# weilonghu/KGC-GCN

Measured on NVIDIA B200. Metric: edges/sec GCN fwd+bwd, higher is better.
Workload: dtype f32

## Files before the change

### include/kgc_b200.h

```cpp
#ifndef KGC_B200_H_
#define KGC_B200_H_

#include <stddef.h>
#include <stdint.h>

#ifdef __cplusplus
extern "C" {
#endif
#if defined(__GNUC__)
#pragma GCC visibility push(default)
#endif

#define KGC_ABI_VERSION 1

typedef struct { int32_t beg, end, out, flags; } kgc_item_t;

#define KGC_CHUNK_EDGES 32
typedef struct { int32_t head_slot, tail_slot; } kgc_chunk_t;

typedef struct { int32_t eid, a, b; float norm; } kgc_edge_rec_t;

const char* kgc_last_error(void);
int kgc_abi_version(void);

size_t kgc_csr_workspace_bytes(int64_t n_edges2, int64_t n_nodes, int64_t n_types);
int kgc_csr_build(const int64_t* src, const int64_t* dst, const int64_t* type,
                  int64_t n_edges2, int64_t n_edges_in, int64_t n_nodes, int64_t n_dst_rows, int64_t dst_offset,
                  int64_t n_types, int32_t deg_given, int32_t* deg, float* norm,
                  int32_t* perm_dst, int32_t* rowptr_dst, int32_t* rowmid_dst, kgc_edge_rec_t* rec_dst,
                  int32_t* perm_src, int32_t* rowptr_src, kgc_edge_rec_t* rec_src,
                  int32_t* perm_type, int32_t* rowptr_type, kgc_edge_rec_t* rec_type,
                  int64_t type_block_rows, void* workspace, size_t workspace_bytes, void* stream);
int64_t kgc_csr_type_rows(int64_t n_nodes, int64_t n_types, int64_t type_block_rows);
int kgc_block_sum(const float* in, int64_t n_blocks, int64_t n, float* out, void* stream);

int kgc_stream_plan_flags(const int32_t* seg_beg, const int32_t* seg_end, const int32_t* seg_row, int64_t n_seg,
                          int64_t n_rec, int32_t chunk, uint32_t* rowflags, int32_t* rec_seg, int32_t* inter, void* stream);

int kgc_agg_fwd(const float* x, const float* rel, int64_t n_types, const float* ee,
                const kgc_edge_rec_t* rec_dst, const uint32_t* rowflags, const kgc_chunk_t* chunks, int64_t n_rec,
                float* out_final, float* carry, int32_t D, void* stream);

int kgc_rows_fill(const int32_t* rows, int64_t n_rows, const float* addend, float* out, int32_t D, void* stream);

int kgc_rows_reduce(const float* part_in, const kgc_item_t* items, int64_t n_items, int64_t n_large,
                    float* out_final, float* out_part, const float* addend, int32_t D, void* stream);

int kgc_agg_bwd_src(const float* x, const float* rel, int64_t n_types, const float* ee, const float* g3,
                    const kgc_edge_rec_t* rec_src, const uint32_t* rowflags, const kgc_chunk_t* chunks, int64_t n_rec,
                    int64_t n_dst_rows, int64_t n_edges_in, const float* loop_addend,
                    float* d_ee, float* dx_final, float* carry, int32_t D, void* stream);

int kgc_agg_bwd_rel(const float* x, const float* ee, const float* g3,
                    const kgc_edge_rec_t* rec_type, const uint32_t* rowflags, const kgc_chunk_t* chunks, int64_t n_rec,
                    int64_t n_dst_rows, int64_t n_edges_in,
                    float* drel_final, float* carry, int32_t D, void* stream);

int64_t kgc_tail_num_blocks(int64_t n_rows);
int kgc_dropout_mask(const int64_t* seed, int32_t plane, float drop_p, int64_t n_elem, uint8_t* mask, void* stream);
int32_t kgc_keep_pitch(void);
int kgc_tail_fwd(const float* res3, const uint8_t* mask_in, const uint8_t* mask_out, const int64_t* seed, float drop_p,
                 float keep_scale, const float* bias, int64_t n_rows, int32_t Dout, float* pre, double* partials,
                 uint8_t* keep, void* stream);
int kgc_colsum_finalize(const double* partials, int64_t n_blocks, int32_t Dout, double* sums, void* stream);
int kgc_colstats_from_sums(const double* sums, int64_t n_rows, int32_t Dout, float eps, int32_t training,
                           const float* running_mean, const float* running_var, float* stats, void* stream);
int kgc_colstats_finalize(const double* partials, int64_t n_blocks, int64_t n_rows, int32_t Dout, float eps,
                          float momentum, float* running_mean, float* running_var, int64_t* num_batches_tracked,
                          double* sums, float* stats, void* stream);
int kgc_colsum_finalize2(const double* partials, int64_t n_blocks, int32_t Dout, double* sums, float* sums32,
                         void* stream);
int kgc_tail_apply(const float* pre, const float* stats, const float* gamma, const float* beta,
                   int64_t n_rows, int32_t Dout, float* all_ent, const int64_t* out_seed, float out_drop_p,
                   uint8_t* out_keep, void* stream);
int kgc_tail_bwd_reduce(const float* g_ent, const float* pre, const float* stats, const float* gamma, const float* beta,
                        int64_t n_rows, int32_t Dout, double* partials, const uint8_t* out_keep, float out_scale,
                        void* stream);
int kgc_tail_bwd_apply(const float* g_ent, const float* pre, const float* stats, const float* gamma, const float* beta,
                       const double* sums, int32_t training, int64_t n_rows, int64_t n_rows_global, int32_t Dout,
                       float* d_out, const uint8_t* keep, float keep_scale, float* d_res2, const uint8_t* out_keep,
                       float out_scale, void* stream);

int kgc_conv_prep(const float* rels, int32_t n_rels, const float* loop_rel, const float* loop_edge, const float* w_in,
                  const float* w_out, const float* w_loop, const float* w_rel, int32_t D, int32_t Dout, float* relp,
                  float* all_rel, float* packed_fwd, float* packed_bwd, void* stream);
int kgc_conv_param_grads(const float* m_loop, const float* w_loop, const float* loop_rel, const float* loop_edge,
                         const float* relp, const float* w_rel, const float* g_rel, const float* d_relp,
                         int32_t n_rels, int32_t D, int32_t Dout, float* d_w_loop, float* d_loop_rel,
                         float* d_loop_edge, float* d_rels, float* d_w_rel, const float* rel_add, void* stream);

size_t kgc_gemm_packed_b_bytes(int32_t N, int32_t K);
int kgc_gemm_pack_b(const float* B, int64_t stride_k, int64_t stride_n, int32_t N, int32_t K, float* packed,
                    void* stream);
int kgc_gemm_nt(const float* A, int64_t M, int32_t K, int64_t lda, const float* packed_b, int32_t N, float* C,
                int64_t ldc, void* stream);
int kgc_gemm_nt_batch(int32_t n_prob, const float* const* A, int64_t M, int32_t K, int64_t lda,
                      const float* const* packed_b, int32_t N, float* const* C, int64_t ldc, void* stream);
int kgc_gemm_nt_batch_masked(int32_t n_prob, const float* const* A, int64_t M, int32_t K, int64_t lda,
                             const float* const* packed_b, int32_t N, float* const* C, int64_t ldc, const uint8_t* keep,
                             int32_t keep_pitch, float keep_scale, void* stream);
int kgc_gemm_nt_trans(const float* At, int64_t M, int32_t K, int64_t ldat, const float* packed_b, int32_t N,
                      float* Ct, int64_t ldct, void* stream);
void kgc_gemm_set_debug(long long* buf);

size_t kgc_gemm_tn_workspace_bytes(int64_t M, int32_t Ka, int32_t Nb);
int kgc_gemm_tn(const float* A, int64_t lda, const float* B, int64_t ldb, int64_t M, int32_t Ka, int32_t Nb,
                float* C, void* workspace, size_t workspace_bytes, void* stream);

size_t kgc_gemm_tn_tc_workspace_bytes(int64_t M, int32_t Ka, int32_t Nb);
int kgc_gemm_tn_tc(const float* A, int64_t lda, const float* B, int64_t ldb, int64_t M, int32_t Ka, int32_t Nb,
                   float* C, void* workspace, size_t workspace_bytes, void* stream);

int kgc_gemm_nt_splitk(const float* A, int64_t lda, const float* Bt, int64_t ldb, int64_t K, int32_t Ma, int32_t Nb,
                       float* C, void* workspace, size_t workspace_bytes, void* stream);

int kgc_gemm_tn_tc_batch(int32_t n_prob, const float* const* A, int64_t lda, const float* const* B, int64_t ldb,
                         int64_t M, int32_t Ka, int32_t Nb, float* const* C, void* workspace, size_t workspace_bytes,
                         void* stream);
int kgc_gemm_tn_tc_batch_masked(int32_t n_prob, const float* const* A, int64_t lda, const float* const* B, int64_t ldb,
                                int64_t M, int32_t Ka, int32_t Nb, float* const* C, void* workspace, size_t workspace_bytes,
                                const uint8_t* keep, int32_t keep_pitch, float keep_scale, void* stream);

int kgc_label_build(const int64_t* qid, int64_t B, const int64_t* triples, const int64_t* ptr,
                    const int32_t* idx, int64_t n_entity, float pos, float add,
                    int64_t* triple_out, float* label, void* stream);

int kgc_neg_sample(const int64_t* qid, int64_t B, const int64_t* ptr, const int32_t* idx, int64_t n_entity,
                   const uint32_t* draws, int32_t k, int32_t tries, int32_t* neg, void* stream);

int kgc_edge_sample(const int64_t* src, const int64_t* dst, const int64_t* type, int64_t n_triples, const uint32_t* draws,
                    int64_t m, int64_t* sub_src, int64_t* sub_dst, int64_t* sub_type, int64_t* eids, void* stream);

size_t kgc_bn2d_partials_bytes(int32_t C);
int kgc_bn2d_relu_drop_fwd(const float* x, int64_t B, int32_t C, int32_t HW, const float* gamma, const float* beta,
                           float* running_mean, float* running_var, float eps, float momentum, int32_t training,
                           int32_t relu, const int64_t* seed, float drop_p, double* partials, float* stats, float* y,
                           void* stream);
int kgc_bn2d_relu_drop_bwd(const float* dy, const float* x, int64_t B, int32_t C, int32_t HW, const float* gamma,
                           const float* beta, const float* stats, int32_t training, int32_t relu, const int64_t* seed,
                           float drop_p, double* partials, float* sums, float* dx, void* stream);

int kgc_conv1ch_supported(int32_t F, int32_t K, int32_t H, int32_t W);
size_t kgc_conv1ch_bwd_workspace_bytes(int64_t B, int32_t F, int32_t K);
int kgc_conv1ch_fwd(const float* x, const float* w, const float* bias, int64_t B, int32_t F, int32_t K, int32_t H,
                    int32_t W, float* y, void* stream);
int kgc_conv1ch_bwd(const float* dy, const float* x, const float* w, int64_t B, int32_t F, int32_t K, int32_t H,
                    int32_t W, float* dx, float* dw, void* workspace, void* stream);

typedef struct { float* param; const float* grad; float* exp_avg; float* exp_avg_sq; } kgc_opt_tensor_t;
int32_t kgc_opt_chunk_elems(void);
int kgc_clip_adam_step(const kgc_opt_tensor_t* tensors, const int32_t* items, int64_t n_items, const float* hyper,
                       double* state, double* partials, void* stream);

int kgc_p2p_allreduce(void* const* stage_ptrs_dev, int64_t offset_bytes, void* const* flag_ptrs_dev, int32_t rank,
                      int32_t world, uint32_t* epoch, int32_t* error, const void* in, void* out, int64_t n_bytes,
                      int32_t is_double, void* stream);
int kgc_p2p_barrier(void* const* flag_ptrs_dev, int32_t rank, int32_t world, uint32_t* epoch, int32_t* error, void* stream);
int kgc_p2p_halo_gather(void* const* table_ptrs_dev, int32_t rank, const int32_t* rows, const int32_t* order, int64_t n_rows,
                        int64_t block_rows, int32_t D, void* stream);
int kgc_p2p_halo_reduce(void* const* part_ptrs_dev, int32_t world, const int32_t* idx, const int32_t* row_ids, int64_t n_rows,
                        const float* addend, float* out, int32_t D, void* stream);

typedef struct kgc_ingest kgc_ingest_t;
int kgc_ingest_open(const char* data_dir, kgc_ingest_t** out);
void kgc_ingest_close(kgc_ingest_t* h);
int64_t kgc_ingest_count(const kgc_ingest_t* h, int32_t what);
int kgc_ingest_copy(const kgc_ingest_t* h, int32_t array, void* dst, int64_t capacity_bytes);
const char* kgc_ingest_name(const kgc_ingest_t* h, int32_t kind, int64_t id);

int kgc_score_1n_fwd(const float* ent, int64_t n_ent, int32_t D, int64_t ld_ent, const float* packed_x, int32_t B,
                     const float* bias, float* pred, int64_t ld_pred, void* stream);
int kgc_score_1n_logits(const float* ent, int64_t n_ent, int32_t D, int64_t ld_ent, const float* packed_x, int32_t B,
                        const float* bias, float* logits, int64_t ld_logits, void* stream);
int kgc_score_1n_bwd_logit(const float* d_pred, int64_t ld_dp, const float* pred, int64_t ld_p, int64_t n_ent,
                           int32_t B, int32_t ldt, float* d_logitT, float* d_bias, void* stream);

int64_t kgc_label_mask_words(int64_t n_entity);
int kgc_label_mask_build(const int64_t* qid, int64_t B, const int64_t* triples, const int64_t* ptr, const int32_t* idx,
                         int64_t n_entity, uint32_t* mask, int64_t* triple_out, void* stream);
int kgc_bce_1n_bwd_logit(const float* pred, int64_t ld_p, const uint32_t* mask, int64_t n_ent, int32_t B, int32_t ldt,
                         float pos, float add, float* d_logitT, float* d_bias, double* loss_partial, float* loss,
                         void* stream);
int kgc_score_1n_fwd_t(const float* ent, int64_t n_ent, int32_t D, int64_t ld_ent, const float* packed_x, int32_t B,
                       const float* bias, float* pred_t, int64_t ld_t, void* stream);
int64_t kgc_bce_1n_t_blocks(int64_t n_ent);
int kgc_label_mask_t_build(const int64_t* qid, int64_t B, const int64_t* ptr, const int32_t* idx, int64_t n_entity,
                           uint32_t* mask_t, void* stream);
int kgc_bce_1n_bwd_logit_t(float* pred_t, const uint32_t* mask_t, int64_t n_ent, int32_t B, int32_t ldt, float pos, float add,
                           float* d_bias, double* loss_partial, float* loss, void* stream);

int32_t kgc_score_kpad(int32_t d);
int kgc_score_pack_entities(const float* all_ent, const float* bias, int64_t n, int32_t d,
                            uint16_t* e_bf16, void* stream);
int kgc_score_pack_queries(const float* xq, int64_t b, int32_t d, uint16_t* q_bf16, void* stream);
size_t kgc_score_pairs_workspace_bytes(int64_t n_pairs, int32_t kpad);
int kgc_score_pairs(const uint16_t* q_bf16, const uint16_t* e_bf16, const int32_t* pair_q, const int32_t* pair_e,
                    int64_t n_pairs, int32_t kpad, float* s_out, void* workspace, size_t workspace_bytes,
                    void* stream);
int kgc_score_rank(const uint16_t* q_bf16, const uint16_t* e_bf16, int64_t b, int64_t n, int32_t kpad,
                   const float* thr, int32_t* count_gt, int32_t* count_eq, void* stream);
int kgc_rank_count_dense(const float* logits, int64_t ld, int64_t n_ent, int64_t b, const float* thr,
                         int32_t* count_gt, int32_t* count_eq, void* stream);
int kgc_rank_finalize(const int32_t* count_gt, const int32_t* count_eq, const float* thr, const float* s_filt,
                      const int64_t* filt_ptr, const int32_t* filt_idx, const int64_t* obj, int64_t b,
                      int32_t* ranks, int32_t* eq_out, double* sums13, void* stream);

size_t kgc_score_topk_workspace_bytes(int64_t b, int64_t n, int32_t kpad, int32_t k);
int kgc_score_topk(const uint16_t* q_bf16, const uint16_t* e_bf16, int64_t b, int64_t n, int32_t kpad,
                   const int64_t* excl_ptr, const int32_t* excl_idx, int32_t k, float* top_s, int32_t* top_id,
                   int32_t* count, void* workspace, size_t workspace_bytes, void* stream);
size_t kgc_topk_dense_workspace_bytes(int64_t b, int64_t n, int32_t k);
int kgc_topk_dense(const float* logits, int64_t ld, int64_t n, int64_t b, const int64_t* excl_ptr,
                   const int32_t* excl_idx, int32_t k, float* top_s, int32_t* top_id, int32_t* count,
                   void* workspace, size_t workspace_bytes, void* stream);

#if defined(__GNUC__)
#pragma GCC visibility pop
#endif
#ifdef __cplusplus
}
#endif
#endif
```

### kgc-gcn_b200/_lib.py

```python
import ctypes
import os

import torch

_HERE = os.path.dirname(os.path.abspath(__file__))
LIB_PATH = os.environ.get('KGC_LIB_PATH') or os.path.join(_HERE, 'libkgc_b200.so')
_LIB = None

_vp, _i64, _i32, _f32, _sz = ctypes.c_void_p, ctypes.c_int64, ctypes.c_int32, ctypes.c_float, ctypes.c_size_t

SIGNATURES = {
    'kgc_last_error': (ctypes.c_char_p, []),
    'kgc_abi_version': (ctypes.c_int, []),
    'kgc_csr_workspace_bytes': (_sz, [_i64, _i64, _i64]),
    'kgc_csr_build': (ctypes.c_int, [_vp, _vp, _vp, _i64, _i64, _i64, _i64, _i64, _i64, _i32, _vp, _vp, _vp, _vp, _vp,
                                     _vp, _vp, _vp, _vp, _vp, _vp, _vp, _i64, _vp, _sz, _vp]),
    'kgc_csr_type_rows': (_i64, [_i64, _i64, _i64]),
    'kgc_block_sum': (ctypes.c_int, [_vp, _i64, _i64, _vp, _vp]),
    'kgc_stream_plan_flags': (ctypes.c_int, [_vp, _vp, _vp, _i64, _i64, _i32, _vp, _vp, _vp, _vp]),
    'kgc_agg_fwd': (ctypes.c_int, [_vp, _vp, _i64, _vp, _vp, _vp, _vp, _i64, _vp, _vp, _i32, _vp]),
    'kgc_rows_fill': (ctypes.c_int, [_vp, _i64, _vp, _vp, _i32, _vp]),
    'kgc_rows_reduce': (ctypes.c_int, [_vp, _vp, _i64, _i64, _vp, _vp, _vp, _i32, _vp]),
    'kgc_agg_bwd_src': (ctypes.c_int, [_vp, _vp, _i64, _vp, _vp, _vp, _vp, _vp, _i64, _i64, _i64, _vp, _vp, _vp, _vp, _i32, _vp]),
    'kgc_agg_bwd_rel': (ctypes.c_int, [_vp, _vp, _vp, _vp, _vp, _vp, _i64, _i64, _i64, _vp, _vp, _i32, _vp]),
    'kgc_tail_num_blocks': (_i64, [_i64]),
    'kgc_dropout_mask': (ctypes.c_int, [_vp, _i32, _f32, _i64, _vp, _vp]),
    'kgc_keep_pitch': (_i32, []),
    'kgc_tail_fwd': (ctypes.c_int, [_vp, _vp, _vp, _vp, _f32, _f32, _vp, _i64, _i32, _vp, _vp, _vp, _vp]),
    'kgc_colsum_finalize': (ctypes.c_int, [_vp, _i64, _i32, _vp, _vp]),
    'kgc_colstats_from_sums': (ctypes.c_int, [_vp, _i64, _i32, _f32, _i32, _vp, _vp, _vp, _vp]),
    'kgc_colstats_finalize': (ctypes.c_int, [_vp, _i64, _i64, _i32, _f32, _f32, _vp, _vp, _vp, _vp, _vp, _vp]),
    'kgc_colsum_finalize2': (ctypes.c_int, [_vp, _i64, _i32, _vp, _vp, _vp]),
    'kgc_tail_apply': (ctypes.c_int, [_vp, _vp, _vp, _vp, _i64, _i32, _vp, _vp, _f32, _vp, _vp]),
    'kgc_tail_bwd_reduce': (ctypes.c_int, [_vp, _vp, _vp, _vp, _vp, _i64, _i32, _vp, _vp, _f32, _vp]),
    'kgc_tail_bwd_apply': (ctypes.c_int, [_vp, _vp, _vp, _vp, _vp, _vp, _i32, _i64, _i64, _i32, _vp, _vp, _f32, _vp, _vp, _f32, _vp]),
    'kgc_gemm_packed_b_bytes': (_sz, [_i32, _i32]),
    'kgc_gemm_pack_b': (ctypes.c_int, [_vp, _i64, _i64, _i32, _i32, _vp, _vp]),
    'kgc_gemm_nt': (ctypes.c_int, [_vp, _i64, _i32, _i64, _vp, _i32, _vp, _i64, _vp]),
    'kgc_conv_prep': (ctypes.c_int, [_vp, _i32] + [_vp] * 6 + [_i32, _i32] + [_vp] * 5),
    'kgc_conv_param_grads': (ctypes.c_int, [_vp] * 8 + [_i32, _i32, _i32] + [_vp] * 7),
    'kgc_gemm_nt_batch': (ctypes.c_int, [_i32, _vp, _i64, _i32, _i64, _vp, _i32, _vp, _i64, _vp]),
    'kgc_gemm_nt_batch_masked': (ctypes.c_int, [_i32, _vp, _i64, _i32, _i64, _vp, _i32, _vp, _i64, _vp, _i32, _f32, _vp]),
    'kgc_gemm_tn_tc_batch_masked': (ctypes.c_int, [_i32, _vp, _i64, _vp, _i64, _i64, _i32, _i32, _vp, _vp, _sz, _vp, _i32, _f32, _vp]),
    'kgc_gemm_nt_trans': (ctypes.c_int, [_vp, _i64, _i32, _i64, _vp, _i32, _vp, _i64, _vp]),
    'kgc_gemm_nt_splitk': (ctypes.c_int, [_vp, _i64, _vp, _i64, _i64, _i32, _i32, _vp, _vp, _sz, _vp]),
    'kgc_gemm_set_debug': (None, [_vp]),
    'kgc_gemm_tn_workspace_bytes': (_sz, [_i64, _i32, _i32]),
    'kgc_gemm_tn_tc_workspace_bytes': (_sz, [_i64, _i32, _i32]),
    'kgc_gemm_tn_tc': (ctypes.c_int, [_vp, _i64, _vp, _i64, _i64, _i32, _i32, _vp, _vp, _sz, _vp]),
    'kgc_gemm_tn_tc_batch': (ctypes.c_int, [_i32, _vp, _i64, _vp, _i64, _i64, _i32, _i32, _vp, _vp, _sz, _vp]),
    'kgc_gemm_tn': (ctypes.c_int, [_vp, _i64, _vp, _i64, _i64, _i32, _i32, _vp, _vp, _sz, _vp]),
    'kgc_label_build': (ctypes.c_int, [_vp, _i64, _vp, _vp, _vp, _i64, _f32, _f32, _vp, _vp, _vp]),
    'kgc_neg_sample': (ctypes.c_int, [_vp, _i64, _vp, _vp, _i64, _vp, _i32, _i32, _vp, _vp]),
    'kgc_edge_sample': (ctypes.c_int, [_vp, _vp, _vp, _i64, _vp, _i64, _vp, _vp, _vp, _vp, _vp]),
    'kgc_bn2d_partials_bytes': (_sz, [_i32]),
    'kgc_bn2d_relu_drop_fwd': (ctypes.c_int, [_vp, _i64, _i32, _i32, _vp, _vp, _vp, _vp, _f32, _f32, _i32, _i32, _vp, _f32, _vp, _vp, _vp, _vp]),
    'kgc_bn2d_relu_drop_bwd': (ctypes.c_int, [_vp, _vp, _i64, _i32, _i32, _vp, _vp, _vp, _i32, _i32, _vp, _f32, _vp, _vp, _vp, _vp]),
    'kgc_conv1ch_supported': (_i32, [_i32, _i32, _i32, _i32]),
    'kgc_conv1ch_bwd_workspace_bytes': (_sz, [_i64, _i32, _i32]),
    'kgc_conv1ch_fwd': (ctypes.c_int, [_vp, _vp, _vp, _i64, _i32, _i32, _i32, _i32, _vp, _vp]),
    'kgc_conv1ch_bwd': (ctypes.c_int, [_vp, _vp, _vp, _i64, _i32, _i32, _i32, _i32, _vp, _vp, _vp, _vp]),
    'kgc_opt_chunk_elems': (_i32, []),
    'kgc_clip_adam_step': (ctypes.c_int, [_vp, _vp, _i64, _vp, _vp, _vp, _vp]),
    'kgc_p2p_allreduce': (ctypes.c_int, [_vp, _i64, _vp, _i32, _i32, _vp, _vp, _vp, _vp, _i64, _i32, _vp]),
    'kgc_p2p_barrier': (ctypes.c_int, [_vp, _i32, _i32, _vp, _vp, _vp]),
    'kgc_p2p_halo_gather': (ctypes.c_int, [_vp, _i32, _vp, _vp, _i64, _i64, _i32, _vp]),
    'kgc_p2p_halo_reduce': (ctypes.c_int, [_vp, _i32, _vp, _vp, _i64, _vp, _vp, _i32, _vp]),
    'kgc_ingest_open': (ctypes.c_int, [ctypes.c_char_p, _vp]),
    'kgc_ingest_close': (None, [_vp]),
    'kgc_ingest_count': (_i64, [_vp, _i32]),
    'kgc_ingest_copy': (ctypes.c_int, [_vp, _i32, _vp, _i64]),
    'kgc_ingest_name': (ctypes.c_char_p, [_vp, _i32, _i64]),
    'kgc_score_1n_fwd': (ctypes.c_int, [_vp, _i64, _i32, _i64, _vp, _i32, _vp, _vp, _i64, _vp]),
    'kgc_score_1n_logits': (ctypes.c_int, [_vp, _i64, _i32, _i64, _vp, _i32, _vp, _vp, _i64, _vp]),
    'kgc_rank_count_dense': (ctypes.c_int, [_vp, _i64, _i64, _i64, _vp, _vp, _vp, _vp]),
    'kgc_score_1n_bwd_logit': (ctypes.c_int, [_vp, _i64, _vp, _i64, _i64, _i32, _i32, _vp, _vp, _vp]),
    'kgc_label_mask_words': (_i64, [_i64]),
    'kgc_label_mask_build': (ctypes.c_int, [_vp, _i64, _vp, _vp, _vp, _i64, _vp, _vp, _vp]),
    'kgc_bce_1n_bwd_logit': (ctypes.c_int, [_vp, _i64, _vp, _i64, _i32, _i32, _f32, _f32, _vp, _vp, _vp, _vp, _vp]),
    'kgc_score_1n_fwd_t': (ctypes.c_int, [_vp, _i64, _i32, _i64, _vp, _i32, _vp, _vp, _i64, _vp]),
    'kgc_bce_1n_t_blocks': (_i64, [_i64]),
    'kgc_label_mask_t_build': (ctypes.c_int, [_vp, _i64, _vp, _vp, _i64, _vp, _vp]),
    'kgc_bce_1n_bwd_logit_t': (ctypes.c_int, [_vp, _vp, _i64, _i32, _i32, _f32, _f32, _vp, _vp, _vp, _vp]),
    'kgc_score_kpad': (_i32, [_i32]),
    'kgc_score_pack_entities': (ctypes.c_int, [_vp, _vp, _i64, _i32, _vp, _vp]),
    'kgc_score_pack_queries': (ctypes.c_int, [_vp, _i64, _i32, _vp, _vp]),
    'kgc_score_pairs_workspace_bytes': (_sz, [_i64, _i32]),
    'kgc_score_pairs': (ctypes.c_int, [_vp, _vp, _vp, _vp, _i64, _i32, _vp, _vp, _sz, _vp]),
    'kgc_score_rank': (ctypes.c_int, [_vp, _vp, _i64, _i64, _i32, _vp, _vp, _vp, _vp]),
    'kgc_rank_finalize': (ctypes.c_int, [_vp, _vp, _vp, _vp, _vp, _vp, _vp, _i64, _vp, _vp, _vp, _vp]),
    'kgc_score_topk_workspace_bytes': (_sz, [_i64, _i64, _i32, _i32]),
    'kgc_score_topk': (ctypes.c_int, [_vp, _vp, _i64, _i64, _i32, _vp, _vp, _i32, _vp, _vp, _vp, _vp, _sz, _vp]),
    'kgc_topk_dense_workspace_bytes': (_sz, [_i64, _i64, _i32]),
    'kgc_topk_dense': (ctypes.c_int, [_vp, _i64, _i64, _i64, _vp, _vp, _i32, _vp, _vp, _vp, _vp, _sz, _vp]),
}


def lib():
    global _LIB
    if _LIB is None:
        if not os.path.exists(LIB_PATH):
            raise RuntimeError('{} is missing: build it with `python -c "import __graft_entry__ as g; g.build()"` '
                               '(nvcc, sm_100a). There is no CPU or PyTorch fallback.'.format(LIB_PATH))
        handle = ctypes.CDLL(LIB_PATH)
        for name, (res, args) in SIGNATURES.items():
            fn = getattr(handle, name)
            fn.restype, fn.argtypes = res, args
        if handle.kgc_abi_version() != 1:
            raise RuntimeError('libkgc_b200.so ABI version mismatch')
        _LIB = handle
    return _LIB


LAUNCHES = 0
_KERNELS_PER_CALL = {'kgc_csr_build': 16, 'kgc_label_mask_build': 2, 'kgc_bce_1n_bwd_logit': 2, 'kgc_bce_1n_bwd_logit_t': 2, 'kgc_label_mask_t_build': 2, 'kgc_score_pairs': 3, 'kgc_rank_finalize': 2, 'kgc_score_topk': 2, 'kgc_topk_dense': 2, 'kgc_gemm_tn': 2, 'kgc_gemm_tn_tc': 2, 'kgc_gemm_tn_tc_batch': 2, 'kgc_gemm_tn_tc_batch_masked': 2}


def call(name, *args):
    global LAUNCHES
    h = lib()
    LAUNCHES += _KERNELS_PER_CALL.get(name, 1)
    rc = getattr(h, name)(*args)
    if rc != 0:
        raise RuntimeError('{} failed: {}'.format(name, h.kgc_last_error().decode('utf-8', 'replace')))


_WARNED = set()


def library_path(site, reason):
    msg = 'kgc_gcn_b200: {} is running on the torch library path ({})'.format(site, reason)
    if os.environ.get('KGC_STRICT', '0') not in ('', '0'):
        raise RuntimeError(msg + ' and KGC_STRICT=1 forbids it')
    if site not in _WARNED:
        _WARNED.add(site)
        import warnings
        warnings.warn(msg, RuntimeWarning, stacklevel=3)


def ptr(t):
    return None if t is None else ctypes.c_void_p(t.data_ptr())


def stream():
    return ctypes.c_void_p(torch.cuda.current_stream().cuda_stream)


def require_cuda(t, dtype, name):
    if not (torch.is_tensor(t) and t.is_cuda):
        raise RuntimeError('{} must be a CUDA tensor: the M-GCN hot path runs on the GPU only (no CPU fallback)'.format(name))
    if t.dtype != dtype:
        raise TypeError('{} must be {}, got {}'.format(name, dtype, t.dtype))
    return t if t.is_contiguous() else t.contiguous()
```

### kgc-gcn_b200/conv.py

```python
import os

import torch
import torch.nn as nn

from . import _lib
from .plan import get_plan


def get_param(shape):
    param = nn.Parameter(torch.empty(*shape))
    nn.init.xavier_uniform_(param.data)
    return param


def _mm(a, b, out):
    return torch.mm(a, b, out=out)


def gemm_nt(a, b_kn, out, plan=None, tag='b', packed=None):
    M, K = a.shape
    N = out.shape[1]
    if a.stride(1) != 1 or out.stride(1) != 1:
        raise ValueError('gemm_nt needs unit inner strides')
    p = _lib.ptr
    if packed is None:
        nbytes = int(_lib.lib().kgc_gemm_packed_b_bytes(N, K))
        if nbytes == 0:
            raise ValueError('gemm_nt: unsupported shape K={} N={}'.format(K, N))
        packed = plan.scratch('gemm_pack_' + tag, (nbytes // 4,)) if plan is not None else \
            torch.empty((nbytes // 4,), dtype=torch.float32, device=a.device)
        _lib.call('kgc_gemm_pack_b', p(b_kn), b_kn.stride(0), b_kn.stride(1), N, K, p(packed), _lib.stream())
    dst = out if (out.data_ptr() % 16 == 0 and out.stride(0) % 4 == 0) else \
        torch.empty((M, (N + 3) // 4 * 4), dtype=torch.float32, device=a.device)[:, :N]
    _lib.call('kgc_gemm_nt', p(a), M, K, a.stride(0), p(packed), N, p(dst), dst.stride(0), _lib.stream())
    if dst is not out:
        out.copy_(dst)
    return out


def gemm_nt_batch(a_list, packed_list, out_list, keep=None, keep_scale=1.0):
    import ctypes
    n = len(a_list)
    M, K = a_list[0].shape
    N = out_list[0].shape[1]
    lda, ldc = a_list[0].stride(0), out_list[0].stride(0)
    for a, o in zip(a_list, out_list):
        if a.shape != (M, K) or o.shape != (M, N) or a.stride() != (lda, 1) or o.stride() != (ldc, 1):
            raise ValueError('gemm_nt_batch needs operands of identical shape and strides')
    arr = lambda ts: (ctypes.c_void_p * n)(*[t.data_ptr() for t in ts])
    if keep is not None:
        _lib.call('kgc_gemm_nt_batch_masked', n, arr(a_list), M, K, lda, arr(packed_list), N, arr(out_list), ldc,
                  _lib.ptr(keep), keep.stride(0), float(keep_scale), _lib.stream())
    else:
        _lib.call('kgc_gemm_nt_batch', n, arr(a_list), M, K, lda, arr(packed_list), N, arr(out_list), ldc, _lib.stream())
    return out_list


def gemm_tn_batch(a_list, b_list, out_list, plan=None, keep=None, keep_scale=1.0):
    import ctypes
    n = len(a_list)
    M, Ka = a_list[0].shape
    Nb = b_list[0].shape[1]
    lda, ldb = a_list[0].stride(0), b_list[0].stride(0)
    same = all(a.shape == (M, Ka) and b.shape == (M, Nb) and a.stride() == (lda, 1) and b.stride() == (ldb, 1)
               and o.is_contiguous() for a, b, o in zip(a_list, b_list, out_list))
    if not same or Ka > 128 or Nb > 224:
        if keep is not None:
            raise ValueError('gemm_tn_batch: the masked form needs Ka <= 128, Nb <= 224 and operands of identical shape')
        for a, b, o in zip(a_list, b_list, out_list):
            gemm_tn(a, b, o, plan)
        return out_list
    nbytes = int(_lib.lib().kgc_gemm_tn_tc_workspace_bytes(M, Ka, Nb))
    ws = plan.scratch('kgc_gemm_tn_tc_ws', (nbytes // 4,)) if plan is not None else \
        torch.empty((nbytes // 4,), dtype=torch.float32, device=a_list[0].device)
    arr = lambda ts: (ctypes.c_void_p * n)(*[t.data_ptr() for t in ts])
    if keep is not None:
        _lib.call('kgc_gemm_tn_tc_batch_masked', n, arr(a_list), lda, arr(b_list), ldb, M, Ka, Nb, arr(out_list), _lib.ptr(ws),
                  nbytes, _lib.ptr(keep), keep.stride(0), float(keep_scale), _lib.stream())
    else:
        _lib.call('kgc_gemm_tn_tc_batch', n, arr(a_list), lda, arr(b_list), ldb, M, Ka, Nb, arr(out_list), _lib.ptr(ws), nbytes,
                  _lib.stream())
    return out_list


def _pack_b(b_kn):
    K, N = b_kn.shape
    nbytes = int(_lib.lib().kgc_gemm_packed_b_bytes(N, K))
    if nbytes == 0:
        raise ValueError('unsupported small operand K={} N={} (K <= 256, N <= 1024)'.format(K, N))
    packed = torch.empty((nbytes // 4,), dtype=torch.float32, device=b_kn.device)
    _lib.call('kgc_gemm_pack_b', _lib.ptr(b_kn), b_kn.stride(0), b_kn.stride(1), N, K, _lib.ptr(packed), _lib.stream())
    return packed


def gemm_nt_trans(a_t, b_kn, out_t):
    K, M = a_t.shape
    N = b_kn.shape[1]
    if a_t.stride(1) != 1 or out_t.stride(1) != 1 or out_t.shape != (N, M):
        raise ValueError('gemm_nt_trans needs unit inner strides and out_t of shape [N, M]')
    p = _lib.ptr
    _lib.call('kgc_gemm_nt_trans', p(a_t), M, K, a_t.stride(0), p(_pack_b(b_kn)), N, p(out_t), out_t.stride(0), _lib.stream())
    return out_t


def gemm_nt_splitk(a, bt, out):
    Ma, K = a.shape
    Nb = bt.shape[0]
    if a.stride(1) != 1 or bt.stride(1) != 1 or not out.is_contiguous():
        raise ValueError('gemm_nt_splitk needs unit inner strides and a contiguous output')
    nbytes = int(_lib.lib().kgc_gemm_tn_tc_workspace_bytes(K, Ma, Nb))
    ws = torch.empty((nbytes // 4,), dtype=torch.float32, device=a.device)
    p = _lib.ptr
    _lib.call('kgc_gemm_nt_splitk', p(a), a.stride(0), p(bt), bt.stride(0), K, Ma, Nb, p(out), p(ws), nbytes, _lib.stream())
    return out


class _LinearFn(torch.autograd.Function):

    @staticmethod
    def forward(ctx, x, weight, bias):
        x_, w_ = x.detach(), weight.detach()
        y = gemm_nt_splitk(x_, w_, torch.empty((x_.shape[0], w_.shape[0]), dtype=torch.float32, device=x.device))
        if bias is not None:
            y += bias.detach()
        ctx.save_for_backward(x_, w_)
        ctx.has_bias = bias is not None
        return y

    @staticmethod
    def backward(ctx, dy):
        x, w = ctx.saved_tensors
        dy = dy.contiguous()
        dx = dw = db = None
        if ctx.needs_input_grad[0]:
            dx = gemm_nt_trans(w, dy.t(), torch.empty_like(x))
        if ctx.needs_input_grad[1]:
            dw = gemm_nt_trans(x, dy, torch.empty_like(w))
        if ctx.has_bias and ctx.needs_input_grad[2]:
            db = dy.sum(0)
        return dx, dw, db


def linear_tc_supported(x, weight):
    B, F = x.shape
    O = weight.shape[0]
    return (x.is_cuda and x.dtype == torch.float32 and weight.dtype == torch.float32 and x.is_contiguous()
            and weight.is_contiguous() and 0 < B <= 128 and O <= 224 and O % 4 == 0 and F % 32 == 0 and F >= 4096
            and x.data_ptr() % 16 == 0 and weight.data_ptr() % 16 == 0)


def linear_tc(x, weight, bias=None):
    return _LinearFn.apply(x, weight, bias)


def gemm_tn(a, b, out, plan=None, tensor_cores=True):
    M, Ka = a.shape
    Nb = b.shape[1]
    if a.stride(1) != 1 or b.stride(1) != 1 or not out.is_contiguous():
        raise ValueError('gemm_tn needs unit inner strides and a contiguous output')
    if Nb > 256:
        raise ValueError('gemm_tn supports Nb <= 256')
    name = 'kgc_gemm_tn_tc' if (tensor_cores and Nb <= 224) else 'kgc_gemm_tn'
    for i0 in range(0, Ka, 128):
        kb = min(128, Ka - i0)
        a_blk, out_blk = a[:, i0:i0 + kb], out[i0:i0 + kb]
        nbytes = int(getattr(_lib.lib(), name + '_workspace_bytes')(M, kb, Nb))
        ws = plan.scratch(name + '_ws', (nbytes // 4,)) if plan is not None else \
            torch.empty((nbytes // 4,), dtype=torch.float32, device=a.device)
        p = _lib.ptr
        _lib.call(name, p(a_blk), a.stride(0), p(b), b.stride(0), M, kb, Nb, p(out_blk), p(ws), nbytes, _lib.stream())
    return out


class _Done(object):

    def wait(self):
        return None


class _StreamJoin(object):

    def __init__(self, stream):
        self.stream = stream

    def wait(self):
        torch.cuda.current_stream().wait_stream(self.stream)


class _Collectives(object):

    def __init__(self, group, world, n_global, n_hub=0, hub_idx_mine=None, hub_rows_mine=None, p2p=None, rank=0,
                 halo_rows=None, n_loc=None):
        self.group, self.world, self.n_global, self.rank = group, int(world), int(n_global), int(rank)
        self.n_loc = None if n_loc is None else int(n_loc)
        self.p2p = p2p
        self.halo_rows = halo_rows
        self.n_hub, self.hub_idx_mine, self.hub_rows_mine = int(n_hub), hub_idx_mine, hub_rows_mine

    def sum_hub_rows(self, planes, n_loc):
        if self.n_hub == 0:
            return
        buf = planes[:, n_loc:, :].contiguous()
        self.all_reduce(buf, 'hub_f')
        if self.hub_idx_mine.numel():
            planes[:, self.hub_rows_mine, :] = buf[:, self.hub_idx_mine, :]

    def spread_hub_rows(self, planes, n_planes, n_loc):
        if self.n_hub == 0:
            return
        buf = torch.zeros((n_planes, self.n_hub, planes.shape[2]), dtype=planes.dtype, device=planes.device)
        if self.hub_idx_mine.numel():
            buf[:, self.hub_idx_mine, :] = planes[:n_planes, self.hub_rows_mine, :]
        self.all_reduce(buf, 'hub_b')
        planes[:n_planes, n_loc:, :] = buf

    def all_gather_rows(self, x_local, async_op=False):
        import torch.distributed as dist
        out = torch.empty((self.world * x_local.shape[0],) + tuple(x_local.shape[1:]), dtype=x_local.dtype,
                          device=x_local.device)
        work = dist.all_gather_into_tensor(out, x_local.contiguous(), group=self.group, async_op=async_op)
        return (out, work) if async_op else out

    def gather_compact(self, x_blk):
        full = self.all_gather_rows(x_blk)
        return torch.cat([x_blk, full.index_select(0, self.halo_rows)], 0)

    def reduce_compact(self, partial, block):
        full = partial.new_zeros((self.world * block, partial.shape[1]))
        full[self.rank * block:(self.rank + 1) * block] = partial[:block]
        full[self.halo_rows] = partial[block:block + self.halo_rows.numel()]
        return self.reduce_scatter_rows(full)

    def reduce_scatter_rows(self, full, async_op=False):
        import torch.distributed as dist
        rows = full.shape[0] // self.world
        if dist.get_backend(self.group) == 'gloo':
            dist.all_reduce(full, group=self.group)
            r = dist.get_rank(self.group)
            out = full[r * rows:(r + 1) * rows].clone()
            return (out, None) if async_op else out
        out = torch.empty((rows,) + tuple(full.shape[1:]), dtype=full.dtype, device=full.device)
        work = dist.reduce_scatter_tensor(out, full.contiguous(), group=self.group, async_op=async_op)
        return (out, work) if async_op else out

    def all_reduce(self, t, tag=None):
        if self.p2p is not None and tag is not None and self.p2p.all_reduce(t, tag):
            return t
        import torch.distributed as dist
        dist.all_reduce(t, group=self.group)
        return t


class _ConvFn(torch.autograd.Function):

    @staticmethod
    def forward(ctx, x, rels, ee, w_in, w_out, w_loop, w_rel, loop_rel, loop_edge, gamma, beta, bias,
                plan, mask_in, mask_out, keep_scale, training, running_mean, running_var, eps, coll, seed, drop_p,
                bn_track=None, out_drop=None):
        Nl, D = x.shape
        Dout = w_in.shape[1]
        p, st = _lib.ptr, _lib.stream
        x = _lib.require_cuda(x, torch.float32, 'x')
        ee = _lib.require_cuda(ee, torch.float32, 'edge_embs')
        n_global = Nl if coll is None else coll.n_global
        n_hub = 0 if coll is None else coll.n_hub
        n_loc = Nl if coll is None or coll.n_loc is None else coll.n_loc
        if not 0 <= n_loc - Nl <= 1:
            raise ValueError('x has {} rows, the partition expects {} or {}'.format(Nl, n_loc, n_loc - 1))
        Nb = n_loc + n_hub
        compact = coll is not None and coll.halo_rows is not None
        n_table = Nl if coll is None else (Nb + coll.halo_rows.numel() if compact else Nb * coll.world)
        hybrid = coll is not None and coll.p2p is not None and coll.p2p.hybrid
        n_dst = n_table if hybrid else Nb
        if ee.shape[0] != plan.num_edges2 or n_dst != plan.num_dst_rows or plan.num_nodes != n_table:
            raise ValueError('edge_embs / x do not match the graph plan')
        T = rels.shape[0] + 1
        if T != plan.num_types:
            raise ValueError('rels_embs rows + 1 must equal the number of edge types of the plan')
        nf = int(_lib.lib().kgc_gemm_packed_b_bytes(Dout, D)) // 4
        nbk = int(_lib.lib().kgc_gemm_packed_b_bytes(D, Dout)) // 4
        if nf == 0 or nbk == 0:
            raise ValueError('unsupported layer width {} -> {} (<= 256)'.format(D, Dout))
        relp = torch.empty((T, D), dtype=torch.float32, device=x.device)
        all_rel_pad = torch.empty((T, Dout), dtype=torch.float32, device=x.device)
        packed_f = torch.empty((3, nf), dtype=torch.float32, device=x.device)
        packed_b = torch.empty((4, nbk), dtype=torch.float32, device=x.device)
        rels_c, wts = rels.detach().contiguous(), [w.detach().contiguous() for w in (w_in, w_out, w_loop, w_rel)]
        main, side = torch.cuda.current_stream(), plan.side_stream()
        side.wait_stream(main)
        with torch.cuda.stream(side):
            _lib.call('kgc_conv_prep', p(rels_c), T - 1, p(loop_rel.detach()), p(loop_edge.detach()), p(wts[0]), p(wts[1]),
                      p(wts[2]), p(wts[3]), D, Dout, p(relp), p(all_rel_pad), p(packed_f), p(packed_b), st())
        gather = None
        if coll is None:
            x_full = x
        elif coll.p2p is not None:
            ex = coll.p2p.exchange_stream
            ex.wait_stream(main)
            with torch.cuda.stream(ex):
                x_full = coll.p2p.gather(x, fence=not training)
            gather = _StreamJoin(ex)
        elif compact:
            x_blk = x if Nb == Nl else torch.cat([x, x.new_zeros((Nb - Nl, D))], 0)
            x_full, gather = coll.gather_compact(x_blk), _Done()
        else:
            x_full, gather = coll.all_gather_rows(x if Nb == Nl else torch.cat([x, x.new_zeros((Nb - Nl, D))], 0),
                                                  async_op=True)

        res3 = plan.scratch('res3', (3, Nl, Dout))
        if gather is not None:
            main.wait_stream(side)
            gemm_nt(x, None, res3[2], packed=packed_f[2])
            gather.wait()
        if max(x_full.shape[0], 3 * n_dst, ee.shape[0]) * (D // 4) >= 1 << 32:
            raise ValueError('kgc_gcn_b200: node / edge tables of 2^32 float4 elements or more are not supported')
        agg = torch.empty((2, n_dst, D), dtype=torch.float32, device=x.device)

        def level0(sp, out_final, carry):
            _lib.call('kgc_agg_fwd', p(x_full), p(rels_c), T - 1, p(ee), p(plan.rec_dst), p(sp.rowflags), p(sp.chunks), sp.n_rec,
                      p(out_final), p(carry), D, st())
        plan.run_reduction(plan.fwd, level0, agg, D, tag='f')
        if gather is None:
            main.wait_stream(side)

        if hybrid:
            coll.p2p.reduce_agg(agg)
        if gather is not None:
            coll.sum_hub_rows(agg, n_loc)
            gemm_nt_batch([agg[0, :Nl], agg[1, :Nl]], [packed_f[0], packed_f[1]], [res3[0], res3[1]])
        else:
            gemm_nt_batch([agg[0], agg[1], x], [packed_f[0], packed_f[1], packed_f[2]], [res3[0], res3[1], res3[2]])

        nb = int(_lib.lib().kgc_tail_num_blocks(Nl))
        partials = plan.scratch('colpart', (nb, 2, Dout), torch.float64)
        sums = torch.empty((2, Dout), dtype=torch.float64, device=x.device)
        pre = torch.empty((Nl, Dout), dtype=torch.float32, device=x.device)
        stats = torch.empty((3, Dout), dtype=torch.float32, device=x.device)
        all_ent = torch.empty((Nl, Dout), dtype=torch.float32, device=x.device)
        dropping = (mask_in is not None or seed is not None) and drop_p > 0.0
        keep = torch.empty((Nl, int(_lib.lib().kgc_keep_pitch())), dtype=torch.uint8, device=x.device) if dropping else None
        _lib.call('kgc_tail_fwd', p(res3), p(mask_in), p(mask_out), p(seed), float(drop_p), float(keep_scale), p(bias),
                  Nl, Dout, p(pre), p(partials), p(keep), st())
        if training and coll is None:
            mom, nbt = bn_track if bn_track is not None else (0.0, None)
            _lib.call('kgc_colstats_finalize', p(partials), nb, n_global, Dout, float(eps), float(mom),
                      p(running_mean) if bn_track is not None else None, p(running_var) if bn_track is not None else None,
                      p(nbt), None, p(stats), st())
        else:
            if training:
                _lib.call('kgc_colsum_finalize', p(partials), nb, Dout, p(sums), st())
                coll.all_reduce(sums, 'bn_f')
            _lib.call('kgc_colstats_from_sums', p(sums), n_global, Dout, float(eps), int(training), p(running_mean),
                      p(running_var), p(stats), st())
        out_p, out_seed = out_drop if out_drop is not None else (0.0, None)
        out_keep = torch.empty((Nl, int(_lib.lib().kgc_keep_pitch())), dtype=torch.uint8, device=x.device) if out_seed is not None else None
        _lib.call('kgc_tail_apply', p(pre), p(stats), p(gamma), p(beta), Nl, Dout, p(all_ent), p(out_seed), float(out_p),
                  p(out_keep), st())
        ctx.out_scale = 1.0 / (1.0 - float(out_p)) if out_seed is not None else 1.0
        all_rel = all_rel_pad[:-1]

        ctx.plan, ctx.training, ctx.keep_scale, ctx.has_bias, ctx.coll = plan, bool(training), float(keep_scale), \
            bias is not None, coll
        ctx.drop_p = float(drop_p)
        ctx.save_for_backward(x, x_full, relp, ee, w_in, w_out, w_loop, w_rel, loop_rel, loop_edge, gamma, beta, agg, pre,
                              all_ent, stats, keep, packed_b, out_keep)
        ctx.mark_non_differentiable(stats)
        return all_ent, all_rel, stats

    @staticmethod
    def backward(ctx, g_ent, g_rel, _g_stats):
        (x, x_full, relp, ee, w_in, w_out, w_loop, w_rel, loop_rel, loop_edge, gamma, beta, agg, pre, all_ent, stats, keep,
         packed_b, out_keep) = ctx.saved_tensors
        plan, coll = ctx.plan, ctx.coll
        Nl, D = x.shape
        n_global = Nl if coll is None else coll.n_global
        n_hub = 0 if coll is None else coll.n_hub
        n_loc = Nl if coll is None or coll.n_loc is None else coll.n_loc
        Nb = n_loc + n_hub
        Dout = w_in.shape[1]
        T = relp.shape[0]
        p, st = _lib.ptr, _lib.stream
        dev = x.device
        if g_ent is None:
            g_ent = torch.zeros_like(all_ent)
        g_ent = g_ent.contiguous()

        nb = int(_lib.lib().kgc_tail_num_blocks(Nl))
        partials = plan.scratch('colpart', (nb, 2, Dout), torch.float64)
        sums = torch.empty((2, Dout), dtype=torch.float64, device=dev)
        d_out = plan.scratch('d_out', (Nl, Dout))
        _lib.call('kgc_tail_bwd_reduce', p(g_ent), p(pre), p(stats), p(gamma), p(beta), Nl, Dout, p(partials), p(out_keep),
                  ctx.out_scale, st())
        if coll is None:
            sums32 = torch.empty((2, Dout), dtype=torch.float32, device=dev)
            _lib.call('kgc_colsum_finalize2', p(partials), nb, Dout, p(sums), p(sums32), st())
        else:
            _lib.call('kgc_colsum_finalize', p(partials), nb, Dout, p(sums), st())
            coll.all_reduce(sums, 'bn_b')
            sums32 = sums.float()
        mode = os.environ.get('KGC_TAIL_PLANES', '')
        three = (3 * Nl * Dout * 4 > (48 << 20)) if mode not in ('1', '3') else mode == '3'
        d_res2 = plan.scratch('d_res2', (2, Nl, Dout)) if three else None
        _lib.call('kgc_tail_bwd_apply', p(g_ent), p(pre), p(stats), p(gamma), p(beta), p(sums), int(ctx.training), Nl,
                  n_global, Dout, p(d_out), p(keep), ctx.keep_scale, p(d_res2), p(out_keep), ctx.out_scale, st())
        ups = [d_res2[0], d_res2[1], d_out] if three else [d_out, d_out, d_out]
        gkeep = None if three else keep
        d_beta, d_gamma = sums32[0], sums32[1]

        flat = torch.empty((3 * D * Dout + T * D + (Dout if ctx.has_bias else 0),), dtype=torch.float32, device=dev)
        d_w_in, d_w_out, m_loop = (flat[k * D * Dout:(k + 1) * D * Dout].view(D, Dout) for k in range(3))
        d_relp = flat[3 * D * Dout:3 * D * Dout + T * D].view(T, D)
        main, side = torch.cuda.current_stream(), plan.side_stream()
        side.wait_stream(main)
        with torch.cuda.stream(side):
            gemm_tn_batch([agg[0, :Nl], agg[1, :Nl], x], ups, [d_w_in, d_w_out, m_loop], plan,
                          keep=gkeep, keep_scale=ctx.keep_scale)
            if ctx.has_bias:
                torch.sum(d_out, 0, out=flat[3 * D * Dout + T * D:])

        hybrid = coll is not None and coll.p2p is not None and coll.p2p.hybrid
        g3 = coll.p2p.g3_planes() if hybrid else plan.scratch('g3', (3, Nb, D))
        gemm_nt_batch(ups, [packed_b[0], packed_b[1], packed_b[2]],
                      [g3[0, :Nl], g3[1, :Nl], g3[2, :Nl]], keep=gkeep, keep_scale=ctx.keep_scale)
        if n_hub:
            coll.spread_hub_rows(g3, 2, n_loc)
        if hybrid:
            coll.p2p.gather_g()
        p2p = None if coll is None else coll.p2p
        d_x_full = p2p.partial if (p2p is not None and not hybrid) else torch.empty((plan.num_nodes, D), dtype=torch.float32, device=dev)
        d_ee = torch.empty_like(ee)
        loop_addend = g3[2] if (coll is None or hybrid) else None

        def level0_src(sp, out_final, carry):
            _lib.call('kgc_agg_bwd_src', p(x_full), p(relp), relp.shape[0], p(ee), p(g3), p(plan.rec_src), p(sp.rowflags), p(sp.chunks),
                      sp.n_rec, plan.num_dst_rows, plan.num_edges_in, p(loop_addend), p(d_ee), p(out_final), p(carry),
                      D, st())
        plan.run_reduction(plan.bwd_src, level0_src, d_x_full, D, addend=loop_addend, tag='s')
        scatter = None
        if hybrid:
            ex = p2p.exchange_stream
            ex.wait_stream(main)
            with torch.cuda.stream(ex):
                p2p.reduce_dx(d_x_full, channel=1)
            d_x = d_x_full[:Nl]
        elif p2p is not None:
            d_x = torch.empty((Nl, D), dtype=torch.float32, device=dev)
            ex = p2p.exchange_stream
            ex.wait_stream(main)
            with torch.cuda.stream(ex):
                p2p.reduce(g3[2, :Nl], Nl, out=d_x, channel=1)
        compact = coll is not None and coll.halo_rows is not None
        if coll is not None and p2p is None and not compact:
            d_x, scatter = coll.reduce_scatter_rows(d_x_full, async_op=True)

        def level0_rel(sp, out_final, carry):
            _lib.call('kgc_agg_bwd_rel', p(x_full), p(ee), p(g3), p(plan.rec_type), p(sp.rowflags), p(sp.chunks), sp.n_rec,
                      plan.num_dst_rows, plan.num_edges_in, p(out_final), p(carry), D, st())
        plan.run_rel_reduction(level0_rel, d_relp, D)

        main.wait_stream(side)
        if coll is None:
            d_x = d_x_full
        elif p2p is not None:
            coll.all_reduce(flat, 'flat')
            main.wait_stream(p2p.exchange_stream)
        elif compact:
            coll.all_reduce(flat, 'flat')
            d_x = coll.reduce_compact(d_x_full, Nb)[:Nl] + g3[2, :Nl]
        else:
            coll.all_reduce(flat, 'flat')
            if scatter is not None:
                scatter.wait()
            d_x = d_x[:Nl] + g3[2, :Nl]
        d_bias = flat[3 * D * Dout + T * D:] * 3.0 if ctx.has_bias else None
        small = torch.empty((2 * D * Dout + 2 * D + (T - 1) * D,), dtype=torch.float32, device=dev)
        d_w_loop, d_w_rel = small[:D * Dout].view(D, Dout), small[D * Dout:2 * D * Dout].view(D, Dout)
        o = 2 * D * Dout
        d_loop_rel, d_loop_edge, d_rels = small[o:o + D].view(1, D), small[o + D:o + 2 * D].view(1, D), small[o + 2 * D:].view(T - 1, D)
        g_rel_c = None if g_rel is None else g_rel.contiguous()
        rel_add = None
        if g_rel_c is not None and T - 1 >= 256 and g_rel_c.data_ptr() % 16 == 0 and Dout % 4 == 0 and (D * Dout) % 32 == 0:
            rel_add = gemm_nt(g_rel_c, None, torch.empty((T - 1, D), dtype=torch.float32, device=dev), packed=packed_b[3])
            gemm_tn(relp[:T - 1], g_rel_c, d_w_rel, plan)
        _lib.call('kgc_conv_param_grads', p(m_loop), p(w_loop.detach().contiguous()), p(loop_rel.detach()), p(loop_edge.detach()),
                  p(relp), p(w_rel.detach().contiguous()), p(g_rel_c), p(d_relp), T - 1, D, Dout, p(d_w_loop), p(d_loop_rel),
                  p(d_loop_edge), p(d_rels), p(d_w_rel), p(rel_add), st())
        return (d_x, d_rels, d_ee, d_w_in, d_w_out, d_w_loop, d_w_rel, d_loop_rel, d_loop_edge, d_gamma, d_beta, d_bias,
                None, None, None, None, None, None, None, None, None, None, None, None, None)


class MGCNConv(nn.Module):

    def __init__(self, in_channels, out_channels, num_relations, bias=False, dropout=0.1, **kwargs):
        super(MGCNConv, self).__init__()
        self.in_channels = in_channels
        self.out_channels = out_channels
        self.num_relations = num_relations
        self.aggr = 'add'

        self.ent_bn = nn.BatchNorm1d(out_channels)
        self.drop = nn.Dropout(dropout)
        self.act = torch.tanh

        self.loop_weight = get_param((in_channels, out_channels))
        self.in_weight = get_param((in_channels, out_channels))
        self.out_weight = get_param((in_channels, out_channels))
        self.rels_weight = get_param((in_channels, out_channels))
        self.loop_rel = get_param((1, in_channels))
        self.loop_edge = get_param((1, in_channels))

        if bias is True:
            self.register_parameter('bias', nn.Parameter(torch.zeros(out_channels)))
        else:
            self.register_parameter('bias', None)
        self._forced_masks = None
        self.register_buffer('_drop_seed', torch.zeros(1, dtype=torch.int64), persistent=False)
        self._drop_seeded = False

    def set_dropout_masks(self, mask_in, mask_out):
        self._forced_masks = None if mask_in is None else (mask_in, mask_out)

    def compute_norm(self, edge_index, num_ent):
        ei = torch.cat([edge_index, edge_index], 1).contiguous()
        et = torch.zeros(ei.size(1), dtype=torch.int64, device=ei.device)
        return get_plan(ei, et, num_ent, 1).norm[:edge_index.size(1)].clone()

    def _masks(self, n_rows, device):
        p = self.drop.p
        if not self.training or p == 0.0:
            return None, None, 1.0, None, 0.0
        if self._forced_masks is not None:
            m_in, m_out = self._forced_masks
            return (m_in.to(device=device, dtype=torch.uint8).contiguous(),
                    m_out.to(device=device, dtype=torch.uint8).contiguous(), 1.0 / (1.0 - p), None, p)
        if not self._drop_seeded:
            self._drop_seed.fill_(int(torch.randint(0, 2 ** 62, (1,)).item()))
            self._drop_seeded = True
        self._drop_seed.add_(0x9E3779B97F4A7C15 & 0x7FFFFFFFFFFFFFFF)
        return None, None, 1.0 / (1.0 - p), self._drop_seed.clone(), p

    def _out_drop_cfg(self, p, seed):
        if not self.training or not p or p <= 0.0:
            return None
        if seed is None:
            if not self._drop_seeded:
                self._drop_seed.fill_(int(torch.randint(0, 2 ** 62, (1,)).item()))
                self._drop_seeded = True
            self._drop_seed.add_(0x9E3779B97F4A7C15 & 0x7FFFFFFFFFFFFFFF)
            seed = self._drop_seed.clone()
        self._last_out_seed = seed
        return float(p), seed

    def dropout_masks(self, seed, n_rows):
        out = []
        for plane in (0, 1):
            m = torch.empty((n_rows, self.out_channels), dtype=torch.uint8, device=seed.device)
            _lib.call('kgc_dropout_mask', _lib.ptr(seed), plane, float(self.drop.p), m.numel(), _lib.ptr(m), _lib.stream())
            out.append(m)
        return out

    def forward(self, x, edge_index, edge_type, edge_norm, edge_embs, rels_embs, size=None, _out_drop=0.0):
        num_ent = x.size(0)
        plan = get_plan(edge_index, edge_type, num_ent, rels_embs.size(0) + 1)
        m_in, m_out, keep_scale, seed, drop_p = self._masks(num_ent, x.device)
        self._last_seed = seed
        bn = self.ent_bn
        use_batch_stats = self.training or bn.running_mean is None
        track = self.training and bn.track_running_stats and bn.running_mean is not None
        fused = track and bn.momentum is not None
        all_ent, all_rel, stats = _ConvFn.apply(
            x, rels_embs, edge_embs, self.in_weight, self.out_weight, self.loop_weight, self.rels_weight,
            self.loop_rel, self.loop_edge, bn.weight, bn.bias, self.bias, plan, m_in, m_out, keep_scale,
            use_batch_stats, bn.running_mean, bn.running_var, bn.eps, None, seed, drop_p,
            (float(bn.momentum), bn.num_batches_tracked) if fused else None, self._out_drop_cfg(_out_drop, seed))
        if track and not fused:
            self._update_running_stats(stats, num_ent)
        return all_ent, all_rel

    def _update_running_stats(self, stats, n_rows):
        bn = self.ent_bn
        if self.training and bn.track_running_stats and bn.running_mean is not None:
            with torch.no_grad():
                bn.num_batches_tracked += 1
                mom = bn.momentum if bn.momentum is not None else 1.0 / float(bn.num_batches_tracked)
                unbias = float(n_rows) / float(max(n_rows - 1, 1))
                bn.running_mean.mul_(1.0 - mom).add_(stats[0], alpha=mom)
                bn.running_var.mul_(1.0 - mom).add_(stats[1], alpha=mom * unbias)

    def forward_partitioned(self, x_local, part, edge_embs_local, rels_embs):
        m_in, m_out, keep_scale, seed, drop_p = self._masks(x_local.size(0), x_local.device)
        if seed is not None:
            seed = seed + part.rank
        self._last_seed = seed
        bn = self.ent_bn
        use_batch_stats = self.training or bn.running_mean is None
        coll = _Collectives(part.group, part.world, part.num_nodes, part.n_hub, part.hub_idx_mine, part.hub_rows_mine,
                            part.p2p(x_local.shape[1]), part.rank, getattr(part, 'halo_rows64', None), part.n_loc)
        all_ent, all_rel, stats = _ConvFn.apply(
            x_local, rels_embs, edge_embs_local, self.in_weight, self.out_weight, self.loop_weight, self.rels_weight,
            self.loop_rel, self.loop_edge, bn.weight, bn.bias, self.bias, part.plan, m_in, m_out, keep_scale,
            use_batch_stats, bn.running_mean, bn.running_var, bn.eps, coll, seed, drop_p)
        self._update_running_stats(stats, part.num_nodes)
        return all_ent, all_rel

    def __repr__(self):
        return '{}({}, {}, num_relations={})'.format(self.__class__.__name__, self.in_channels, self.out_channels,
                                                     self.num_relations)
```

### kgc-gcn_b200/csrc/gemm_tf32x3.cu

```cuda
#include <cuda.h>

#include <cstdlib>
#include "common.cuh"

namespace kgc {
namespace {

constexpr int kBM = 128;
constexpr int kBK = 32;
constexpr int kUK = 8;
constexpr int kMaxKB = 8;
constexpr int kMaxStages = 8;
constexpr int kAStages = 4;
constexpr int kAccCols = 256;
constexpr int kTmemColsTS = kAccCols + kAStages * 64;
constexpr int kTileA = kBM * kBK * 4;
constexpr int kThreadsG = 480;
constexpr int kSplitWarps = 8;
constexpr int kBBudget = 116 * 1024;
constexpr int kTmemColsG = 256;
constexpr int kEpiBuf = 32 * 128;
constexpr int kEpiStage = 4 * 2 * kEpiBuf;

__device__ __forceinline__ uint32_t s_u32(const void* p) { return (uint32_t)__cvta_generic_to_shared(p); }
__device__ __forceinline__ void mb_init(uint64_t* bar, uint32_t count) {
  asm volatile("mbarrier.init.shared::cta.b64 [%0], %1;" ::"r"(s_u32(bar)), "r"(count));
}
__device__ __forceinline__ void mb_expect_tx(uint64_t* bar, uint32_t bytes) {
  asm volatile("mbarrier.arrive.expect_tx.shared::cta.b64 _, [%0], %1;" ::"r"(s_u32(bar)), "r"(bytes) : "memory");
}
__device__ __forceinline__ void mb_arrive(uint64_t* bar) {
  asm volatile("mbarrier.arrive.shared::cta.b64 _, [%0];" ::"r"(s_u32(bar)) : "memory");
}
__device__ __forceinline__ void mb_wait(uint64_t* bar, uint32_t parity) {
  asm volatile(
      "{\n"
      ".reg .pred P1;\n"
      "LAB_WAIT:\n"
      "mbarrier.try_wait.parity.shared::cta.b64 P1, [%0], %1;\n"
      "@P1 bra DONE;\n"
      "bra LAB_WAIT;\n"
      "DONE:\n"
      "}" ::"r"(s_u32(bar)),
      "r"(parity)
      : "memory");
}
__device__ __forceinline__ void tma_2d(void* smem_dst, const CUtensorMap* map, uint64_t* bar, int c0, int c1) {
  asm volatile(
      "cp.async.bulk.tensor.2d.shared::cluster.global.mbarrier::complete_tx::bytes [%0], [%1, {%3, %4}], [%2];" ::"r"(
          s_u32(smem_dst)),
      "l"(reinterpret_cast<uint64_t>(map)), "r"(s_u32(bar)), "r"(c0), "r"(c1)
      : "memory");
}
__device__ __forceinline__ void tma_3d(void* smem_dst, const CUtensorMap* map, uint64_t* bar, int c0, int c1, int c2) {
  asm volatile(
      "cp.async.bulk.tensor.3d.shared::cluster.global.mbarrier::complete_tx::bytes [%0], [%1, {%3, %4, %5}], [%2];" ::"r"(
          s_u32(smem_dst)),
      "l"(reinterpret_cast<uint64_t>(map)), "r"(s_u32(bar)), "r"(c0), "r"(c1), "r"(c2)
      : "memory");
}
__device__ __forceinline__ void tma_store_2d(const CUtensorMap* map, const void* smem_src, int c0, int c1) {
  asm volatile("cp.async.bulk.tensor.2d.global.shared::cta.bulk_group [%0, {%2, %3}], [%1];" ::"l"(
                   reinterpret_cast<uint64_t>(map)),
               "r"(s_u32(smem_src)), "r"(c0), "r"(c1)
               : "memory");
}
__device__ __forceinline__ void tma_store_3d(const CUtensorMap* map, const void* smem_src, int c0, int c1, int c2) {
  asm volatile("cp.async.bulk.tensor.3d.global.shared::cta.bulk_group [%0, {%2, %3, %4}], [%1];" ::"l"(
                   reinterpret_cast<uint64_t>(map)),
               "r"(s_u32(smem_src)), "r"(c0), "r"(c1), "r"(c2)
               : "memory");
}
__device__ __forceinline__ void umma_tf32(uint32_t tmem_d, uint64_t adesc, uint64_t bdesc, uint32_t idesc, uint32_t acc) {
  asm volatile(
      "{\n"
      ".reg .pred p;\n"
      "setp.ne.b32 p, %4, 0;\n"
      "tcgen05.mma.cta_group::1.kind::tf32 [%0], %1, %2, %3, p;\n"
      "}" ::"r"(tmem_d),
      "l"(adesc), "l"(bdesc), "r"(idesc), "r"(acc)
      : "memory");
}
__device__ __forceinline__ void umma_tf32_ts(uint32_t tmem_d, uint32_t a_tmem, uint64_t bdesc, uint32_t idesc, uint32_t acc) {
  asm volatile(
      "{\n"
      ".reg .pred p;\n"
      "setp.ne.b32 p, %4, 0;\n"
      "tcgen05.mma.cta_group::1.kind::tf32 [%0], [%1], %2, %3, p;\n"
      "}" ::"r"(tmem_d),
      "r"(a_tmem), "l"(bdesc), "r"(idesc), "r"(acc)
      : "memory");
}
__device__ __forceinline__ void tmem_st16_g(uint32_t taddr, const uint32_t (&v)[16]) {
  asm volatile(
      "tcgen05.st.sync.aligned.32x32b.x16.b32 [%0], "
      "{%1, %2, %3, %4, %5, %6, %7, %8, %9, %10, %11, %12, %13, %14, %15, %16};" ::"r"(taddr),
      "r"(v[0]), "r"(v[1]), "r"(v[2]), "r"(v[3]), "r"(v[4]), "r"(v[5]), "r"(v[6]), "r"(v[7]), "r"(v[8]), "r"(v[9]),
      "r"(v[10]), "r"(v[11]), "r"(v[12]), "r"(v[13]), "r"(v[14]), "r"(v[15])
      : "memory");
}
__device__ __forceinline__ bool elect_one() {
  uint32_t pred = 0;
  asm volatile(
      "{\n"
      ".reg .b32 rx;\n"
      ".reg .pred px;\n"
      "elect.sync rx|px, 0xFFFFFFFF;\n"
      "@px mov.s32 %0, 1;\n"
      "}"
      : "+r"(pred));
  return pred != 0;
}
__device__ __forceinline__ uint32_t tf32_rn(float v) { return (__float_as_uint(v) + 0x1000u) & 0xFFFFE000u; }
__device__ __forceinline__ void split_tf32(uint32_t v, uint32_t& hi, uint32_t& lo) {
  hi = tf32_rn(__uint_as_float(v));
  lo = tf32_rn(__uint_as_float(v) - __uint_as_float(hi));
}
__device__ __forceinline__ void umma_commit_g(uint64_t* bar) {
  asm volatile("tcgen05.commit.cta_group::1.mbarrier::arrive::one.shared::cluster.b64 [%0];" ::"r"(s_u32(bar)) : "memory");
}
__device__ __forceinline__ void tmem_ld32_g(uint32_t taddr, uint32_t (&v)[32]) {
  asm volatile(
      "tcgen05.ld.sync.aligned.32x32b.x32.b32 "
      "{%0, %1, %2, %3, %4, %5, %6, %7, %8, %9, %10, %11, %12, %13, %14, %15, "
      "%16, %17, %18, %19, %20, %21, %22, %23, %24, %25, %26, %27, %28, %29, %30, %31}, [%32];"
      : "=r"(v[0]), "=r"(v[1]), "=r"(v[2]), "=r"(v[3]), "=r"(v[4]), "=r"(v[5]), "=r"(v[6]), "=r"(v[7]), "=r"(v[8]),
        "=r"(v[9]), "=r"(v[10]), "=r"(v[11]), "=r"(v[12]), "=r"(v[13]), "=r"(v[14]), "=r"(v[15]), "=r"(v[16]),
        "=r"(v[17]), "=r"(v[18]), "=r"(v[19]), "=r"(v[20]), "=r"(v[21]), "=r"(v[22]), "=r"(v[23]), "=r"(v[24]),
        "=r"(v[25]), "=r"(v[26]), "=r"(v[27]), "=r"(v[28]), "=r"(v[29]), "=r"(v[30]), "=r"(v[31])
      : "r"(taddr));
}
__device__ __forceinline__ uint64_t sw128_desc(uint32_t smem_addr) {
  uint64_t d = 0;
  d |= (uint64_t)((smem_addr & 0x3FFFF) >> 4);
  d |= (uint64_t)(1024 >> 4) << 32;
  d |= (uint64_t)1 << 46;
  d |= (uint64_t)2 << 61;
  return d;
}

constexpr int kMaxBatch = 3;
struct GemmMaps {
  CUtensorMap a[kMaxBatch], bhi[kMaxBatch], blo[kMaxBatch], c[kMaxBatch], c16[kMaxBatch];
};

struct GemmParams {
  int64_t M;
  int32_t n_prob;
  int32_t N, K;
  int32_t n_kb, ksteps, NT, n_ntiles, n_mtiles, stages;
  float* C;
  int64_t ldc;
  const float* row_bias;
  int32_t act;
  int32_t trans_c;
  int32_t trans_a;
  const uint8_t* keep;
  int32_t keep_pitch;
  float keep_scale;
  long long* dbg;
};

__global__ void __launch_bounds__(kThreadsG, 1)
gemm_tf32x3_kernel(const __grid_constant__ GemmMaps maps, const GemmParams P) {
  extern __shared__ uint8_t smem_raw[];
  if (P.dbg != nullptr && threadIdx.x == 0) {
    long long g;
    asm volatile("mov.u64 %0, %globaltimer;" : "=l"(g));
    atomicMin(reinterpret_cast<long long*>(P.dbg) + 8 * 64 + 0, g);
    if (blockIdx.x == 0) { P.dbg[8 * 64 + 2] = g; P.dbg[8 * 64 + 3] = clock64(); }
  }
  uint8_t* base = reinterpret_cast<uint8_t*>((reinterpret_cast<uintptr_t>(smem_raw) + 1023) & ~uintptr_t(1023));
  const int warp = threadIdx.x / 32, lane = threadIdx.x % 32;
  const int tile_b = P.NT * kBK * 4;
  const int tile_b_al = (tile_b + 1023) & ~1023;
  uint8_t* s_bhi = base;
  uint8_t* s_blo = s_bhi + P.n_kb * tile_b_al;
  const int kStages = P.stages;
  uint8_t* s_a = s_blo + P.n_kb * tile_b_al;
  uint8_t* s_stage = s_a + kStages * kTileA;
  uint64_t* bars = reinterpret_cast<uint64_t*>(s_stage + kEpiStage);
  uint64_t* b_full = bars;
  uint64_t* raw_full = bars + 1;
  uint64_t* raw_empty = raw_full + kMaxStages;
  uint64_t* split_full = raw_empty + kMaxStages;
  uint64_t* split_empty = split_full + kAStages;
  uint64_t* acc_full = split_empty + kAStages;
  uint64_t* acc_empty = acc_full + 2;
  uint32_t* tmem_slot = reinterpret_cast<uint32_t*>(acc_empty + 2);

  if (warp == 0 && lane == 0) {
    mb_init(b_full, 1);
    for (int i = 0; i < kStages; ++i) {
      mb_init(raw_full + i, 1);
      mb_init(raw_empty + i, kSplitWarps);
    }
    for (int i = 0; i < kAStages; ++i) {
      mb_init(split_full + i, kSplitWarps);
      mb_init(split_empty + i, 1);
    }
    for (int i = 0; i < 2; ++i) {
      mb_init(acc_full + i, 1);
      mb_init(acc_empty + i, 4);
    }
    asm volatile("fence.mbarrier_init.release.cluster;" ::: "memory");
    asm volatile("fence.proxy.async.shared::cta;" ::: "memory");
  }
  if (warp == 14) {
    asm volatile("tcgen05.alloc.cta_group::1.sync.aligned.shared::cta.b32 [%0], %1;" ::"r"(s_u32(tmem_slot)), "r"(kTmemColsTS)
                 : "memory");
    asm volatile("tcgen05.relinquish_alloc_permit.cta_group::1.sync.aligned;" ::: "memory");
  }
  asm volatile("tcgen05.fence::before_thread_sync;" ::: "memory");
  __syncthreads();
  asm volatile("tcgen05.fence::after_thread_sync;" ::: "memory");
  const uint32_t tmem_base = *tmem_slot;
  const uint32_t tmem_a = tmem_base + kAccCols;
  const bool dbg_on = P.dbg != nullptr && blockIdx.x == 0;
  int dbg_n = 0;
#define KGC_DBG(role) do { if (dbg_on && dbg_n < 64) P.dbg[(role) * 64 + dbg_n++] = clock64(); } while (0)

  const int groups = P.n_prob * P.n_ntiles;
  const int prob = (blockIdx.x % groups) / P.n_ntiles;
  const int nt = blockIdx.x % P.n_ntiles;
  const int first = blockIdx.x / groups;
  const int step = gridDim.x / groups;
  const CUtensorMap* map_a = &maps.a[prob];
  const CUtensorMap* map_bhi = &maps.bhi[prob];
  const CUtensorMap* map_blo = &maps.blo[prob];
  const CUtensorMap* map_c = &maps.c[prob];
  const CUtensorMap* map_c16 = &maps.c16[prob];

  if (warp == 0) {
    if (lane == 0) {
      mb_expect_tx(b_full, 2u * P.n_kb * tile_b);
      for (int kb = 0; kb < P.n_kb; ++kb) {
        tma_2d(s_bhi + kb * tile_b_al, map_bhi, b_full, kb * kBK, nt * P.NT);
        tma_2d(s_blo + kb * tile_b_al, map_blo, b_full, kb * kBK, nt * P.NT);
      }
      int stage = 0;
      uint32_t phase = 0;
      for (int mt = first; mt < P.n_mtiles; mt += step) {
        for (int kb = 0; kb < P.n_kb; ++kb) {
          mb_wait(raw_empty + stage, phase ^ 1);
          KGC_DBG(0);
          mb_expect_tx(raw_full + stage, kTileA);
          if (P.trans_a) tma_3d(s_a + stage * kTileA, map_a, raw_full + stage, 0, kb * kBK, mt * (kBM / 32));
          else tma_2d(s_a + stage * kTileA, map_a, raw_full + stage, kb * kBK, mt * kBM);
          if (++stage == kStages) { stage = 0; phase ^= 1; }
        }
      }
    }
  } else if (warp >= 2 && warp < 2 + kSplitWarps) {
    const int quarter = warp % 4, half = (warp - 2) / 4;
    const int r = quarter * 32 + lane;
    int stage = 0, ts = 0;
    uint32_t phase = 0, tphase = 0;
    const bool masked = P.keep != nullptr && prob < 2 && !P.trans_a;
    uint32_t kcur[kMaxKB], knxt[kMaxKB];
#pragma unroll
    for (int j = 0; j < kMaxKB; ++j) kcur[j] = knxt[j] = 0u;
    auto load_keep = [&](int mt_, uint32_t (&w)[kMaxKB]) {
      const int64_t grow = (int64_t)mt_ * kBM + r;
      if (mt_ < P.n_mtiles && grow < P.M) {
        const uint4* kp = reinterpret_cast<const uint4*>(P.keep + grow * P.keep_pitch);
#pragma unroll
        for (int q = 0; q < kMaxKB / 2; ++q) {
          const uint4 t4 = __ldg(kp + q);
          w[2 * q] = half ? t4.y : t4.x;
          w[2 * q + 1] = half ? t4.w : t4.z;
        }
      }
    };
    if (masked) load_keep(first, knxt);
    for (int mt = first; mt < P.n_mtiles; mt += step) {
      if (masked) {
#pragma unroll
        for (int j = 0; j < kMaxKB; ++j) kcur[j] = knxt[j];
        load_keep(mt + step, knxt);
      }
      for (int kb = 0; kb < P.n_kb; ++kb) {
        uint32_t kw = 0;
        if (masked) {
#pragma unroll
          for (int j = 0; j < kMaxKB; ++j)
            if (kb == j) kw = kcur[j];
          if (prob == 1) kw >>= 4;
        }
        mb_wait(raw_full + stage, phase);
        if (warp == 2 && lane == 0) KGC_DBG(1);
        uint32_t h[16], l[16];
        if (P.trans_a) {
          const uint8_t* col = s_a + stage * kTileA + quarter * 4096 + ((lane & 3) << 2);
#pragma unroll
          for (int i = 0; i < 16; ++i) {
            const int kk = half * 16 + i;
            const uint32_t v = *reinterpret_cast<const uint32_t*>(col + kk * 128 + (((lane >> 2) ^ (kk & 7)) << 4));
            split_tf32(v, h[i], l[i]);
          }
        } else {
          const uint8_t* row = s_a + stage * kTileA + r * 128;
          uint4 v[4];
#pragma unroll
          for (int i = 0; i < 4; ++i) v[i] = *reinterpret_cast<const uint4*>(row + (((half * 4 + i) ^ (r & 7)) << 4));
          if (masked) {
#pragma unroll
            for (int i = 0; i < 4; ++i) {
              const uint32_t nb = kw >> (8 * i);
              v[i].x = (nb & 1u) ? __float_as_uint(__uint_as_float(v[i].x) * P.keep_scale) : 0u;
              v[i].y = (nb & 2u) ? __float_as_uint(__uint_as_float(v[i].y) * P.keep_scale) : 0u;
              v[i].z = (nb & 4u) ? __float_as_uint(__uint_as_float(v[i].z) * P.keep_scale) : 0u;
              v[i].w = (nb & 8u) ? __float_as_uint(__uint_as_float(v[i].w) * P.keep_scale) : 0u;
            }
          }
#pragma unroll
          for (int i = 0; i < 4; ++i) {
            split_tf32(v[i].x, h[4 * i + 0], l[4 * i + 0]);
            split_tf32(v[i].y, h[4 * i + 1], l[4 * i + 1]);
            split_tf32(v[i].z, h[4 * i + 2], l[4 * i + 2]);
            split_tf32(v[i].w, h[4 * i + 3], l[4 * i + 3]);
          }
        }
        __syncwarp();
        if (lane == 0) mb_arrive(raw_empty + stage);
        mb_wait(split_empty + ts, tphase ^ 1);
        if (warp == 2 && lane == 0) KGC_DBG(2);
        asm volatile("tcgen05.fence::after_thread_sync;" ::: "memory");
        const uint32_t taddr = tmem_a + ((uint32_t)(quarter * 32) << 16) + ts * 64 + half * 16;
        tmem_st16_g(taddr, h);
        tmem_st16_g(taddr + 32, l);
        asm volatile("tcgen05.wait::st.sync.aligned;" ::: "memory");
        asm volatile("tcgen05.fence::before_thread_sync;" ::: "memory");
        __syncwarp();
        if (lane == 0) mb_arrive(split_full + ts);
        if (warp == 2 && lane == 0) KGC_DBG(3);
        if (++stage == kStages) { stage = 0; phase ^= 1; }
        if (++ts == kAStages) { ts = 0; tphase ^= 1; }
      }
    }
  } else if (warp == 1) {
    {
      const uint32_t idesc = (1u << 4) | (2u << 7) | (2u << 10) | ((uint32_t)(P.NT >> 3) << 17) | ((uint32_t)(kBM >> 4) << 24);
      int ts = 0, acc = 0;
      uint32_t tphase = 0, acc_phase = 0;
      mb_wait(b_full, 0);
      asm volatile("tcgen05.fence::after_thread_sync;" ::: "memory");
      for (int mt = first; mt < P.n_mtiles; mt += step) {
        mb_wait(acc_empty + acc, acc_phase ^ 1);
        asm volatile("tcgen05.fence::after_thread_sync;" ::: "memory");
        const uint32_t d_addr = tmem_base + acc * (kAccCols / 2);
        for (int kb = 0; kb < P.n_kb; ++kb) {
          mb_wait(split_full + ts, tphase);
          if (lane == 0) KGC_DBG(4);
          asm volatile("tcgen05.fence::after_thread_sync;" ::: "memory");
          const int nk = min(kBK / kUK, P.ksteps - kb * (kBK / kUK));
          const uint32_t a_hi = tmem_a + ts * 64, a_lo = a_hi + 32;
          const uint64_t b_hi = sw128_desc(s_u32(s_bhi + kb * tile_b_al));
          const uint64_t b_lo = sw128_desc(s_u32(s_blo + kb * tile_b_al));
          if (elect_one()) {
#pragma unroll
            for (int k = 0; k < kBK / kUK; ++k) {
              if (k < nk) {
                umma_tf32_ts(d_addr, a_lo + 8 * k, b_hi + 2 * k, idesc, (k != 0 || kb != 0) ? 1u : 0u);
                umma_tf32_ts(d_addr, a_hi + 8 * k, b_lo + 2 * k, idesc, 1u);
                umma_tf32_ts(d_addr, a_hi + 8 * k, b_hi + 2 * k, idesc, 1u);
              }
            }
            umma_commit_g(split_empty + ts);
            if (kb == P.n_kb - 1) umma_commit_g(acc_full + acc);
          }
          __syncwarp();
          if (lane == 0) KGC_DBG(5);
          if (++ts == kAStages) { ts = 0; tphase ^= 1; }
        }
        if (++acc == 2) { acc = 0; acc_phase ^= 1; }
      }
    }
  } else if (warp >= 10 && warp <= 13) {
    const int quarter = warp % 4;
    uint8_t* stg = s_stage + (warp - 10) * (2 * kEpiBuf);
    const int64_t row_q = quarter * 32;
    int acc = 0, buf = 0;
    uint32_t acc_phase = 0;
    for (int mt = first; mt < P.n_mtiles; mt += step) {
      mb_wait(acc_full + acc, acc_phase);
      if (warp == 10 && lane == 0) KGC_DBG(6);
      asm volatile("tcgen05.fence::after_thread_sync;" ::: "memory");
      const int64_t m0 = (int64_t)mt * kBM + row_q;
      const uint32_t taddr = tmem_base + ((uint32_t)(quarter * 32) << 16) + acc * (kAccCols / 2);
      for (int c0 = 0; c0 < P.NT; c0 += 32) {
        uint32_t v[32];
        tmem_ld32_g(taddr + c0, v);
        asm volatile("tcgen05.wait::ld.sync.aligned;" ::: "memory");
        if (c0 + 32 >= P.NT) {
          asm volatile("tcgen05.fence::before_thread_sync;" ::: "memory");
          __syncwarp();
          if (lane == 0) mb_arrive(acc_empty + acc);
        }
        if (lane == 0) asm volatile("cp.async.bulk.wait_group.read 1;" ::: "memory");
        __syncwarp();
        uint8_t* bb = stg + buf * kEpiBuf;
        const bool wide = c0 + 32 <= P.NT;
        if (P.row_bias != nullptr) {
          const float bv = m0 + lane < P.M ? P.row_bias[m0 + lane] : 0.f;
#pragma unroll
          for (int j = 0; j < 32; ++j) {
            const float z = __uint_as_float(v[j]) + bv;
            v[j] = __float_as_uint(P.act == 1 ? 1.f / (1.f + expf(-z)) : z);
          }
        }
        if (P.trans_c) {
#pragma unroll
          for (int j = 0; j < 32; ++j)
            *reinterpret_cast<uint32_t*>(bb + j * 128 + ((((lane >> 2) ^ (j & 7)) << 4) | ((lane & 3) << 2))) = v[j];
        } else if (wide) {
          uint8_t* bx = bb + lane * 128;
          const int sw = lane & 7;
#pragma unroll
          for (int q = 0; q < 8; ++q)
            *reinterpret_cast<uint4*>(bx + ((q ^ sw) << 4)) = make_uint4(v[4 * q], v[4 * q + 1], v[4 * q + 2], v[4 * q + 3]);
        } else {
          uint8_t* bx = bb + lane * 64;
          const int sw = (lane >> 1) & 3;
#pragma unroll
          for (int q = 0; q < 4; ++q)
            *reinterpret_cast<uint4*>(bx + ((q ^ sw) << 4)) = make_uint4(v[4 * q], v[4 * q + 1], v[4 * q + 2], v[4 * q + 3]);
        }
        asm volatile("fence.proxy.async.shared::cta;" ::: "memory");
        __syncwarp();
        if (lane == 0) {
          const int col = nt * P.NT + c0;
          if (m0 < P.M && col < P.N) {
            if (P.trans_c) tma_store_2d(wide ? map_c : map_c16, bb, (int)m0, col);
            else tma_store_2d(wide ? map_c : map_c16, bb, col, (int)m0);
          }
          asm volatile("cp.async.bulk.commit_group;" ::: "memory");
        }
        buf ^= 1;
      }
      if (warp == 10 && lane == 0) KGC_DBG(7);
      if (++acc == 2) { acc = 0; acc_phase ^= 1; }
    }
    if (lane == 0) asm volatile("cp.async.bulk.wait_group 0;" ::: "memory");
  }
  asm volatile("tcgen05.fence::before_thread_sync;" ::: "memory");
  __syncthreads();
  if (P.dbg != nullptr && threadIdx.x == 0) {
    long long g;
    asm volatile("mov.u64 %0, %globaltimer;" : "=l"(g));
    atomicMax(reinterpret_cast<long long*>(P.dbg) + 8 * 64 + 1, g);
    if (blockIdx.x == 0) { P.dbg[8 * 64 + 4] = g; P.dbg[8 * 64 + 5] = clock64(); }
  }
  if (warp == 14) {
    asm volatile("tcgen05.dealloc.cta_group::1.sync.aligned.b32 %0, %1;" ::"r"(tmem_base), "r"(kTmemColsTS) : "memory");
  }
}

__global__ void pack_b_kernel(const float* __restrict__ B, int64_t sk, int64_t sn, int N, int K, int n_pad, int k_pad,
                              float* __restrict__ hi, float* __restrict__ lo) {
  const int i = blockIdx.x * blockDim.x + threadIdx.x;
  if (i >= n_pad * k_pad) return;
  const int n = i / k_pad, k = i % k_pad;
  float v = 0.f;
  if (n < N && k < K) v = B[(int64_t)k * sk + (int64_t)n * sn];
  uint32_t h, l;
  split_tf32(__float_as_uint(v), h, l);
  hi[i] = __uint_as_float(h);
  lo[i] = __uint_as_float(l);
}

struct PrepArgs {
  const float *rels, *loop_rel, *loop_edge, *w0, *w1, *w2, *w_rel;
  int n_rels, D, Dout;
  int n_pad_f, k_pad_f, n_pad_b, k_pad_b;
  float *relp, *all_rel, *packed_f, *packed_b;
};

__global__ void __launch_bounds__(256) conv_prep_kernel(const PrepArgs a) {
  const int T = a.n_rels + 1;
  int i = blockIdx.x * blockDim.x + threadIdx.x;
  const int n0 = T * a.D, n1 = T * a.Dout, nf = a.n_pad_f * a.k_pad_f, nb = a.n_pad_b * a.k_pad_b;
  if (i < n0) {
    const int t = i / a.D, c = i % a.D;
    a.relp[i] = t < a.n_rels ? a.rels[i] : a.loop_rel[c];
    return;
  }
  i -= n0;
  if (i < n1) {
    const int t = i / a.Dout, o = i % a.Dout;
    const float* r = t < a.n_rels ? a.rels + (int64_t)t * a.D : a.loop_rel;
    float acc = 0.f;
#pragma unroll 25
    for (int c = 0; c < a.D; ++c) acc = fmaf(r[c], a.w_rel[(int64_t)c * a.Dout + o], acc);
    a.all_rel[i] = acc;
    return;
  }
  i -= n1;
  if (i < 3 * nf) {
    const int h = i / nf, j0 = i % nf, k = j0 / a.n_pad_f, n = j0 % a.n_pad_f, j = n * a.k_pad_f + k;
    float v = 0.f;
    if (n < a.Dout && k < a.D) {
      const float* wh = h == 0 ? a.w0 : (h == 1 ? a.w1 : a.w2);
      v = wh[(int64_t)k * a.Dout + n];
      if (h == 2) v *= a.loop_rel[k] * a.loop_edge[k];
    }
    uint32_t hi, lo;
    split_tf32(__float_as_uint(v), hi, lo);
    float* dst = a.packed_f + (int64_t)h * 2 * nf;
    dst[j] = __uint_as_float(hi);
    dst[nf + j] = __uint_as_float(lo);
    return;
  }
  i -= 3 * nf;
  if (i < 4 * nb) {
    const int h = i / nb, j = i % nb, n = j / a.k_pad_b, k = j % a.k_pad_b;
    float v = 0.f;
    if (n < a.D && k < a.Dout) {
      const float* wh = h == 0 ? a.w0 : (h == 1 ? a.w1 : (h == 2 ? a.w2 : a.w_rel));
      v = wh[(int64_t)n * a.Dout + k];
      if (h == 2) v *= a.loop_rel[n] * a.loop_edge[n];
    }
    uint32_t hi, lo;
    split_tf32(__float_as_uint(v), hi, lo);
    float* dst = a.packed_b + (int64_t)h * 2 * nb;
    dst[j] = __uint_as_float(hi);
    dst[nb + j] = __uint_as_float(lo);
  }
}

struct ParamGradArgs {
  const float *m_loop, *w_loop, *loop_rel, *loop_edge, *relp, *w_rel, *g_rel, *d_relp;
  int n_rels, D, Dout;
  float *d_w_loop, *d_loop_rel, *d_loop_edge, *d_rels, *d_w_rel;
};

__global__ void __launch_bounds__(256) conv_param_grads_kernel(const ParamGradArgs a) {
  const int T = a.n_rels + 1;
  int i = blockIdx.x * blockDim.x + threadIdx.x;
  const int nw = a.D * a.Dout;
  if (i < nw) {
    const int c = i / a.Dout;
    a.d_w_loop[i] = a.loop_rel[c] * a.loop_edge[c] * a.m_loop[i];
    return;
  }
  i -= nw;
  if (i < nw) {
    const int c = i / a.Dout, o = i % a.Dout;
    float acc = 0.f;
    if (a.g_rel != nullptr) {
#pragma unroll 8
      for (int t = 0; t < a.n_rels; ++t) acc = fmaf(a.relp[(int64_t)t * a.D + c], a.g_rel[(int64_t)t * a.Dout + o], acc);
    }
    a.d_w_rel[i] = acc;
    return;
  }
  i -= nw;
  const int pair = i / 32, lane = i % 32;
  if (pair < T * a.D) {
    const int t = pair / a.D, c = pair % a.D;
    const float* u = t < a.n_rels ? a.g_rel + (int64_t)t * a.Dout : a.m_loop + (int64_t)c * a.Dout;
    const float* w = t < a.n_rels ? a.w_rel + (int64_t)c * a.Dout : a.w_loop + (int64_t)c * a.Dout;
    float acc = 0.f;
    if (t == a.n_rels || a.g_rel != nullptr)
      for (int o = lane; o < a.Dout; o += 32) acc = fmaf(u[o], w[o], acc);
#pragma unroll
    for (int s = 16; s > 0; s >>= 1) acc += __shfl_xor_sync(0xFFFFFFFFu, acc, s);
    if (lane == 0) {
      const float val = a.d_relp[pair];
      if (t < a.n_rels) {
        a.d_rels[pair] = val + acc;
      } else {
        a.d_loop_edge[c] = acc * a.loop_rel[c];
        a.d_loop_rel[c] = acc * a.loop_edge[c] + val;
      }
    }
  }
}

__global__ void __launch_bounds__(256) conv_param_grads2_kernel(const ParamGradArgs a, const float* __restrict__ rel_add) {
  int i = blockIdx.x * blockDim.x + threadIdx.x;
  const int nw = a.D * a.Dout;
  if (i < nw) {
    const int c = i / a.Dout;
    a.d_w_loop[i] = a.loop_rel[c] * a.loop_edge[c] * a.m_loop[i];
    return;
  }
  i -= nw;
  const int n_el = a.n_rels * a.D, n_el_pad = (n_el + 31) & ~31;
  if (i < n_el_pad) {
    if (i < n_el) a.d_rels[i] = a.d_relp[i] + rel_add[i];
    return;
  }
  i -= n_el_pad;
  const int c = i / 32, lane = i % 32;
  if (c < a.D) {
    const float* u = a.m_loop + (int64_t)c * a.Dout;
    const float* w = a.w_loop + (int64_t)c * a.Dout;
    float acc = 0.f;
    for (int o = lane; o < a.Dout; o += 32) acc = fmaf(u[o], w[o], acc);
#pragma unroll
    for (int s = 16; s > 0; s >>= 1) acc += __shfl_xor_sync(0xFFFFFFFFu, acc, s);
    if (lane == 0) {
      a.d_loop_edge[c] = acc * a.loop_rel[c];
      a.d_loop_rel[c] = acc * a.loop_edge[c] + a.d_relp[(int64_t)a.n_rels * a.D + c];
    }
  }
}

typedef CUresult (*EncodeTiledFn)(CUtensorMap*, CUtensorMapDataType, cuuint32_t, void*, const cuuint64_t*, const cuuint64_t*,
                                  const cuuint32_t*, const cuuint32_t*, CUtensorMapInterleave, CUtensorMapSwizzle,
                                  CUtensorMapL2promotion, CUtensorMapFloatOOBfill);
int encode_fn(EncodeTiledFn* out) {
  ensure_thread_context();
  static EncodeTiledFn cached = nullptr;
  if (!cached) {
    void* fn = nullptr;
    cudaDriverEntryPointQueryResult qres;
    KGC_CUDA_TRY(cudaGetDriverEntryPoint("cuTensorMapEncodeTiled", &fn, cudaEnableDefault, &qres));
    KGC_REQUIRE(qres == cudaDriverEntryPointSuccess && fn != nullptr, "cuTensorMapEncodeTiled not available");
    cached = reinterpret_cast<EncodeTiledFn>(fn);
  }
  *out = cached;
  return 0;
}
int make_map_f32(CUtensorMap* map, const void* ptr, int64_t rows, int64_t cols, int64_t pitch, int box_rows,
                 CUtensorMapSwizzle swizzle = CU_TENSOR_MAP_SWIZZLE_128B, int box_cols = kBK) {
  EncodeTiledFn enc;
  if (encode_fn(&enc)) return 1;
  KGC_REQUIRE((reinterpret_cast<uintptr_t>(ptr) & 15) == 0 && (pitch * 4) % 16 == 0, "operand must be 16-byte aligned with a 16-byte pitch");
  cuuint64_t dims[2] = {(cuuint64_t)cols, (cuuint64_t)rows};
  cuuint64_t strides[1] = {(cuuint64_t)pitch * 4};
  cuuint32_t box[2] = {(cuuint32_t)box_cols, (cuuint32_t)box_rows};
  cuuint32_t estr[2] = {1, 1};
  CUresult r = enc(map, CU_TENSOR_MAP_DATA_TYPE_FLOAT32, 2, const_cast<void*>(ptr), dims, strides, box, estr,
                   CU_TENSOR_MAP_INTERLEAVE_NONE, swizzle, CU_TENSOR_MAP_L2_PROMOTION_L2_256B,
                   CU_TENSOR_MAP_FLOAT_OOB_FILL_NONE);
  KGC_REQUIRE(r == CUDA_SUCCESS, "cuTensorMapEncodeTiled failed (" + std::to_string((int)r) + ")");
  return 0;
}

int make_map_f32_groups(CUtensorMap* map, const void* ptr, int64_t rows, int groups, int64_t pitch, int box_groups,
                        CUtensorMapSwizzle swizzle) {
  EncodeTiledFn enc;
  if (encode_fn(&enc)) return 1;
  KGC_REQUIRE((reinterpret_cast<uintptr_t>(ptr) & 15) == 0 && (pitch * 4) % 16 == 0, "operand must be 16-byte aligned with a 16-byte pitch");
  cuuint64_t dims[3] = {32, (cuuint64_t)rows, (cuuint64_t)groups};
  cuuint64_t strides[2] = {(cuuint64_t)pitch * 4, 128};
  cuuint32_t box[3] = {32, 32, (cuuint32_t)box_groups};
  cuuint32_t estr[3] = {1, 1, 1};
  CUresult r = enc(map, CU_TENSOR_MAP_DATA_TYPE_FLOAT32, 3, const_cast<void*>(ptr), dims, strides, box, estr,
                   CU_TENSOR_MAP_INTERLEAVE_NONE, swizzle, CU_TENSOR_MAP_L2_PROMOTION_L2_256B,
                   CU_TENSOR_MAP_FLOAT_OOB_FILL_NONE);
  KGC_REQUIRE(r == CUDA_SUCCESS, "cuTensorMapEncodeTiled (grouped operand) failed (" + std::to_string((int)r) + ")");
  return 0;
}
int make_map_f32_mn_groups(CUtensorMap* map, const void* ptr, int64_t rows, int groups, int64_t pitch) {
  return make_map_f32_groups(map, ptr, rows, groups, pitch, groups, CU_TENSOR_MAP_SWIZZLE_128B_ATOM_32B);
}

int make_map_f32_parts(CUtensorMap* map, const void* ptr, int64_t parts, int64_t rows, int64_t cols) {
  EncodeTiledFn enc;
  if (encode_fn(&enc)) return 1;
  KGC_REQUIRE((reinterpret_cast<uintptr_t>(ptr) & 15) == 0 && cols % 4 == 0, "partials must be 16-byte aligned with a 16-byte pitch");
  cuuint64_t dims[3] = {(cuuint64_t)cols, (cuuint64_t)rows, (cuuint64_t)parts};
  cuuint64_t strides[2] = {(cuuint64_t)cols * 4, (cuuint64_t)rows * cols * 4};
  cuuint32_t box[3] = {32, 32, 1};
  cuuint32_t estr[3] = {1, 1, 1};
  CUresult r = enc(map, CU_TENSOR_MAP_DATA_TYPE_FLOAT32, 3, const_cast<void*>(ptr), dims, strides, box, estr,
                   CU_TENSOR_MAP_INTERLEAVE_NONE, CU_TENSOR_MAP_SWIZZLE_128B, CU_TENSOR_MAP_L2_PROMOTION_L2_256B,
                   CU_TENSOR_MAP_FLOAT_OOB_FILL_NONE);
  KGC_REQUIRE(r == CUDA_SUCCESS, "cuTensorMapEncodeTiled failed (" + std::to_string((int)r) + ")");
  return 0;
}

struct Tiling {
  int n_kb, k_pad, ksteps, NT, n_ntiles, n_pad;
};
int make_tiling(int N, int K, Tiling* t) {
  if (N <= 0 || K <= 0 || K > kMaxKB * kBK || N > 1024) return 1;
  t->n_kb = (K + kBK - 1) / kBK;
  t->k_pad = t->n_kb * kBK;
  t->ksteps = (K + kUK - 1) / kUK;
  int nt_max = kBBudget / (2 * t->n_kb * kBK * 4);
  nt_max = nt_max / 16 * 16;
  if (nt_max > 128) nt_max = 128;
  if (nt_max < 16) return 1;
  t->n_ntiles = (N + nt_max - 1) / nt_max;
  t->NT = ((N + t->n_ntiles - 1) / t->n_ntiles + 15) / 16 * 16;
  t->n_pad = t->NT * t->n_ntiles;
  return 0;
}


constexpr int kTnRows = 32;
constexpr int kTnBox = kTnRows * 128;
constexpr int kTnStages = 3;
constexpr int kTnLoStages = 2;
constexpr int kTnMaxGb = 7;

struct GemmTnMaps {
  CUtensorMap a[kMaxBatch], b[kMaxBatch], a3[kMaxBatch], b3[kMaxBatch], p[kMaxBatch];
};

struct GemmTnParams {
  int64_t M;
  int32_t n_prob, n_slabs;
  int32_t Ka, Nb, ga, gb, n_pad;
  int32_t ga_full, gb_full;
  int32_t kmajor;
  int64_t rows_per_cta;
  float* partial;
  const uint8_t* keep;
  int32_t keep_pitch;
  float keep_scale;
  long long* dbg;
};

__device__ __forceinline__ uint64_t sw128_mn_desc(uint32_t smem_addr) {
  uint64_t d = 0;
  d |= (uint64_t)((smem_addr & 0x3FFFF) >> 4);
  d |= (uint64_t)(kTnBox >> 4) << 16;
  d |= (uint64_t)(512 >> 4) << 32;
  d |= (uint64_t)1 << 46;
  d |= (uint64_t)1 << 61;
  return d;
}

__global__ void __launch_bounds__(kThreadsG, 1)
gemm_tn_tc_kernel(const __grid_constant__ GemmTnMaps maps, const GemmTnParams P) {
  extern __shared__ uint8_t smem_raw[];
  if (P.dbg != nullptr && threadIdx.x == 0) {
    long long g;
    asm volatile("mov.u64 %0, %globaltimer;" : "=l"(g));
    atomicMin(reinterpret_cast<long long*>(P.dbg) + 8 * 64 + 0, g);
    if (blockIdx.x == 0) { P.dbg[8 * 64 + 2] = g; P.dbg[8 * 64 + 3] = clock64(); }
  }
  uint8_t* base = reinterpret_cast<uint8_t*>((reinterpret_cast<uintptr_t>(smem_raw) + 1023) & ~uintptr_t(1023));
  const int warp = threadIdx.x / 32, lane = threadIdx.x % 32;
  const int stage_bytes = (P.ga + P.gb) * kTnBox;
  uint8_t* s_raw = base;
  uint8_t* s_lo = s_raw + kTnStages * stage_bytes;
  uint64_t* bars = reinterpret_cast<uint64_t*>(s_lo + kTnLoStages * stage_bytes);
  uint64_t* raw_full = bars;
  uint64_t* split_full = raw_full + kTnStages;
  uint64_t* empty = split_full + kTnStages;
  uint64_t* lo_empty = empty + kTnStages;
  uint64_t* acc_full = lo_empty + kTnLoStages;
  uint32_t* tmem_slot = reinterpret_cast<uint32_t*>(acc_full + 1);

  if (warp == 0 && lane == 0) {
    for (int i = 0; i < kTnStages; ++i) {
      mb_init(raw_full + i, 1);
      mb_init(split_full + i, kSplitWarps);
      mb_init(empty + i, 1);
    }
    for (int i = 0; i < kTnLoStages; ++i) mb_init(lo_empty + i, 1);
    mb_init(acc_full, 1);
    asm volatile("fence.mbarrier_init.release.cluster;" ::: "memory");
    asm volatile("fence.proxy.async.shared::cta;" ::: "memory");
  }
  if (warp == 14) {
    asm volatile("tcgen05.alloc.cta_group::1.sync.aligned.shared::cta.b32 [%0], %1;" ::"r"(s_u32(tmem_slot)), "r"(kTmemColsG)
                 : "memory");
    asm volatile("tcgen05.relinquish_alloc_permit.cta_group::1.sync.aligned;" ::: "memory");
  }
  asm volatile("tcgen05.fence::before_thread_sync;" ::: "memory");
  __syncthreads();
  asm volatile("tcgen05.fence::after_thread_sync;" ::: "memory");
  const uint32_t tmem_base = *tmem_slot;
  const bool dbg_on = P.dbg != nullptr && blockIdx.x == 0;
  int dbg_n = 0;

  const int prob = blockIdx.x % P.n_prob, slab = blockIdx.x / P.n_prob;
  const CUtensorMap* map_a = &maps.a[prob];
  const CUtensorMap* map_b = &maps.b[prob];
  const CUtensorMap* map_a3 = &maps.a3[prob];
  const CUtensorMap* map_b3 = &maps.b3[prob];
  const CUtensorMap* map_p = &maps.p[prob];
  const int64_t m0 = slab * P.rows_per_cta;
  const int64_t m1 = m0 + P.rows_per_cta < P.M ? m0 + P.rows_per_cta : P.M;
  const int n_kb = m1 > m0 ? (int)((m1 - m0 + kTnRows - 1) / kTnRows) : 0;

  if (warp == 0) {
    if (lane == 0) {
      int stage = 0;
      uint32_t phase = 0;
      for (int kb = 0; kb < n_kb; ++kb) {
        mb_wait(empty + stage, phase ^ 1);
        KGC_DBG(0);
        uint8_t* dst = s_raw + stage * stage_bytes;
        const int row = (int)(m0 + (int64_t)kb * kTnRows);
        if (P.kmajor) {
          mb_expect_tx(raw_full + stage, (uint32_t)(kTileA + P.n_pad * 128));
          tma_2d(dst, map_a, raw_full + stage, row, 0);
          tma_2d(dst + kTileA, map_b, raw_full + stage, row, 0);
          if (++stage == kTnStages) { stage = 0; phase ^= 1; }
          continue;
        }
        mb_expect_tx(raw_full + stage, (uint32_t)stage_bytes);
        if (P.ga_full > 0) tma_3d(dst, map_a3, raw_full + stage, 0, row, 0);
        for (int g = P.ga_full; g < P.ga; ++g) tma_2d(dst + g * kTnBox, map_a, raw_full + stage, g * 32, row);
        if (P.gb_full > 0) tma_3d(dst + P.ga * kTnBox, map_b3, raw_full + stage, 0, row, 0);
        for (int g = P.gb_full; g < P.gb; ++g) tma_2d(dst + (P.ga + g) * kTnBox, map_b, raw_full + stage, g * 32, row);
        if (++stage == kTnStages) { stage = 0; phase ^= 1; }
      }
    }
  } else if (warp >= 2 && warp < 2 + kSplitWarps) {
    const int t = threadIdx.x - 64;
    constexpr int kSplitThreads = kSplitWarps * 32;
    int stage = 0, ls = 0;
    uint32_t phase = 0, lphase = 0;
    const int n_vec = stage_bytes / 16;
    const bool masked = P.keep != nullptr && prob < 2 && !P.kmajor;
    const int brow_t = (t & 255) >> 3;
    const int c16_t = ((((t & 7) >> 1) ^ (brow_t & 3)) << 1) | (t & 1);
    uint32_t nbn[kTnMaxGb];
#pragma unroll
    for (int g = 0; g < kTnMaxGb; ++g) nbn[g] = 0u;
    if (masked && n_kb > 0 && m0 + brow_t < m1) {
      const uint8_t* kp = P.keep + (m0 + brow_t) * P.keep_pitch + c16_t;
#pragma unroll
      for (int g = 0; g < kTnMaxGb; ++g)
        if (g < P.gb) nbn[g] = (uint32_t)__ldg(kp + g * 8);
    }
    for (int kb = 0; kb < n_kb; ++kb) {
      mb_wait(raw_full + stage, phase);
      if (t == 0) KGC_DBG(1);
      mb_wait(lo_empty + ls, lphase ^ 1);
      if (t == 0) KGC_DBG(2);
      uint4* hi = reinterpret_cast<uint4*>(s_raw + stage * stage_bytes);
      uint4* lo = reinterpret_cast<uint4*>(s_lo + ls * stage_bytes);
      const int rows_valid = P.kmajor ? kTnRows : (int)min((int64_t)kTnRows, m1 - (m0 + (int64_t)kb * kTnRows));
      if (masked) {
        uint32_t nbc[kTnMaxGb];
#pragma unroll
        for (int g = 0; g < kTnMaxGb; ++g) nbc[g] = nbn[g];
        if (kb + 1 < n_kb) {
          const uint8_t* kp = P.keep + (m0 + (int64_t)(kb + 1) * kTnRows + brow_t) * P.keep_pitch + c16_t;
          const bool ok = m0 + (int64_t)(kb + 1) * kTnRows + brow_t < m1;
#pragma unroll
          for (int g = 0; g < kTnMaxGb; ++g) nbn[g] = (ok && g < P.gb) ? (uint32_t)__ldg(kp + g * 8) : 0u;
        }
#pragma unroll
        for (int k = 0; k < 4 + kTnMaxGb; ++k) {
          if (k < 4 + P.gb) {
            const int v = t + k * kSplitThreads;
            uint4 x = hi[v];
            if (brow_t >= rows_valid) x = make_uint4(0u, 0u, 0u, 0u);
            else if (k >= 4) {
              uint32_t nb = nbc[k >= 4 ? k - 4 : 0];
              if (prob == 1) nb >>= 4;
              x.x = (nb & 1u) ? __float_as_uint(__uint_as_float(x.x) * P.keep_scale) : 0u;
              x.y = (nb & 2u) ? __float_as_uint(__uint_as_float(x.y) * P.keep_scale) : 0u;
              x.z = (nb & 4u) ? __float_as_uint(__uint_as_float(x.z) * P.keep_scale) : 0u;
              x.w = (nb & 8u) ? __float_as_uint(__uint_as_float(x.w) * P.keep_scale) : 0u;
            }
            uint4 h, l;
            split_tf32(x.x, h.x, l.x);
            split_tf32(x.y, h.y, l.y);
            split_tf32(x.z, h.z, l.z);
            split_tf32(x.w, h.w, l.w);
            hi[v] = h;
            lo[v] = l;
          }
        }
      } else
      for (int v = t; v < n_vec; v += kSplitThreads) {
        uint4 x = hi[v];
        if (((v & 255) >> 3) >= rows_valid) x = make_uint4(0u, 0u, 0u, 0u);
        uint4 h, l;
        split_tf32(x.x, h.x, l.x);
        split_tf32(x.y, h.y, l.y);
        split_tf32(x.z, h.z, l.z);
        split_tf32(x.w, h.w, l.w);
        hi[v] = h;
        lo[v] = l;
      }
      asm volatile("fence.proxy.async.shared::cta;" ::: "memory");
      __syncwarp();
      if (lane == 0) mb_arrive(split_full + stage);
      if (t == 0) KGC_DBG(3);
      if (++stage == kTnStages) { stage = 0; phase ^= 1; }
      if (++ls == kTnLoStages) { ls = 0; lphase ^= 1; }
    }
  } else if (warp == 1) {
    const uint32_t idesc = (1u << 4) | (2u << 7) | (2u << 10) | (1u << 15) | (1u << 16) | ((uint32_t)(P.n_pad >> 3) << 17) |
                           ((uint32_t)(kBM >> 4) << 24);
    int stage = 0, ls = 0;
    uint32_t phase = 0;
    for (int kb = 0; kb < n_kb; ++kb) {
      mb_wait(split_full + stage, phase);
      if (lane == 0) KGC_DBG(4);
      asm volatile("tcgen05.fence::after_thread_sync;" ::: "memory");
      const uint32_t hi_a = s_u32(s_raw + stage * stage_bytes), hi_b = hi_a + P.ga * kTnBox;
      const uint32_t lo_a = s_u32(s_lo + ls * stage_bytes), lo_b = lo_a + P.ga * kTnBox;
      if (P.kmajor) {
        const uint32_t idesc_k = (1u << 4) | (2u << 7) | (2u << 10) | ((uint32_t)(P.n_pad >> 3) << 17) | ((uint32_t)(kBM >> 4) << 24);
        const uint64_t a_hi = sw128_desc(hi_a), a_lo = sw128_desc(lo_a);
        const uint64_t b_hi = sw128_desc(hi_a + kTileA), b_lo = sw128_desc(lo_a + kTileA);
        if (elect_one()) {
          for (int k = 0; k < kTnRows / kUK; ++k) {
            umma_tf32(tmem_base, a_lo + 2 * k, b_hi + 2 * k, idesc_k, (kb | k) != 0 ? 1u : 0u);
            umma_tf32(tmem_base, a_hi + 2 * k, b_lo + 2 * k, idesc_k, 1u);
            umma_tf32(tmem_base, a_hi + 2 * k, b_hi + 2 * k, idesc_k, 1u);
          }
          umma_commit_g(empty + stage);
          umma_commit_g(lo_empty + ls);
          if (kb == n_kb - 1) umma_commit_g(acc_full);
        }
      } else if (elect_one()) {
        for (int k = 0; k < kTnRows / kUK; ++k) {
          const uint32_t off = k * 1024;
          umma_tf32(tmem_base, sw128_mn_desc(lo_a + off), sw128_mn_desc(hi_b + off), idesc, (kb | k) != 0 ? 1u : 0u);
          umma_tf32(tmem_base, sw128_mn_desc(hi_a + off), sw128_mn_desc(lo_b + off), idesc, 1u);
          umma_tf32(tmem_base, sw128_mn_desc(hi_a + off), sw128_mn_desc(hi_b + off), idesc, 1u);
        }
        umma_commit_g(empty + stage);
        umma_commit_g(lo_empty + ls);
        if (kb == n_kb - 1) umma_commit_g(acc_full);
      }
      __syncwarp();
      if (lane == 0) KGC_DBG(5);
      if (++stage == kTnStages) { stage = 0; phase ^= 1; }
      if (++ls == kTnLoStages) ls = 0;
    }
  } else if (warp >= 10 && warp <= 13) {
    const int quarter = warp % 4;
    const int i = quarter * 32 + lane;
    float* out = P.partial + (((int64_t)prob * P.n_slabs + slab) * P.Ka + i) * P.Nb;
    if (n_kb > 0) {
      mb_wait(acc_full, 0);
      if (warp == 10 && lane == 0) KGC_DBG(6);
      asm volatile("tcgen05.fence::after_thread_sync;" ::: "memory");
      const uint32_t taddr = tmem_base + ((uint32_t)(quarter * 32) << 16);
      uint8_t* stg = s_raw + (warp - 10) * (2 * kEpiBuf);
      int buf = 0;
      for (int c0 = 0; c0 < P.n_pad; c0 += 32) {
        uint32_t v[32];
        tmem_ld32_g(taddr + c0, v);
        asm volatile("tcgen05.wait::ld.sync.aligned;" ::: "memory");
        if (lane == 0) asm volatile("cp.async.bulk.wait_group.read 1;" ::: "memory");
        __syncwarp();
        uint8_t* bb = stg + buf * kEpiBuf;
        uint8_t* bx = bb + lane * 128;
        const int sw = lane & 7;
#pragma unroll
        for (int q = 0; q < 8; ++q)
          *reinterpret_cast<uint4*>(bx + ((q ^ sw) << 4)) = make_uint4(v[4 * q], v[4 * q + 1], v[4 * q + 2], v[4 * q + 3]);
        asm volatile("fence.proxy.async.shared::cta;" ::: "memory");
        __syncwarp();
        if (lane == 0) {
          if (c0 < P.Nb && quarter * 32 < P.Ka) tma_store_3d(map_p, bb, c0, quarter * 32, slab);
          asm volatile("cp.async.bulk.commit_group;" ::: "memory");
        }
        buf ^= 1;
      }
      if (lane == 0) asm volatile("cp.async.bulk.wait_group 0;" ::: "memory");
      if (warp == 10 && lane == 0) KGC_DBG(7);
    } else if (i < P.Ka) {
      for (int j = 0; j < P.Nb; ++j) out[j] = 0.f;
    }
  }
  asm volatile("tcgen05.fence::before_thread_sync;" ::: "memory");
  __syncthreads();
  if (P.dbg != nullptr && threadIdx.x == 0) {
    long long g;
    asm volatile("mov.u64 %0, %globaltimer;" : "=l"(g));
    atomicMax(reinterpret_cast<long long*>(P.dbg) + 8 * 64 + 1, g);
    if (blockIdx.x == 0) { P.dbg[8 * 64 + 4] = g; P.dbg[8 * 64 + 5] = clock64(); }
  }
  if (warp == 14) {
    asm volatile("tcgen05.dealloc.cta_group::1.sync.aligned.b32 %0, %1;" ::"r"(tmem_base), "r"(kTmemColsG) : "memory");
  }
}

struct TnOut { float* c[kMaxBatch]; };
__global__ void __launch_bounds__(256)
gemm_tn_partials_reduce(const float* __restrict__ partial_all, int n_parts, int n_elem, const TnOut outs) {
  __shared__ double sm[8][33];
  const float* partial = partial_all + (int64_t)blockIdx.y * n_parts * n_elem;
  float* C = blockIdx.y == 0 ? outs.c[0] : (blockIdx.y == 1 ? outs.c[1] : outs.c[2]);
  const int e = blockIdx.x * 32 + threadIdx.x;
  double s = 0.0;
  if (e < n_elem) {
    int g = threadIdx.y;
    for (; g + 24 < n_parts; g += 32) {
      const float v0 = partial[(int64_t)g * n_elem + e], v1 = partial[(int64_t)(g + 8) * n_elem + e];
      const float v2 = partial[(int64_t)(g + 16) * n_elem + e], v3 = partial[(int64_t)(g + 24) * n_elem + e];
      s += (double)v0; s += (double)v1; s += (double)v2; s += (double)v3;
    }
    for (; g < n_parts; g += 8) s += (double)partial[(int64_t)g * n_elem + e];
  }
  sm[threadIdx.y][threadIdx.x] = s;
  __syncthreads();
  if (threadIdx.y == 0 && e < n_elem) {
    double t = sm[0][threadIdx.x];
#pragma unroll
    for (int k = 1; k < 8; ++k) t += sm[k][threadIdx.x];
    C[e] = (float)t;
  }
}

int make_map_f32_mn(CUtensorMap* map, const void* ptr, int64_t rows, int64_t cols, int64_t pitch) {
  return make_map_f32(map, ptr, rows, cols, pitch, kTnRows, CU_TENSOR_MAP_SWIZZLE_128B_ATOM_32B);
}

}
}

using namespace kgc;

static long long* g_gemm_dbg = nullptr;

extern "C" int kgc_conv_prep(const float* rels, int32_t n_rels, const float* loop_rel, const float* loop_edge, const float* w_in,
                             const float* w_out, const float* w_loop, const float* w_rel, int32_t D, int32_t Dout, float* relp,
                             float* all_rel, float* packed_fwd, float* packed_bwd, void* stream) {
  Tiling tf, tb;
  KGC_REQUIRE(make_tiling(Dout, D, &tf) == 0 && make_tiling(D, Dout, &tb) == 0, "unsupported layer width (<= 256)");
  KGC_REQUIRE(n_rels >= 0 && rels && loop_rel && loop_edge && w_in && w_out && w_loop && w_rel && relp && all_rel && packed_fwd && packed_bwd,
              "null buffer");
  PrepArgs a;
  a.rels = rels; a.loop_rel = loop_rel; a.loop_edge = loop_edge; a.w0 = w_in; a.w1 = w_out; a.w2 = w_loop; a.w_rel = w_rel;
  a.n_rels = n_rels; a.D = D; a.Dout = Dout;
  a.n_pad_f = tf.n_pad; a.k_pad_f = tf.k_pad; a.n_pad_b = tb.n_pad; a.k_pad_b = tb.k_pad;
  a.relp = relp; a.all_rel = all_rel; a.packed_f = packed_fwd; a.packed_b = packed_bwd;
  const int64_t total = (int64_t)(n_rels + 1) * (D + Dout) + 3 * (int64_t)tf.n_pad * tf.k_pad + 4 * (int64_t)tb.n_pad * tb.k_pad;
  conv_prep_kernel<<<(unsigned)ceil_div(total, 256), 256, 0, as_stream(stream)>>>(a);
  KGC_LAUNCH_CHECK();
  return 0;
}

extern "C" int kgc_conv_param_grads(const float* m_loop, const float* w_loop, const float* loop_rel, const float* loop_edge,
                                    const float* relp, const float* w_rel, const float* g_rel, const float* d_relp,
                                    int32_t n_rels, int32_t D, int32_t Dout, float* d_w_loop, float* d_loop_rel,
                                    float* d_loop_edge, float* d_rels, float* d_w_rel, const float* rel_add, void* stream) {
  KGC_REQUIRE(m_loop && w_loop && loop_rel && loop_edge && relp && w_rel && d_relp && d_w_loop && d_loop_rel && d_loop_edge && d_rels && d_w_rel,
              "null buffer");
  ParamGradArgs a;
  a.m_loop = m_loop; a.w_loop = w_loop; a.loop_rel = loop_rel; a.loop_edge = loop_edge; a.relp = relp; a.w_rel = w_rel;
  a.g_rel = g_rel; a.d_relp = d_relp; a.n_rels = n_rels; a.D = D; a.Dout = Dout;
  a.d_w_loop = d_w_loop; a.d_loop_rel = d_loop_rel; a.d_loop_edge = d_loop_edge; a.d_rels = d_rels; a.d_w_rel = d_w_rel;
  if (rel_add != nullptr) {
    KGC_REQUIRE((D * Dout) % 32 == 0, "D * Dout must be a multiple of 32");
    const int64_t total2 = (int64_t)D * Dout + (((int64_t)n_rels * D + 31) & ~31ll) + (int64_t)D * 32;
    conv_param_grads2_kernel<<<(unsigned)ceil_div(total2, 256), 256, 0, as_stream(stream)>>>(a, rel_add);
    KGC_LAUNCH_CHECK();
    return 0;
  }
  const int64_t total = 2 * (int64_t)D * Dout + (int64_t)(n_rels + 1) * D * 32;
  conv_param_grads_kernel<<<(unsigned)ceil_div(total, 256), 256, 0, as_stream(stream)>>>(a);
  KGC_LAUNCH_CHECK();
  return 0;
}

extern "C" size_t kgc_gemm_packed_b_bytes(int32_t N, int32_t K) {
  Tiling t;
  if (make_tiling(N, K, &t)) return 0;
  return (size_t)2 * t.n_pad * t.k_pad * sizeof(float);
}

extern "C" int kgc_gemm_pack_b(const float* B, int64_t stride_k, int64_t stride_n, int32_t N, int32_t K, float* packed,
                               void* stream) {
  Tiling t;
  KGC_REQUIRE(make_tiling(N, K, &t) == 0, "unsupported GEMM shape (K <= 256, N <= 1024)");
  const int total = t.n_pad * t.k_pad;
  pack_b_kernel<<<(total + 255) / 256, 256, 0, as_stream(stream)>>>(B, stride_k, stride_n, N, K, t.n_pad, t.k_pad, packed,
                                                                    packed + total);
  KGC_LAUNCH_CHECK();
  return 0;
}

extern "C" void kgc_gemm_set_debug(long long* buf) { g_gemm_dbg = buf; }

static int launch_gemm_nt(int n_prob, const float* const* A, int64_t M, int32_t K, int64_t lda, const float* const* packed_b,
                          int32_t N, float* const* C, int64_t ldc, const float* row_bias, int32_t act, int32_t trans_c,
                          int32_t trans_a, void* stream, const uint8_t* keep = nullptr, int32_t keep_pitch = 0,
                          float keep_scale = 1.f) {
  Tiling t;
  KGC_REQUIRE(n_prob >= 1 && n_prob <= kMaxBatch, "1..3 problems per launch");
  KGC_REQUIRE(make_tiling(N, K, &t) == 0, "unsupported GEMM shape (K <= 256, N <= 1024)");
  KGC_REQUIRE(M > 0 && lda >= (trans_a ? M : (int64_t)K) && ldc >= (trans_c ? M : (int64_t)N), "bad leading dimensions");
  KGC_REQUIRE(!trans_a || M % 32 == 0, "a transposed A operand needs M % 32 == 0");
  KGC_REQUIRE(ldc % 4 == 0, "C needs a 16-byte row pitch (TMA store)");
  GemmMaps maps;
  const int total = t.n_pad * t.k_pad;
  for (int i = 0; i < kMaxBatch; ++i) {
    const int j = i < n_prob ? i : 0;
    KGC_REQUIRE((reinterpret_cast<uintptr_t>(C[j]) & 15) == 0, "C must be 16-byte aligned (TMA store)");
    if (trans_c) {
      if (make_map_f32(&maps.c[i], C[j], N, M, ldc, 32, CU_TENSOR_MAP_SWIZZLE_128B, 32)) return 1;
      if (make_map_f32(&maps.c16[i], C[j], N, M, ldc, 16, CU_TENSOR_MAP_SWIZZLE_128B, 32)) return 1;
    } else {
      if (make_map_f32(&maps.c[i], C[j], M, N, ldc, 32, CU_TENSOR_MAP_SWIZZLE_128B, 32)) return 1;
      if (make_map_f32(&maps.c16[i], C[j], M, N, ldc, 32, CU_TENSOR_MAP_SWIZZLE_64B, 16)) return 1;
    }
    if (trans_a) {
      if (make_map_f32_groups(&maps.a[i], A[j], K, (int)(M / 32), lda, kBM / 32, CU_TENSOR_MAP_SWIZZLE_128B)) return 1;
    } else if (make_map_f32(&maps.a[i], A[j], M, K, lda, kBM)) {
      return 1;
    }
    if (make_map_f32(&maps.bhi[i], packed_b[j], t.n_pad, t.k_pad, t.k_pad, t.NT)) return 1;
    if (make_map_f32(&maps.blo[i], packed_b[j] + total, t.n_pad, t.k_pad, t.k_pad, t.NT)) return 1;
  }
  GemmParams P;
  P.M = M; P.N = N; P.K = K; P.n_prob = n_prob;
  P.n_kb = t.n_kb; P.ksteps = t.ksteps; P.NT = t.NT; P.n_ntiles = t.n_ntiles;
  P.n_mtiles = (int32_t)ceil_div(M, kBM);
  P.C = C[0]; P.ldc = ldc; P.row_bias = row_bias; P.act = act; P.trans_c = trans_c; P.trans_a = trans_a; P.dbg = g_gemm_dbg;
  KGC_REQUIRE(keep == nullptr || (!trans_a && keep_pitch % 16 == 0 && keep_pitch >= 8 * kMaxKB && (reinterpret_cast<uintptr_t>(keep) & 15) == 0),
              "keep flags: one byte per 4 columns, 16-byte aligned rows of at least 64 bytes");
  P.keep = keep; P.keep_pitch = keep_pitch; P.keep_scale = keep_scale;
  const int tile_b_al = (t.NT * kBK * 4 + 1023) & ~1023;
  const size_t fixed = (size_t)2 * t.n_kb * tile_b_al + kEpiStage + 512 + 1024;
  int stages = (int)((226 * 1024 - fixed) / kTileA);
  if (stages > kMaxStages) stages = kMaxStages;
  KGC_REQUIRE(stages >= 2, "shared-memory plan does not fit");
  P.stages = stages;
  const size_t smem = fixed + (size_t)stages * kTileA;
  static SmemAttrCache attr;
  KGC_CUDA_TRY(attr.ensure(gemm_tf32x3_kernel, smem));
  const int groups = n_prob * t.n_ntiles;
  int per = kNumSMs / groups;
  if (per > P.n_mtiles) per = P.n_mtiles;
  if (per < 1) per = 1;
  gemm_tf32x3_kernel<<<per * groups, kThreadsG, smem, as_stream(stream)>>>(maps, P);
  KGC_LAUNCH_CHECK();
  return 0;
}

extern "C" int kgc_gemm_nt(const float* A, int64_t M, int32_t K, int64_t lda, const float* packed_b, int32_t N, float* C,
                           int64_t ldc, void* stream) {
  return launch_gemm_nt(1, &A, M, K, lda, &packed_b, N, &C, ldc, nullptr, 0, 0, 0, stream);
}

extern "C" int kgc_gemm_nt_batch(int32_t n_prob, const float* const* A, int64_t M, int32_t K, int64_t lda,
                                 const float* const* packed_b, int32_t N, float* const* C, int64_t ldc, void* stream) {
  KGC_REQUIRE(A && packed_b && C, "null pointer table");
  return launch_gemm_nt(n_prob, A, M, K, lda, packed_b, N, C, ldc, nullptr, 0, 0, 0, stream);
}

extern "C" int kgc_gemm_nt_batch_masked(int32_t n_prob, const float* const* A, int64_t M, int32_t K, int64_t lda,
                                        const float* const* packed_b, int32_t N, float* const* C, int64_t ldc,
                                        const uint8_t* keep, int32_t keep_pitch, float keep_scale, void* stream) {
  KGC_REQUIRE(A && packed_b && C, "null pointer table");
  return launch_gemm_nt(n_prob, A, M, K, lda, packed_b, N, C, ldc, nullptr, 0, 0, 0, stream, keep, keep_pitch, keep_scale);
}

extern "C" int kgc_gemm_nt_trans(const float* At, int64_t M, int32_t K, int64_t ldat, const float* packed_b, int32_t N,
                                 float* Ct, int64_t ldct, void* stream) {
  return launch_gemm_nt(1, &At, M, K, ldat, &packed_b, N, &Ct, ldct, nullptr, 0, 1, 1, stream);
}

extern "C" int kgc_score_1n_fwd(const float* ent, int64_t n_ent, int32_t D, int64_t ld_ent, const float* packed_x, int32_t B,
                                const float* bias, float* pred, int64_t ld_pred, void* stream) {
  KGC_REQUIRE(bias != nullptr, "bias is required");
  return launch_gemm_nt(1, &ent, n_ent, D, ld_ent, &packed_x, B, &pred, ld_pred, bias, 1, 1, 0, stream);
}

constexpr int64_t kTnMaxSlabRows = 1024;

static int64_t tn_max_slab_rows() {
  static int64_t rows = 0;
  if (rows == 0) {
    const char* e = getenv("KGC_TN_SLAB_ROWS");
    rows = e != nullptr && atoll(e) >= 64 ? atoll(e) : kTnMaxSlabRows;
  }
  return rows;
}

static int64_t tn_slabs(int64_t M, int n_prob) {
  const int64_t per_wave = kNumSMs / n_prob > 0 ? kNumSMs / n_prob : 1;
  int64_t slabs = ceil_div(M, (int64_t)2 * kTnRows);
  if (slabs > per_wave) slabs = per_wave;
  const int64_t need = ceil_div(M, tn_max_slab_rows());
  if (slabs < need) slabs = ceil_div(need, per_wave) * per_wave;
  return slabs < 1 ? 1 : slabs;
}

extern "C" int kgc_score_1n_fwd_t(const float* ent, int64_t n_ent, int32_t D, int64_t ld_ent, const float* packed_x, int32_t B,
                                  const float* bias, float* pred_t, int64_t ld_t, void* stream) {
  KGC_REQUIRE(bias != nullptr, "bias is required");
  return launch_gemm_nt(1, &ent, n_ent, D, ld_ent, &packed_x, B, &pred_t, ld_t, bias, 1, 0, 0, stream);
}

extern "C" int kgc_score_1n_logits(const float* ent, int64_t n_ent, int32_t D, int64_t ld_ent, const float* packed_x, int32_t B,
                                   const float* bias, float* logits, int64_t ld_logits, void* stream) {
  KGC_REQUIRE(bias != nullptr, "bias is required");
  return launch_gemm_nt(1, &ent, n_ent, D, ld_ent, &packed_x, B, &logits, ld_logits, bias, 0, 1, 0, stream);
}

extern "C" size_t kgc_gemm_tn_tc_workspace_bytes(int64_t M, int32_t Ka, int32_t Nb) {
  int64_t parts = kNumSMs;
  for (int n = 1; n <= kMaxBatch; ++n) {
    const int64_t s = tn_slabs(M > 0 ? M : 1, n) * n;
    if (s > parts) parts = s;
  }
  return (size_t)parts * Ka * Nb * sizeof(float);
}

static int launch_gemm_tn_tc(int n_prob, const float* const* A, int64_t lda, const float* const* B, int64_t ldb, int64_t M,
                             int32_t Ka, int32_t Nb, float* const* C, void* workspace, size_t workspace_bytes, int32_t kmajor,
                             void* stream, const uint8_t* keep = nullptr, int32_t keep_pitch = 0, float keep_scale = 1.f) {
  KGC_REQUIRE(n_prob >= 1 && n_prob <= kMaxBatch, "1..3 problems per launch");
  KGC_REQUIRE(M > 0 && Ka > 0 && Nb > 0 && Ka <= 128 && Nb <= 224, "supported: Ka <= 128, Nb <= 224");
  KGC_REQUIRE(Nb % 4 == 0 && lda % 4 == 0 && ldb % 4 == 0 && (kmajor || Ka % 4 == 0), "dimensions and leading dimensions must be multiples of 4");
  KGC_REQUIRE(workspace && workspace_bytes >= kgc_gemm_tn_tc_workspace_bytes(M, Ka, Nb), "workspace too small");
  GemmTnParams P;
  P.n_pad = (Nb + 15) / 16 * 16;
  P.kmajor = kmajor;
  P.M = M; P.Ka = Ka; P.Nb = Nb; P.n_prob = n_prob;
  P.ga = 4;
  P.gb = (P.n_pad + 31) / 32;
  int slabs = (int)tn_slabs(M, n_prob);
  P.rows_per_cta = ceil_div(ceil_div(M, slabs), kTnRows) * kTnRows;
  slabs = (int)ceil_div(M, P.rows_per_cta);
  P.n_slabs = slabs;
  P.partial = static_cast<float*>(workspace);
  P.dbg = g_gemm_dbg;
  KGC_REQUIRE(keep == nullptr || (!kmajor && keep_pitch >= 8 * P.gb), "keep flags: one byte per 4 columns of B, rows that cover the padded width");
  P.keep = keep; P.keep_pitch = keep_pitch; P.keep_scale = keep_scale;
  P.ga_full = kmajor ? 0 : Ka / 32;
  P.gb_full = kmajor ? 0 : Nb / 32;
  GemmTnMaps maps;
  TnOut outs;
  for (int i = 0; i < kMaxBatch; ++i) {
    const int j = i < n_prob ? i : 0;
    outs.c[i] = C[j];
    if (kmajor) {
      if (make_map_f32(&maps.a[i], A[j], Ka, M, lda, kBM) || make_map_f32(&maps.b[i], B[j], Nb, M, ldb, P.n_pad)) return 1;
    } else if (make_map_f32_mn(&maps.a[i], A[j], M, Ka, lda) || make_map_f32_mn(&maps.b[i], B[j], M, Nb, ldb)) {
      return 1;
    }
    maps.a3[i] = maps.a[i]; maps.b3[i] = maps.b[i];
    if (P.ga_full > 0 && make_map_f32_mn_groups(&maps.a3[i], A[j], M, P.ga_full, lda)) return 1;
    if (P.gb_full > 0 && make_map_f32_mn_groups(&maps.b3[i], B[j], M, P.gb_full, ldb)) return 1;
    if (make_map_f32_parts(&maps.p[i], P.partial + (int64_t)j * slabs * Ka * Nb, slabs, Ka, Nb)) return 1;
  }
  const size_t stage = (size_t)(P.ga + P.gb) * kTnBox;
  const size_t smem = (kTnStages + kTnLoStages) * stage + 512 + 1024;
  KGC_REQUIRE(smem <= 227 * 1024, "shared-memory plan does not fit");
  static SmemAttrCache attr;
  KGC_CUDA_TRY(attr.ensure(gemm_tn_tc_kernel, smem));
  cudaStream_t st = as_stream(stream);
  gemm_tn_tc_kernel<<<slabs * n_prob, kThreadsG, smem, st>>>(maps, P);
  KGC_LAUNCH_CHECK();
  gemm_tn_partials_reduce<<<dim3((Ka * Nb + 31) / 32, n_prob), dim3(32, 8), 0, st>>>(P.partial, slabs, Ka * Nb, outs);
  KGC_LAUNCH_CHECK();
  return 0;
}

extern "C" int kgc_gemm_tn_tc(const float* A, int64_t lda, const float* B, int64_t ldb, int64_t M, int32_t Ka, int32_t Nb,
                              float* C, void* workspace, size_t workspace_bytes, void* stream) {
  return launch_gemm_tn_tc(1, &A, lda, &B, ldb, M, Ka, Nb, &C, workspace, workspace_bytes, 0, stream);
}

extern "C" int kgc_gemm_tn_tc_batch(int32_t n_prob, const float* const* A, int64_t lda, const float* const* B, int64_t ldb,
                                    int64_t M, int32_t Ka, int32_t Nb, float* const* C, void* workspace,
                                    size_t workspace_bytes, void* stream) {
  KGC_REQUIRE(A && B && C, "null pointer table");
  return launch_gemm_tn_tc(n_prob, A, lda, B, ldb, M, Ka, Nb, C, workspace, workspace_bytes, 0, stream);
}

extern "C" int kgc_gemm_tn_tc_batch_masked(int32_t n_prob, const float* const* A, int64_t lda, const float* const* B, int64_t ldb,
                                           int64_t M, int32_t Ka, int32_t Nb, float* const* C, void* workspace,
                                           size_t workspace_bytes, const uint8_t* keep, int32_t keep_pitch, float keep_scale,
                                           void* stream) {
  KGC_REQUIRE(A && B && C, "null pointer table");
  return launch_gemm_tn_tc(n_prob, A, lda, B, ldb, M, Ka, Nb, C, workspace, workspace_bytes, 0, stream, keep, keep_pitch,
                           keep_scale);
}

extern "C" int kgc_gemm_nt_splitk(const float* A, int64_t lda, const float* Bt, int64_t ldb, int64_t K, int32_t Ma, int32_t Nb,
                                  float* C, void* workspace, size_t workspace_bytes, void* stream) {
  return launch_gemm_tn_tc(1, &A, lda, &Bt, ldb, K, Ma, Nb, &C, workspace, workspace_bytes, 1, stream);
}
```

### kgc-gcn_b200/csrc/tail.cu

```cuda
#include "common.cuh"

namespace kgc {
namespace {

constexpr int kThreads = 256;
constexpr int kMaxBlocks = 4 * kNumSMs;

struct Stripe {
  int64_t row_beg, row_end;
};
__device__ __forceinline__ Stripe block_stripe(int64_t n_rows) {
  const int64_t per = (n_rows + gridDim.x - 1) / gridDim.x;
  Stripe s;
  s.row_beg = blockIdx.x * per;
  s.row_end = s.row_beg + per < n_rows ? s.row_beg + per : n_rows;
  return s;
}

__device__ __forceinline__ float4 mask4(const uint8_t* m, int64_t idx4, float s) {
  const uchar4 v = *reinterpret_cast<const uchar4*>(m + idx4 * 4);
  return make_float4(v.x ? s : 0.f, v.y ? s : 0.f, v.z ? s : 0.f, v.w ? s : 0.f);
}

constexpr int kKeepPitch = 64;
__device__ __forceinline__ uint32_t nibble(const float4& m) {
  return (m.x != 0.f ? 1u : 0u) | (m.y != 0.f ? 2u : 0u) | (m.z != 0.f ? 4u : 0u) | (m.w != 0.f ? 8u : 0u);
}

__device__ __forceinline__ float4 keep4(const float4& g, uint32_t nb, float s) {
  return make_float4((nb & 1u) ? g.x * s : 0.f, (nb & 2u) ? g.y * s : 0.f, (nb & 4u) ? g.z * s : 0.f, (nb & 8u) ? g.w * s : 0.f);
}

struct DropCfg {
  const uint8_t* mask_in;
  const uint8_t* mask_out;
  const int64_t* seed;
  uint32_t drop_thr;
  float keep_scale;
};
__device__ __forceinline__ float4 drop_scale4(const DropCfg& d, int plane, int64_t i) {
  const uint8_t* m = plane == 0 ? d.mask_in : d.mask_out;
  if (m != nullptr) return mask4(m, i, d.keep_scale);
  if (d.seed != nullptr) return philox_mask4(i, (uint32_t)plane, (uint64_t)__ldg(d.seed), d.drop_thr, d.keep_scale);
  return make_float4(1.f, 1.f, 1.f, 1.f);
}

__device__ __forceinline__ void block_store_partials(double4 a, double4 b, int rl, int c, int RL, int Do4,
                                                     double* partials, double4* sm) {
  const bool active = rl < RL;
  if (active) {
    sm[(0 * RL + rl) * Do4 + c] = a;
    sm[(1 * RL + rl) * Do4 + c] = b;
  }
  __syncthreads();
  if (active && rl == 0) {
    double4 sa = sm[c], sb = sm[RL * Do4 + c];
    for (int k = 1; k < RL; ++k) {
      const double4 ta = sm[(0 * RL + k) * Do4 + c], tb = sm[(1 * RL + k) * Do4 + c];
      sa.x += ta.x; sa.y += ta.y; sa.z += ta.z; sa.w += ta.w;
      sb.x += tb.x; sb.y += tb.y; sb.z += tb.z; sb.w += tb.w;
    }
    double4* out = reinterpret_cast<double4*>(partials) + (int64_t)blockIdx.x * 2 * Do4;
    out[c] = sa;
    out[Do4 + c] = sb;
  }
}

__global__ void __launch_bounds__(kThreads)
tail_fwd_kernel(const float4* __restrict__ res3, const DropCfg drop, const float4* __restrict__ bias,
                int64_t n_rows, int Do4, float4* __restrict__ pre, double* __restrict__ partials,
                uint8_t* __restrict__ keep) {
  extern __shared__ double4 sm[];
  const int RL = kThreads / Do4;
  const int rl = threadIdx.x / Do4, c = threadIdx.x % Do4;
  const Stripe s = block_stripe(n_rows);
  const int64_t plane = n_rows * (int64_t)Do4;
  double4 sum = make_double4(0, 0, 0, 0), sq = make_double4(0, 0, 0, 0);
  if (rl < RL) {
    const float4 bv = bias ? __ldg(bias + c) : make_float4(0.f, 0.f, 0.f, 0.f);
    for (int64_t r = s.row_beg + rl; r < s.row_end; r += RL) {
      const int64_t i = r * Do4 + c;
      float4 a = __ldg(res3 + i), b = __ldg(res3 + plane + i);
      const float4 l = __ldg(res3 + 2 * plane + i);
      uint32_t kb = 0;
      { const float4 m = drop_scale4(drop, 0, i); a.x *= m.x; a.y *= m.y; a.z *= m.z; a.w *= m.w; kb |= nibble(m); }
      { const float4 m = drop_scale4(drop, 1, i); b.x *= m.x; b.y *= m.y; b.z *= m.z; b.w *= m.w; kb |= nibble(m) << 4; }
      if (keep != nullptr) keep[r * kKeepPitch + c] = (uint8_t)kb;
      float4 o;
      o.x = (a.x + b.x + l.x) / 3.0f + bv.x;
      o.y = (a.y + b.y + l.y) / 3.0f + bv.y;
      o.z = (a.z + b.z + l.z) / 3.0f + bv.z;
      o.w = (a.w + b.w + l.w) / 3.0f + bv.w;
      pre[i] = o;
      sum.x += o.x; sum.y += o.y; sum.z += o.z; sum.w += o.w;
      sq.x += (double)o.x * o.x; sq.y += (double)o.y * o.y; sq.z += (double)o.z * o.z; sq.w += (double)o.w * o.w;
    }
  }
  block_store_partials(sum, sq, rl, c, RL, Do4, partials, sm);
}

constexpr int kFinCols = 2, kFinLanes = 128;

__device__ __forceinline__ void reduce_partials(const double* __restrict__ partials, int64_t n_blocks, int Dout,
                                                int c, int lane, double (*sm)[kFinLanes][kFinCols], double* s_out,
                                                double* q_out) {
  double s = 0, q = 0;
  if (c < Dout) {
    for (int64_t b = lane; b < n_blocks; b += kFinLanes) {
      s += partials[(b * 2 + 0) * Dout + c];
      q += partials[(b * 2 + 1) * Dout + c];
    }
  }
  const int cc = threadIdx.x % kFinCols;
  sm[0][lane][cc] = s;
  sm[1][lane][cc] = q;
  __syncthreads();
  if (lane == 0) {
    s = sm[0][0][cc];
    q = sm[1][0][cc];
    for (int k = 1; k < kFinLanes; ++k) {
      s += sm[0][k][cc];
      q += sm[1][k][cc];
    }
  }
  *s_out = s;
  *q_out = q;
}

__global__ void __launch_bounds__(kFinCols * kFinLanes)
colsum_finalize_kernel(const double* __restrict__ partials, int64_t n_blocks, int Dout, double* __restrict__ sums) {
  __shared__ double sm[2][kFinLanes][kFinCols];
  const int c = blockIdx.x * kFinCols + threadIdx.x % kFinCols, lane = threadIdx.x / kFinCols;
  double s = 0, q = 0;
  reduce_partials(partials, n_blocks, Dout, c, lane, sm, &s, &q);
  if (lane != 0 || c >= Dout) return;
  sums[c] = s;
  sums[Dout + c] = q;
}

__global__ void __launch_bounds__(kFinCols * kFinLanes)
colsum_finalize2_kernel(const double* __restrict__ partials, int64_t n_blocks, int Dout, double* __restrict__ sums,
                        float* __restrict__ sums32) {
  __shared__ double sm[2][kFinLanes][kFinCols];
  const int c = blockIdx.x * kFinCols + threadIdx.x % kFinCols, lane = threadIdx.x / kFinCols;
  double s = 0, q = 0;
  reduce_partials(partials, n_blocks, Dout, c, lane, sm, &s, &q);
  if (lane != 0 || c >= Dout) return;
  sums[c] = s;
  sums[Dout + c] = q;
  sums32[c] = (float)s;
  sums32[Dout + c] = (float)q;
}

__global__ void __launch_bounds__(kFinCols * kFinLanes)
colstats_finalize_kernel(const double* __restrict__ partials, int64_t n_blocks, int64_t n_rows, int Dout, float eps,
                         float momentum, float* __restrict__ rmean, float* __restrict__ rvar,
                         int64_t* __restrict__ n_tracked, double* __restrict__ sums, float* __restrict__ stats) {
  __shared__ double sm[2][kFinLanes][kFinCols];
  const int c = blockIdx.x * kFinCols + threadIdx.x % kFinCols, lane = threadIdx.x / kFinCols;
  double s = 0, q = 0;
  reduce_partials(partials, n_blocks, Dout, c, lane, sm, &s, &q);
  if (blockIdx.x == 0 && threadIdx.x == 0 && n_tracked != nullptr) *n_tracked += 1;
  if (lane != 0 || c >= Dout) return;
  if (sums != nullptr) {
    sums[c] = s;
    sums[Dout + c] = q;
  }
  const double mean = s / (double)n_rows;
  double var = q / (double)n_rows - mean * mean;
  if (var < 0) var = 0;
  const float meanf = (float)mean, varf = (float)var;
  stats[c] = meanf;
  stats[Dout + c] = varf;
  stats[2 * Dout + c] = (float)(1.0 / sqrt(var + (double)eps));
  if (rmean != nullptr && rvar != nullptr) {
    const float unbias = (float)n_rows / (float)(n_rows > 1 ? n_rows - 1 : 1);
    rmean[c] = rmean[c] * (1.f - momentum) + momentum * meanf;
    rvar[c] = rvar[c] * (1.f - momentum) + (momentum * unbias) * varf;
  }
}

__global__ void colstats_from_sums_kernel(const double* __restrict__ sums, int64_t n_rows, int Dout, float eps,
                                          int training, const float* __restrict__ rmean,
                                          const float* __restrict__ rvar, float* __restrict__ stats) {
  const int c = blockIdx.x * blockDim.x + threadIdx.x;
  if (c >= Dout) return;
  double mean, var;
  if (training) {
    mean = sums[c] / (double)n_rows;
    var = sums[Dout + c] / (double)n_rows - mean * mean;
    if (var < 0) var = 0;
  } else {
    mean = rmean[c];
    var = rvar[c];
  }
  stats[c] = (float)mean;
  stats[Dout + c] = (float)var;
  stats[2 * Dout + c] = (float)(1.0 / sqrt(var + (double)eps));
}

struct OutDrop {
  const int64_t* seed;
  uint32_t drop_thr;
  float keep_scale;
  uint8_t* keep;
};

__global__ void __launch_bounds__(kThreads)
tail_apply_kernel(const float4* __restrict__ pre, const float4* __restrict__ stats, const float4* __restrict__ gamma,
                  const float4* __restrict__ beta, int64_t n4, int Do4, float4* __restrict__ all_ent, const OutDrop od) {
  const int64_t i = blockIdx.x * (int64_t)kThreads + threadIdx.x;
  if (i >= n4) return;
  const int c = (int)(i % Do4);
  const float4 v = __ldg(pre + i), m = __ldg(stats + c), rs = __ldg(stats + 2 * Do4 + c);
  const float4 ga = __ldg(gamma + c), be = __ldg(beta + c);
  float4 o;
  o.x = tanhf((v.x - m.x) * rs.x * ga.x + be.x);
  o.y = tanhf((v.y - m.y) * rs.y * ga.y + be.y);
  o.z = tanhf((v.z - m.z) * rs.z * ga.z + be.z);
  o.w = tanhf((v.w - m.w) * rs.w * ga.w + be.w);
  if (od.seed != nullptr) {
    const float4 k = philox_mask4(i, 2u, (uint64_t)__ldg(od.seed), od.drop_thr, od.keep_scale);
    o.x *= k.x; o.y *= k.y; o.z *= k.z; o.w *= k.w;
    od.keep[(i / Do4) * kKeepPitch + c] = (uint8_t)nibble(k);
  }
  all_ent[i] = o;
}

__global__ void __launch_bounds__(kThreads)
tail_bwd_reduce_kernel(const float4* __restrict__ g_ent, const float4* __restrict__ pre, const float4* __restrict__ stats,
                       const float4* __restrict__ gamma, const float4* __restrict__ beta, int64_t n_rows, int Do4,
                       double* __restrict__ partials, const uint8_t* __restrict__ out_keep, float out_scale) {
  extern __shared__ double4 sm[];
  const int RL = kThreads / Do4;
  const int rl = threadIdx.x / Do4, c = threadIdx.x % Do4;
  const Stripe s = block_stripe(n_rows);
  double4 s1 = make_double4(0, 0, 0, 0), s2 = make_double4(0, 0, 0, 0);
  if (rl < RL) {
    const float4 m = __ldg(stats + c), rs = __ldg(stats + 2 * Do4 + c), ga = __ldg(gamma + c), be = __ldg(beta + c);
    for (int64_t r = s.row_beg + rl; r < s.row_end; r += RL) {
      const int64_t i = r * Do4 + c;
      float4 g = __ldg(g_ent + i);
      const float4 v = __ldg(pre + i);
      if (out_keep != nullptr) g = keep4(g, out_keep[r * kKeepPitch + c], out_scale);
      const float4 xh = make_float4((v.x - m.x) * rs.x, (v.y - m.y) * rs.y, (v.z - m.z) * rs.z, (v.w - m.w) * rs.w);
      const float4 t = make_float4(tanhf(xh.x * ga.x + be.x), tanhf(xh.y * ga.y + be.y), tanhf(xh.z * ga.z + be.z),
                                   tanhf(xh.w * ga.w + be.w));
      const float dzx = g.x * (1.f - t.x * t.x), dzy = g.y * (1.f - t.y * t.y);
      const float dzz = g.z * (1.f - t.z * t.z), dzw = g.w * (1.f - t.w * t.w);
      s1.x += dzx; s1.y += dzy; s1.z += dzz; s1.w += dzw;
      s2.x += (double)dzx * xh.x;
      s2.y += (double)dzy * xh.y;
      s2.z += (double)dzz * xh.z;
      s2.w += (double)dzw * xh.w;
    }
  }
  block_store_partials(s1, s2, rl, c, RL, Do4, partials, sm);
}

__global__ void __launch_bounds__(kThreads)
tail_bwd_apply_kernel(const float4* __restrict__ g_ent, const float4* __restrict__ pre, const float4* __restrict__ stats,
                      const float4* __restrict__ gamma, const float4* __restrict__ beta, const double* __restrict__ sums,
                      int training, int64_t n_rows, int64_t n_rows_global, int Do4, float4* __restrict__ d_out,
                      const uint8_t* __restrict__ keep, float keep_scale, float4* __restrict__ d_res2,
                      const uint8_t* __restrict__ out_keep, float out_scale) {
  const int64_t n4 = n_rows * (int64_t)Do4;
  const int64_t i = blockIdx.x * (int64_t)kThreads + threadIdx.x;
  if (i >= n4) return;
  const int c = (int)(i % Do4);
  float4 g = __ldg(g_ent + i);
  const float4 v = __ldg(pre + i);
  if (out_keep != nullptr) g = keep4(g, out_keep[(i / Do4) * kKeepPitch + c], out_scale);
  const float4 m = __ldg(stats + c), rs = __ldg(stats + 2 * Do4 + c), ga = __ldg(gamma + c), be = __ldg(beta + c);
  const float4 xh = make_float4((v.x - m.x) * rs.x, (v.y - m.y) * rs.y, (v.z - m.z) * rs.z, (v.w - m.w) * rs.w);
  const float4 t = make_float4(tanhf(xh.x * ga.x + be.x), tanhf(xh.y * ga.y + be.y), tanhf(xh.z * ga.z + be.z),
                               tanhf(xh.w * ga.w + be.w));
  float4 dz = make_float4(g.x * (1.f - t.x * t.x), g.y * (1.f - t.y * t.y), g.z * (1.f - t.z * t.z),
                          g.w * (1.f - t.w * t.w));
  float4 dp;
  if (training) {
    const float inv_n = 1.0f / (float)n_rows_global;
    const double* sp = sums + 4 * c;
    const double* sq = sums + 4 * (Do4 + c);
    const float4 s1 = make_float4((float)sp[0], (float)sp[1], (float)sp[2], (float)sp[3]);
    const float4 s2 = make_float4((float)sq[0], (float)sq[1], (float)sq[2], (float)sq[3]);
    dp.x = ga.x * rs.x * (dz.x - s1.x * inv_n - xh.x * s2.x * inv_n);
    dp.y = ga.y * rs.y * (dz.y - s1.y * inv_n - xh.y * s2.y * inv_n);
    dp.z = ga.z * rs.z * (dz.z - s1.z * inv_n - xh.z * s2.z * inv_n);
    dp.w = ga.w * rs.w * (dz.w - s1.w * inv_n - xh.w * s2.w * inv_n);
  } else {
    dp = make_float4(ga.x * rs.x * dz.x, ga.y * rs.y * dz.y, ga.z * rs.z * dz.z, ga.w * rs.w * dz.w);
  }
  const float4 third = make_float4(dp.x / 3.0f, dp.y / 3.0f, dp.z / 3.0f, dp.w / 3.0f);
  d_out[i] = third;
  if (d_res2 != nullptr) {
    const uint32_t kb = keep != nullptr ? keep[(i / Do4) * kKeepPitch + c] : 0xFFu;
    const float s = keep != nullptr ? keep_scale : 1.f;
    d_res2[i] = make_float4((kb & 1u) ? third.x * s : 0.f, (kb & 2u) ? third.y * s : 0.f, (kb & 4u) ? third.z * s : 0.f,
                            (kb & 8u) ? third.w * s : 0.f);
    d_res2[n4 + i] = make_float4((kb & 16u) ? third.x * s : 0.f, (kb & 32u) ? third.y * s : 0.f, (kb & 64u) ? third.z * s : 0.f,
                                 (kb & 128u) ? third.w * s : 0.f);
  }
}

inline int check_dout(int32_t Dout) { return (Dout <= 0 || Dout % 4 != 0 || Dout > 1024) ? 1 : 0; }
inline size_t partial_smem(int Do4) { return size_t(2) * (kThreads / Do4) * Do4 * sizeof(double4); }

}
}

using namespace kgc;

extern "C" int64_t kgc_tail_num_blocks(int64_t n_rows) {
  int64_t nb = ceil_div(n_rows > 0 ? n_rows : 1, 32);
  return nb < kMaxBlocks ? nb : kMaxBlocks;
}

static DropCfg make_drop(const uint8_t* mask_in, const uint8_t* mask_out, const int64_t* seed, float drop_p, float keep_scale) {
  DropCfg d;
  d.mask_in = mask_in;
  d.mask_out = mask_out;
  d.seed = (seed != nullptr && drop_p > 0.f) ? seed : nullptr;
  const double thr = (double)drop_p * 4294967296.0;
  d.drop_thr = thr >= 4294967295.0 ? 0xFFFFFFFFu : (uint32_t)thr;
  d.keep_scale = keep_scale;
  return d;
}

__global__ void dropout_mask_kernel(const int64_t* __restrict__ seed, uint32_t plane, uint32_t drop_thr, int64_t n4,
                                    uchar4* __restrict__ out) {
  const int64_t i = blockIdx.x * (int64_t)blockDim.x + threadIdx.x;
  if (i >= n4) return;
  const float4 m = philox_mask4(i, plane, (uint64_t)__ldg(seed), drop_thr, 1.0f);
  out[i] = make_uchar4(m.x != 0.f, m.y != 0.f, m.z != 0.f, m.w != 0.f);
}

extern "C" int kgc_dropout_mask(const int64_t* seed, int32_t plane, float drop_p, int64_t n_elem, uint8_t* mask, void* stream) {
  KGC_REQUIRE(seed != nullptr && n_elem % 4 == 0 && plane >= 0, "bad arguments");
  const DropCfg d = make_drop(nullptr, nullptr, seed, drop_p, 1.0f);
  const int64_t n4 = n_elem / 4;
  if (n4 == 0) return 0;
  dropout_mask_kernel<<<(unsigned)ceil_div(n4, kThreads), kThreads, 0, as_stream(stream)>>>(seed, (uint32_t)plane, d.drop_thr,
                                                                                     n4, (uchar4*)mask);
  KGC_LAUNCH_CHECK();
  return 0;
}

extern "C" int32_t kgc_keep_pitch() { return kKeepPitch; }

extern "C" int kgc_tail_fwd(const float* res3, const uint8_t* mask_in, const uint8_t* mask_out, const int64_t* seed,
                            float drop_p, float keep_scale, const float* bias, int64_t n_rows, int32_t Dout, float* pre,
                            double* partials, uint8_t* keep, void* stream) {
  KGC_REQUIRE(check_dout(Dout) == 0, "Dout must be a multiple of 4 and <= 1024");
  KGC_REQUIRE(keep == nullptr || Dout <= 4 * kKeepPitch, "packed keep flags need Dout <= 256");
  KGC_REQUIRE(n_rows > 0, "n_rows must be positive");
  const int Do4 = Dout / 4;
  const size_t smem = partial_smem(Do4);
  tail_fwd_kernel<<<(unsigned)kgc_tail_num_blocks(n_rows), kThreads, smem, as_stream(stream)>>>(
      (const float4*)res3, make_drop(mask_in, mask_out, seed, drop_p, keep_scale), (const float4*)bias, n_rows, Do4,
      (float4*)pre, partials, keep);
  KGC_LAUNCH_CHECK();
  return 0;
}

extern "C" int kgc_colsum_finalize(const double* partials, int64_t n_blocks, int32_t Dout, double* sums, void* stream) {
  KGC_REQUIRE(check_dout(Dout) == 0, "Dout must be a multiple of 4 and <= 1024");
  colsum_finalize_kernel<<<(unsigned)ceil_div(Dout, kFinCols), kFinCols * kFinLanes, 0, as_stream(stream)>>>(
      partials, n_blocks, Dout, sums);
  KGC_LAUNCH_CHECK();
  return 0;
}

extern "C" int kgc_colsum_finalize2(const double* partials, int64_t n_blocks, int32_t Dout, double* sums, float* sums32,
                                    void* stream) {
  KGC_REQUIRE(check_dout(Dout) == 0, "Dout must be a multiple of 4 and <= 1024");
  KGC_REQUIRE(partials && sums && sums32 && n_blocks > 0, "null buffer");
  colsum_finalize2_kernel<<<(unsigned)ceil_div(Dout, kFinCols), kFinCols * kFinLanes, 0, as_stream(stream)>>>(
      partials, n_blocks, Dout, sums, sums32);
  KGC_LAUNCH_CHECK();
  return 0;
}

extern "C" int kgc_colstats_finalize(const double* partials, int64_t n_blocks, int64_t n_rows, int32_t Dout, float eps,
                                     float momentum, float* running_mean, float* running_var,
                                     int64_t* num_batches_tracked, double* sums, float* stats, void* stream) {
  KGC_REQUIRE(check_dout(Dout) == 0, "Dout must be a multiple of 4 and <= 1024");
  KGC_REQUIRE(partials && stats && n_blocks > 0 && n_rows > 0, "null buffer");
  KGC_REQUIRE((running_mean == nullptr) == (running_var == nullptr), "running_mean and running_var come together");
  colstats_finalize_kernel<<<(unsigned)ceil_div(Dout, kFinCols), kFinCols * kFinLanes, 0, as_stream(stream)>>>(
      partials, n_blocks, n_rows, Dout, eps, momentum, running_mean, running_var, num_batches_tracked, sums, stats);
  KGC_LAUNCH_CHECK();
  return 0;
}

extern "C" int kgc_colstats_from_sums(const double* sums, int64_t n_rows, int32_t Dout, float eps, int32_t training,
                                      const float* running_mean, const float* running_var, float* stats, void* stream) {
  KGC_REQUIRE(check_dout(Dout) == 0, "Dout must be a multiple of 4 and <= 1024");
  KGC_REQUIRE(training || (running_mean && running_var), "eval mode needs running statistics");
  KGC_REQUIRE(!training || sums, "training mode needs the column sums");
  colstats_from_sums_kernel<<<(unsigned)ceil_div(Dout, 128), 128, 0, as_stream(stream)>>>(
      sums, n_rows, Dout, eps, training, running_mean, running_var, stats);
  KGC_LAUNCH_CHECK();
  return 0;
}

extern "C" int kgc_tail_apply(const float* pre, const float* stats, const float* gamma, const float* beta,
                              int64_t n_rows, int32_t Dout, float* all_ent, const int64_t* out_seed, float out_drop_p,
                              uint8_t* out_keep, void* stream) {
  KGC_REQUIRE(check_dout(Dout) == 0, "Dout must be a multiple of 4 and <= 1024");
  const int Do4 = Dout / 4;
  const int64_t n4 = n_rows * Do4;
  OutDrop od;
  od.seed = (out_seed != nullptr && out_drop_p > 0.f) ? out_seed : nullptr;
  KGC_REQUIRE(od.seed == nullptr || (out_keep != nullptr && Dout <= 4 * kKeepPitch && out_drop_p < 1.f),
              "output dropout needs a keep-flag buffer, Dout <= 256 and p < 1");
  const DropCfg d = make_drop(nullptr, nullptr, out_seed, out_drop_p, 1.f);
  od.drop_thr = d.drop_thr;
  od.keep_scale = 1.f / (1.f - out_drop_p);
  od.keep = out_keep;
  tail_apply_kernel<<<(unsigned)ceil_div(n4, kThreads), kThreads, 0, as_stream(stream)>>>(
      (const float4*)pre, (const float4*)stats, (const float4*)gamma, (const float4*)beta, n4, Do4, (float4*)all_ent, od);
  KGC_LAUNCH_CHECK();
  return 0;
}

extern "C" int kgc_tail_bwd_reduce(const float* g_ent, const float* pre, const float* stats, const float* gamma,
                                   const float* beta, int64_t n_rows, int32_t Dout, double* partials, const uint8_t* out_keep,
                                   float out_scale, void* stream) {
  KGC_REQUIRE(check_dout(Dout) == 0, "Dout must be a multiple of 4 and <= 1024");
  const int Do4 = Dout / 4;
  const size_t smem = partial_smem(Do4);
  tail_bwd_reduce_kernel<<<(unsigned)kgc_tail_num_blocks(n_rows), kThreads, smem, as_stream(stream)>>>(
      (const float4*)g_ent, (const float4*)pre, (const float4*)stats, (const float4*)gamma, (const float4*)beta, n_rows, Do4,
      partials, out_keep, out_scale);
  KGC_LAUNCH_CHECK();
  return 0;
}

extern "C" int kgc_tail_bwd_apply(const float* g_ent, const float* pre, const float* stats, const float* gamma,
                                  const float* beta, const double* sums, int32_t training, int64_t n_rows,
                                  int64_t n_rows_global, int32_t Dout, float* d_out, const uint8_t* keep, float keep_scale,
                                  float* d_res2, const uint8_t* out_keep, float out_scale, void* stream) {
  KGC_REQUIRE(check_dout(Dout) == 0, "Dout must be a multiple of 4 and <= 1024");
  const int Do4 = Dout / 4;
  const int64_t n4 = n_rows * Do4;
  tail_bwd_apply_kernel<<<(unsigned)ceil_div(n4, kThreads), kThreads, 0, as_stream(stream)>>>(
      (const float4*)g_ent, (const float4*)pre, (const float4*)stats, (const float4*)gamma, (const float4*)beta, sums,
      training, n_rows, n_rows_global, Do4, (float4*)d_out, keep, keep_scale, (float4*)d_res2, out_keep, out_scale);
  KGC_LAUNCH_CHECK();
  return 0;
}
```

Before: 879.3 million.

## Fuse forward GEMM batch with dropout/bias/colstat tail via 3-CTA clusters

Adds a templated variant of the tf32x3 tcgen05 GEMM kernel. Each of the three problem CTAs in a 3-CTA cluster computes one product, and the partial tiles are exchanged through distributed shared memory (st.async, mbarriers). The epilogue applies the dropout keep masks, sums the three results, adds the bias and writes pre along with column-sum partials directly. This removes the res3 intermediate (3×M×Dout write plus read) and the separate tail_fwd pass. Keep flags are precomputed on the side stream in a new kernel. The cost is cluster launch constraints, fewer owner CTAs per n-tile, and extra cross-CTA synchronisation.

```diff
diff --git a/diag_fwd_tail.py b/diag_fwd_tail.py
--- /dev/null
+++ b/diag_fwd_tail.py
@@ -0,0 +1,74 @@
+import importlib, os, sys
+import torch
+sys.path.insert(0, os.path.dirname(os.path.abspath(__file__)))
+import kgc_gcn_b200 as k
+conv = importlib.import_module('kgc_gcn_b200.conv')
+L = k._lib
+p, st = L.ptr, L.stream
+D, Dout = 100, 200
+for M in (4594485, 40943, 14541):
+    print('M', M, 'owners', L.lib().kgc_gemm_nt_fwd_tail_blocks(M, D, Dout), flush=True)
+M = int(sys.argv[1]) if len(sys.argv) > 1 else 4594485
+a = [torch.randn(M, D, device='cuda') for _ in range(3)]
+w = [torch.randn(D, Dout, device='cuda') / 10 for _ in range(3)]
+packed = [conv._pack_b(x) for x in w]
+seed = torch.tensor([123], dtype=torch.int64, device='cuda')
+keep = torch.empty((M, 64), dtype=torch.uint8, device='cuda')
+nb = int(L.lib().kgc_gemm_nt_fwd_tail_blocks(M, D, Dout))
+pre = torch.empty(M, Dout, device='cuda')
+part = torch.empty(nb, 2, Dout, dtype=torch.float64, device='cuda')
+res3 = torch.empty(3, M, Dout, device='cuda')
+nbt = int(L.lib().kgc_tail_num_blocks(M))
+part_t = torch.empty(nbt, 2, Dout, dtype=torch.float64, device='cuda')
+sc = 1 / 0.7
+
+
+def flags():
+    L.call('kgc_keep_flags', None, None, p(seed), 0.3, sc, M, Dout, p(keep), st())
+
+
+def fused():
+    conv.fwd_tail(a, packed, keep, sc, None, pre, part)
+
+
+def fused_nomask():
+    conv.fwd_tail(a, packed, None, 1.0, None, pre, part)
+
+
+def gemm():
+    conv.gemm_nt_batch(a, packed, [res3[0], res3[1], res3[2]])
+
+
+def tail():
+    L.call('kgc_tail_fwd', p(res3), None, None, p(seed), 0.3, sc, None, M, Dout, p(pre), p(part_t), p(keep), st())
+
+
+def tm(f, n=10):
+    for _ in range(3):
+        f()
+    e0, e1 = torch.cuda.Event(enable_timing=True), torch.cuda.Event(enable_timing=True)
+    e0.record()
+    for _ in range(n):
+        f()
+    e1.record()
+    torch.cuda.synchronize()
+    return e0.elapsed_time(e1) / n
+
+
+for name, f in (('keep_flags', flags), ('fused', fused), ('fused_nomask', fused_nomask), ('gemm_batch', gemm), ('tail_fwd', tail)):
+    print('%-14s %.3f ms' % (name, tm(f)), flush=True)
+
+dbg = torch.zeros(9 * 64, dtype=torch.int64, device='cuda')
+dbg[8 * 64] = 1 << 62
+L.lib().kgc_gemm_set_debug(L.ptr(dbg))
+fused()
+torch.cuda.synchronize()
+L.lib().kgc_gemm_set_debug(None)
+d = dbg.cpu().view(9, 64)
+env = d[8]
+print('envelope us', (int(env[1]) - int(env[0])) / 1e3, 'cta0 clk', int(env[5]) - int(env[3]))
+t0 = int(d[:8][d[:8] > 0].min())
+names = ['tma_issue', 'split_raw_ready', 'split_lo_free', 'split_done', 'mma_split_ready', 'mma_issued', 'epi_acc_ready', 'epi_done']
+for r, n in enumerate(names):
+    v = [int(x) - t0 for x in d[r] if int(x) > 0]
+    print('%-16s' % n, v[:40])
diff --git a/include/kgc_b200.h b/include/kgc_b200.h
--- a/include/kgc_b200.h
+++ b/include/kgc_b200.h
@@ -62,6 +62,8 @@
 int kgc_tail_fwd(const float* res3, const uint8_t* mask_in, const uint8_t* mask_out, const int64_t* seed, float drop_p,
                  float keep_scale, const float* bias, int64_t n_rows, int32_t Dout, float* pre, double* partials,
                  uint8_t* keep, void* stream);
+int kgc_keep_flags(const uint8_t* mask_in, const uint8_t* mask_out, const int64_t* seed, float drop_p, float keep_scale,
+                   int64_t n_rows, int32_t Dout, uint8_t* keep, void* stream);
 int kgc_colsum_finalize(const double* partials, int64_t n_blocks, int32_t Dout, double* sums, void* stream);
 int kgc_colstats_from_sums(const double* sums, int64_t n_rows, int32_t Dout, float eps, int32_t training,
                            const float* running_mean, const float* running_var, float* stats, void* stream);
@@ -99,6 +101,10 @@
 int kgc_gemm_nt_batch_masked(int32_t n_prob, const float* const* A, int64_t M, int32_t K, int64_t lda,
                              const float* const* packed_b, int32_t N, float* const* C, int64_t ldc, const uint8_t* keep,
                              int32_t keep_pitch, float keep_scale, void* stream);
+int64_t kgc_gemm_nt_fwd_tail_blocks(int64_t M, int32_t K, int32_t N);
+int kgc_gemm_nt_fwd_tail(const float* const* A, int64_t M, int32_t K, int64_t lda, const float* const* packed_b, int32_t N,
+                         const uint8_t* keep, int32_t keep_pitch, float keep_scale, const float* bias, float* pre,
+                         int64_t ldc, double* partials, int64_t n_blocks, void* stream);
 int kgc_gemm_nt_trans(const float* At, int64_t M, int32_t K, int64_t ldat, const float* packed_b, int32_t N,
                       float* Ct, int64_t ldct, void* stream);
 void kgc_gemm_set_debug(long long* buf);
diff --git a/kgc-gcn_b200/_lib.py b/kgc-gcn_b200/_lib.py
--- a/kgc-gcn_b200/_lib.py
+++ b/kgc-gcn_b200/_lib.py
@@ -27,6 +27,7 @@
     'kgc_dropout_mask': (ctypes.c_int, [_vp, _i32, _f32, _i64, _vp, _vp]),
     'kgc_keep_pitch': (_i32, []),
     'kgc_tail_fwd': (ctypes.c_int, [_vp, _vp, _vp, _vp, _f32, _f32, _vp, _i64, _i32, _vp, _vp, _vp, _vp]),
+    'kgc_keep_flags': (ctypes.c_int, [_vp, _vp, _vp, _f32, _f32, _i64, _i32, _vp, _vp]),
     'kgc_colsum_finalize': (ctypes.c_int, [_vp, _i64, _i32, _vp, _vp]),
     'kgc_colstats_from_sums': (ctypes.c_int, [_vp, _i64, _i32, _f32, _i32, _vp, _vp, _vp, _vp]),
     'kgc_colstats_finalize': (ctypes.c_int, [_vp, _i64, _i64, _i32, _f32, _f32, _vp, _vp, _vp, _vp, _vp, _vp]),
@@ -41,6 +42,8 @@
     'kgc_conv_param_grads': (ctypes.c_int, [_vp] * 8 + [_i32, _i32, _i32] + [_vp] * 7),
     'kgc_gemm_nt_batch': (ctypes.c_int, [_i32, _vp, _i64, _i32, _i64, _vp, _i32, _vp, _i64, _vp]),
     'kgc_gemm_nt_batch_masked': (ctypes.c_int, [_i32, _vp, _i64, _i32, _i64, _vp, _i32, _vp, _i64, _vp, _i32, _f32, _vp]),
+    'kgc_gemm_nt_fwd_tail_blocks': (_i64, [_i64, _i32, _i32]),
+    'kgc_gemm_nt_fwd_tail': (ctypes.c_int, [_vp, _i64, _i32, _i64, _vp, _i32, _vp, _i32, _f32, _vp, _vp, _i64, _vp, _i64, _vp]),
     'kgc_gemm_tn_tc_batch_masked': (ctypes.c_int, [_i32, _vp, _i64, _vp, _i64, _i64, _i32, _i32, _vp, _vp, _sz, _vp, _i32, _f32, _vp]),
     'kgc_gemm_nt_trans': (ctypes.c_int, [_vp, _i64, _i32, _i64, _vp, _i32, _vp, _i64, _vp]),
     'kgc_gemm_nt_splitk': (ctypes.c_int, [_vp, _i64, _vp, _i64, _i64, _i32, _i32, _vp, _vp, _sz, _vp]),
diff --git a/kgc-gcn_b200/conv.py b/kgc-gcn_b200/conv.py
--- a/kgc-gcn_b200/conv.py
+++ b/kgc-gcn_b200/conv.py
@@ -113,6 +113,32 @@
     p = _lib.ptr
     _lib.call('kgc_gemm_nt_splitk', p(a), a.stride(0), p(bt), bt.stride(0), K, Ma, Nb, p(out), p(ws), nbytes, _lib.stream())
     return out
+
+
+def fwd_tail_fused(n_rows, D, Dout):
+    mode = os.environ.get('KGC_FWD_TAIL', '')
+    if mode == '0':
+        return False
+    supported = Dout % 4 == 0 and Dout <= 4 * int(_lib.lib().kgc_keep_pitch()) and D % 4 == 0 and \
+        int(_lib.lib().kgc_gemm_nt_fwd_tail_blocks(n_rows, D, Dout)) > 0
+    if mode == '1' and not supported:
+        raise ValueError('KGC_FWD_TAIL=1: the fused forward tail does not support {} x {} -> {}'.format(n_rows, D, Dout))
+    return supported
+
+
+def fwd_tail(a_list, packed_f, keep, keep_scale, bias, pre, partials):
+    import ctypes
+    M, K = a_list[0].shape
+    N = pre.shape[1]
+    lda = a_list[0].stride(0)
+    if any(a.shape != (M, K) or a.stride() != (lda, 1) for a in a_list) or not pre.is_contiguous():
+        raise ValueError('fwd_tail needs operands of identical shape and strides and a contiguous pre')
+    p = _lib.ptr
+    arr = lambda ts: (ctypes.c_void_p * 3)(*[t.data_ptr() for t in ts])
+    _lib.call('kgc_gemm_nt_fwd_tail', arr(a_list), M, K, lda, arr([packed_f[0], packed_f[1], packed_f[2]]), N, p(keep),
+              keep.stride(0) if keep is not None else 0, float(keep_scale), p(bias), p(pre), pre.stride(0), p(partials),
+              partials.shape[0], _lib.stream())
+    return pre
 
 
 class _LinearFn(torch.autograd.Function):
@@ -286,11 +312,17 @@
         packed_f = torch.empty((3, nf), dtype=torch.float32, device=x.device)
         packed_b = torch.empty((4, nbk), dtype=torch.float32, device=x.device)
         rels_c, wts = rels.detach().contiguous(), [w.detach().contiguous() for w in (w_in, w_out, w_loop, w_rel)]
+        dropping = (mask_in is not None or seed is not None) and drop_p > 0.0
+        keep = torch.empty((Nl, int(_lib.lib().kgc_keep_pitch())), dtype=torch.uint8, device=x.device) if dropping else None
+        fused = coll is None and fwd_tail_fused(Nl, D, Dout)
         main, side = torch.cuda.current_stream(), plan.side_stream()
         side.wait_stream(main)
         with torch.cuda.stream(side):
             _lib.call('kgc_conv_prep', p(rels_c), T - 1, p(loop_rel.detach()), p(loop_edge.detach()), p(wts[0]), p(wts[1]),
                       p(wts[2]), p(wts[3]), D, Dout, p(relp), p(all_rel_pad), p(packed_f), p(packed_b), st())
+            if fused and dropping:
+                _lib.call('kgc_keep_flags', p(mask_in), p(mask_out), p(seed), float(drop_p), float(keep_scale), Nl, Dout,
+                          p(keep), st())
         gather = None
         if coll is None:
             x_full = x
@@ -307,7 +339,7 @@
             x_full, gather = coll.all_gather_rows(x if Nb == Nl else torch.cat([x, x.new_zeros((Nb - Nl, D))], 0),
                                                   async_op=True)
 
-        res3 = plan.scratch('res3', (3, Nl, Dout))
+        res3 = None if fused else plan.scratch('res3', (3, Nl, Dout))
         if gather is not None:
             main.wait_stream(side)
             gemm_nt(x, None, res3[2], packed=packed_f[2])
@@ -325,22 +357,24 @@
 
         if hybrid:
             coll.p2p.reduce_agg(agg)
-        if gather is not None:
-            coll.sum_hub_rows(agg, n_loc)
-            gemm_nt_batch([agg[0, :Nl], agg[1, :Nl]], [packed_f[0], packed_f[1]], [res3[0], res3[1]])
+        pre = torch.empty((Nl, Dout), dtype=torch.float32, device=x.device)
+        if fused:
+            nb = int(_lib.lib().kgc_gemm_nt_fwd_tail_blocks(Nl, D, Dout))
+            partials = plan.scratch('colpart_f', (nb, 2, Dout), torch.float64)
+            fwd_tail([agg[0], agg[1], x], packed_f, keep, keep_scale, bias, pre, partials)
         else:
-            gemm_nt_batch([agg[0], agg[1], x], [packed_f[0], packed_f[1], packed_f[2]], [res3[0], res3[1], res3[2]])
-
-        nb = int(_lib.lib().kgc_tail_num_blocks(Nl))
-        partials = plan.scratch('colpart', (nb, 2, Dout), torch.float64)
+            if gather is not None:
+                coll.sum_hub_rows(agg, n_loc)
+                gemm_nt_batch([agg[0, :Nl], agg[1, :Nl]], [packed_f[0], packed_f[1]], [res3[0], res3[1]])
+            else:
+                gemm_nt_batch([agg[0], agg[1], x], [packed_f[0], packed_f[1], packed_f[2]], [res3[0], res3[1], res3[2]])
+            nb = int(_lib.lib().kgc_tail_num_blocks(Nl))
+            partials = plan.scratch('colpart', (nb, 2, Dout), torch.float64)
+            _lib.call('kgc_tail_fwd', p(res3), p(mask_in), p(mask_out), p(seed), float(drop_p), float(keep_scale), p(bias),
+                      Nl, Dout, p(pre), p(partials), p(keep), st())
         sums = torch.empty((2, Dout), dtype=torch.float64, device=x.device)
-        pre = torch.empty((Nl, Dout), dtype=torch.float32, device=x.device)
         stats = torch.empty((3, Dout), dtype=torch.float32, device=x.device)
         all_ent = torch.empty((Nl, Dout), dtype=torch.float32, device=x.device)
-        dropping = (mask_in is not None or seed is not None) and drop_p > 0.0
-        keep = torch.empty((Nl, int(_lib.lib().kgc_keep_pitch())), dtype=torch.uint8, device=x.device) if dropping else None
-        _lib.call('kgc_tail_fwd', p(res3), p(mask_in), p(mask_out), p(seed), float(drop_p), float(keep_scale), p(bias),
-                  Nl, Dout, p(pre), p(partials), p(keep), st())
         if training and coll is None:
             mom, nbt = bn_track if bn_track is not None else (0.0, None)
             _lib.call('kgc_colstats_finalize', p(partials), nb, n_global, Dout, float(eps), float(mom),
diff --git a/kgc-gcn_b200/csrc/gemm_tf32x3.cu b/kgc-gcn_b200/csrc/gemm_tf32x3.cu
--- a/kgc-gcn_b200/csrc/gemm_tf32x3.cu
+++ b/kgc-gcn_b200/csrc/gemm_tf32x3.cu
@@ -1,6 +1,7 @@
 #include <cuda.h>
 
 #include <cstdlib>
+#include <type_traits>
 #include "common.cuh"
 
 namespace kgc {
@@ -129,6 +130,22 @@
         "=r"(v[17]), "=r"(v[18]), "=r"(v[19]), "=r"(v[20]), "=r"(v[21]), "=r"(v[22]), "=r"(v[23]), "=r"(v[24]),
         "=r"(v[25]), "=r"(v[26]), "=r"(v[27]), "=r"(v[28]), "=r"(v[29]), "=r"(v[30]), "=r"(v[31])
       : "r"(taddr));
+}
+__device__ __forceinline__ uint32_t mapa_u32(uint32_t smem_addr, uint32_t rank) {
+  uint32_t r;
+  asm volatile("mapa.shared::cluster.u32 %0, %1, %2;" : "=r"(r) : "r"(smem_addr), "r"(rank));
+  return r;
+}
+__device__ __forceinline__ void st_async_v4(uint32_t cluster_addr, uint32_t a, uint32_t b, uint32_t c, uint32_t d, uint32_t cluster_bar) {
+  asm volatile("st.async.shared::cluster.mbarrier::complete_tx::bytes.v4.b32 [%0], {%1, %2, %3, %4}, [%5];" ::"r"(cluster_addr),
+               "r"(a), "r"(b), "r"(c), "r"(d), "r"(cluster_bar)
+               : "memory");
+}
+__device__ __forceinline__ void mb_arrive_peer(uint32_t cluster_addr) {
+  asm volatile("mbarrier.arrive.shared::cluster.b64 _, [%0];" ::"r"(cluster_addr) : "memory");
+}
+__device__ __forceinline__ void cluster_sync_all() {
+  asm volatile("barrier.cluster.arrive.release.aligned;\n\tbarrier.cluster.wait.acquire.aligned;" ::: "memory");
 }
 __device__ __forceinline__ uint64_t sw128_desc(uint32_t smem_addr) {
   uint64_t d = 0;
@@ -161,8 +178,19 @@
   long long* dbg;
 };
 
+constexpr int kFwdTailBlk = 4;
+constexpr int kFwdTailRecv = kEpiStage;
+struct FwdTailArgs {
+  const uint8_t* keep;
+  int32_t keep_pitch;
+  float keep_scale;
+  const float* bias;
+  double* partials;
+};
+
+template <bool kFwdTail>
 __global__ void __launch_bounds__(kThreadsG, 1)
-gemm_tf32x3_kernel(const __grid_constant__ GemmMaps maps, const GemmParams P) {
+gemm_tf32x3_kernel(const __grid_constant__ GemmMaps maps, const GemmParams P, const FwdTailArgs T) {
   extern __shared__ uint8_t smem_raw[];
   if (P.dbg != nullptr && threadIdx.x == 0) {
     long long g;
@@ -179,7 +207,8 @@
   const int kStages = P.stages;
   uint8_t* s_a = s_blo + P.n_kb * tile_b_al;
   uint8_t* s_stage = s_a + kStages * kTileA;
-  uint64_t* bars = reinterpret_cast<uint64_t*>(s_stage + kEpiStage);
+  uint8_t* s_recv = s_stage + kEpiStage;
+  uint64_t* bars = reinterpret_cast<uint64_t*>(s_stage + kEpiStage + (kFwdTail ? kFwdTailRecv : 0));
   uint64_t* b_full = bars;
   uint64_t* raw_full = bars + 1;
   uint64_t* raw_empty = raw_full + kMaxStages;
@@ -188,6 +217,8 @@
   uint64_t* acc_full = split_empty + kAStages;
   uint64_t* acc_empty = acc_full + 2;
   uint32_t* tmem_slot = reinterpret_cast<uint32_t*>(acc_empty + 2);
+  uint64_t* x_full = acc_empty + 3;
+  uint64_t* x_empty = x_full + 4 * 2;
 
   if (warp == 0 && lane == 0) {
     mb_init(b_full, 1);
@@ -203,8 +234,17 @@
       mb_init(acc_full + i, 1);
       mb_init(acc_empty + i, 4);
     }
+    if constexpr (kFwdTail) {
+      for (int i = 0; i < 4 * 2; ++i) {
+        mb_init(x_full + i, 1);
+        mb_init(x_empty + i, 1);
+      }
+    }
     asm volatile("fence.mbarrier_init.release.cluster;" ::: "memory");
     asm volatile("fence.proxy.async.shared::cta;" ::: "memory");
+    if constexpr (kFwdTail) {
+      for (int i = 0; i < 4 * 2; ++i) mb_expect_tx(x_full + i, kEpiBuf);
+    }
   }
   if (warp == 14) {
     asm volatile("tcgen05.alloc.cta_group::1.sync.aligned.shared::cta.b32 [%0], %1;" ::"r"(s_u32(tmem_slot)), "r"(kTmemColsTS)
@@ -214,15 +254,16 @@
   asm volatile("tcgen05.fence::before_thread_sync;" ::: "memory");
   __syncthreads();
   asm volatile("tcgen05.fence::after_thread_sync;" ::: "memory");
+  if constexpr (kFwdTail) cluster_sync_all();
   const uint32_t tmem_base = *tmem_slot;
   const uint32_t tmem_a = tmem_base + kAccCols;
   const bool dbg_on = P.dbg != nullptr && blockIdx.x == 0;
   int dbg_n = 0;
 #define KGC_DBG(role) do { if (dbg_on && dbg_n < 64) P.dbg[(role) * 64 + dbg_n++] = clock64(); } while (0)
 
-  const int groups = P.n_prob * P.n_ntiles;
-  const int prob = (blockIdx.x % groups) / P.n_ntiles;
-  const int nt = blockIdx.x % P.n_ntiles;
+  const int groups = kFwdTail ? 3 * P.n_ntiles : P.n_prob * P.n_ntiles;
+  const int prob = kFwdTail ? blockIdx.x % 3 : (blockIdx.x % groups) / P.n_ntiles;
+  const int nt = kFwdTail ? (blockIdx.x / 3) % P.n_ntiles : blockIdx.x % P.n_ntiles;
   const int first = blockIdx.x / groups;
   const int step = gridDim.x / groups;
   const CUtensorMap* map_a = &maps.a[prob];
@@ -256,7 +297,7 @@
     const int r = quarter * 32 + lane;
     int stage = 0, ts = 0;
     uint32_t phase = 0, tphase = 0;
-    const bool masked = P.keep != nullptr && prob < 2 && !P.trans_a;
+    const bool masked = !kFwdTail && P.keep != nullptr && prob < 2 && !P.trans_a;
     uint32_t kcur[kMaxKB], knxt[kMaxKB];
 #pragma unroll
     for (int j = 0; j < kMaxKB; ++j) kcur[j] = knxt[j] = 0u;
@@ -377,75 +418,262 @@
       }
     }
   } else if (warp >= 10 && warp <= 13) {
-    const int quarter = warp % 4;
-    uint8_t* stg = s_stage + (warp - 10) * (2 * kEpiBuf);
-    const int64_t row_q = quarter * 32;
-    int acc = 0, buf = 0;
-    uint32_t acc_phase = 0;
-    for (int mt = first; mt < P.n_mtiles; mt += step) {
-      mb_wait(acc_full + acc, acc_phase);
-      if (warp == 10 && lane == 0) KGC_DBG(6);
-      asm volatile("tcgen05.fence::after_thread_sync;" ::: "memory");
-      const int64_t m0 = (int64_t)mt * kBM + row_q;
-      const uint32_t taddr = tmem_base + ((uint32_t)(quarter * 32) << 16) + acc * (kAccCols / 2);
-      for (int c0 = 0; c0 < P.NT; c0 += 32) {
-        uint32_t v[32];
-        tmem_ld32_g(taddr + c0, v);
-        asm volatile("tcgen05.wait::ld.sync.aligned;" ::: "memory");
-        if (c0 + 32 >= P.NT) {
-          asm volatile("tcgen05.fence::before_thread_sync;" ::: "memory");
+    if constexpr (kFwdTail) {
+      const int quarter = warp % 4;
+      uint8_t* stg = s_stage + (warp - 10) * (2 * kEpiBuf);
+      uint8_t* rcv = s_recv + (warp - 10) * (2 * kEpiBuf);
+      const int64_t row_q = quarter * 32;
+      const int sw = lane & 7;
+      auto epilogue = [&](auto rank) {
+        constexpr int R = decltype(rank)::value;
+        const bool masked = R < 2 && T.keep != nullptr;
+        const int kbyte0 = nt * P.NT / 4;
+        uint32_t kcur[2 * kFwdTailBlk], knxt[2 * kFwdTailBlk];
+        auto load_keep = [&](int mt_, uint32_t (&w)[2 * kFwdTailBlk]) {
+          const int64_t grow = (int64_t)mt_ * kBM + row_q + lane;
+          const bool ok = masked && mt_ < P.n_mtiles && grow < P.M;
+          const uint32_t* kp = reinterpret_cast<const uint32_t*>(T.keep + (ok ? grow : 0) * T.keep_pitch + kbyte0);
+#pragma unroll
+          for (int j = 0; j < 2 * kFwdTailBlk; ++j)
+            w[j] = (ok && 16 * j < P.NT && kbyte0 + 4 * j + 4 <= T.keep_pitch) ? (__ldg(kp + j) >> (R == 1 ? 4 : 0)) : 0u;
+        };
+        load_keep(first, knxt);
+        double csum[kFwdTailBlk], csq[kFwdTailBlk];
+#pragma unroll
+        for (int b = 0; b < kFwdTailBlk; ++b) csum[b] = csq[b] = 0.0;
+        int acc = 0, buf = 0;
+        uint32_t acc_phase = 0, xphase = 0;
+        for (int mt = first; mt < P.n_mtiles; mt += step) {
+#pragma unroll
+          for (int j = 0; j < 2 * kFwdTailBlk; ++j) kcur[j] = knxt[j];
+          load_keep(mt + step, knxt);
+          mb_wait(acc_full + acc, acc_phase);
+          if (warp == 10 && lane == 0) KGC_DBG(6);
+          asm volatile("tcgen05.fence::after_thread_sync;" ::: "memory");
+          const int64_t m0 = (int64_t)mt * kBM + row_q;
+          const int rows = P.M - m0 < 32 ? (int)(P.M - m0) : 32;
+          const uint32_t taddr = tmem_base + ((uint32_t)(quarter * 32) << 16) + acc * (kAccCols / 2);
+#pragma unroll 1
+          for (int b = 0; 32 * b < P.NT; ++b) {
+            {
+              const int c0 = 32 * b;
+              const int col = nt * P.NT + c0;
+              const bool wide = c0 + 32 <= P.NT;
+              uint32_t v[32];
+              tmem_ld32_g(taddr + c0, v);
+              asm volatile("tcgen05.wait::ld.sync.aligned;" ::: "memory");
+              if (32 * b + 32 >= P.NT) {
+                asm volatile("tcgen05.fence::before_thread_sync;" ::: "memory");
+                __syncwarp();
+                if (lane == 0) mb_arrive(acc_empty + acc);
+              }
+              if (masked) {
+                uint32_t kw[2] = {kcur[0], kcur[1]};
+#pragma unroll
+                for (int i = 1; i < kFwdTailBlk; ++i)
+                  if (b == i) { kw[0] = kcur[2 * i]; kw[1] = kcur[2 * i + 1]; }
+#pragma unroll
+                for (int j = 0; j < 32; ++j) {
+                  const uint32_t w = kw[j / 16];
+                  const float m = ((w >> (8 * ((j % 16) / 4) + j % 4)) & 1u) ? T.keep_scale : 0.f;
+                  v[j] = __float_as_uint(__uint_as_float(v[j]) * m);
+                }
+              }
+              if constexpr (R > 0) {
+                const float bl = (R == 2 && T.bias != nullptr && col + lane < P.N) ? __ldg(T.bias + col + lane) : 0.f;
+                mb_wait(x_full + quarter * 2 + buf, xphase);
+                const uint8_t* rx = rcv + buf * kEpiBuf + lane * 128;
+#pragma unroll
+                for (int q = 0; q < 8; ++q) {
+                  if (q < 4 || wide) {
+                    const uint4 u = *reinterpret_cast<const uint4*>(rx + ((q ^ sw) << 4));
+                    const float uv[4] = {__uint_as_float(u.x), __uint_as_float(u.y), __uint_as_float(u.z), __uint_as_float(u.w)};
+#pragma unroll
+                    for (int e = 0; e < 4; ++e) {
+                      const int j = 4 * q + e;
+                      const float s = uv[e] + __uint_as_float(v[j]);
+                      if constexpr (R == 1) {
+                        v[j] = __float_as_uint(s);
+                      } else {
+                        const float bias_j = T.bias != nullptr ? __shfl_sync(0xFFFFFFFFu, bl, j) : 0.f;
+                        v[j] = __float_as_uint(s / 3.0f + bias_j);
+                      }
+                    }
+                  }
+                }
+                __syncwarp();
+                if (lane == 0) {
+                  mb_expect_tx(x_full + quarter * 2 + buf, kEpiBuf);
+                  mb_arrive_peer(mapa_u32(s_u32(x_empty + quarter * 2 + buf), (uint32_t)(R - 1)));
+                }
+              }
+              if constexpr (R < 2) {
+                mb_wait(x_empty + quarter * 2 + buf, xphase ^ 1);
+                const uint32_t dst = mapa_u32(s_u32(rcv + buf * kEpiBuf + lane * 128), (uint32_t)(R + 1));
+                const uint32_t bar = mapa_u32(s_u32(x_full + quarter * 2 + buf), (uint32_t)(R + 1));
+#pragma unroll
+                for (int q = 0; q < 8; ++q) st_async_v4(dst + ((q ^ sw) << 4), v[4 * q], v[4 * q + 1], v[4 * q + 2], v[4 * q + 3], bar);
+              } else {
+                if (lane == 0) asm volatile("cp.async.bulk.wait_group.read 1;" ::: "memory");
+                __syncwarp();
+                uint8_t* bb = stg + buf * kEpiBuf;
+                if (wide) {
+                  uint8_t* bx = bb + lane * 128;
+#pragma unroll
+                  for (int q = 0; q < 8; ++q)
+                    *reinterpret_cast<uint4*>(bx + ((q ^ sw) << 4)) = make_uint4(v[4 * q], v[4 * q + 1], v[4 * q + 2], v[4 * q + 3]);
+                } else {
+                  uint8_t* bx = bb + lane * 64;
+                  const int sw64 = (lane >> 1) & 3;
+#pragma unroll
+                  for (int q = 0; q < 4; ++q)
+                    *reinterpret_cast<uint4*>(bx + ((q ^ sw64) << 4)) = make_uint4(v[4 * q], v[4 * q + 1], v[4 * q + 2], v[4 * q + 3]);
+                }
+                asm volatile("fence.proxy.async.shared::cta;" ::: "memory");
+                __syncwarp();
+                if (lane == 0) {
+                  if (m0 < P.M && col < P.N) tma_store_2d(wide ? map_c : map_c16, bb, col, (int)m0);
+                  asm volatile("cp.async.bulk.commit_group;" ::: "memory");
+                }
+                if (wide || lane < 16) {
+                  double s = csum[0], sq = csq[0];
+#pragma unroll
+                  for (int i = 1; i < kFwdTailBlk; ++i)
+                    if (b == i) { s = csum[i]; sq = csq[i]; }
+#pragma unroll
+                  for (int r = 0; r < 32; ++r) {
+                    if (r < rows) {
+                      const int off = wide ? r * 128 + ((((lane >> 2) ^ (r & 7)) << 4) | ((lane & 3) << 2))
+                                           : r * 64 + ((((lane >> 2) ^ ((r >> 1) & 3)) << 4) | ((lane & 3) << 2));
+                      const float o = *reinterpret_cast<const float*>(bb + off);
+                      s += o;
+                      sq += (double)o * o;
+                    }
+                  }
+#pragma unroll
+                  for (int i = 0; i < kFwdTailBlk; ++i)
+                    if (b == i) { csum[i] = s; csq[i] = sq; }
+                }
+              }
+              buf ^= 1;
+              if (buf == 0) xphase ^= 1;
+            }
+          }
+          if (warp == 10 && lane == 0) KGC_DBG(7);
+          if (++acc == 2) { acc = 0; acc_phase ^= 1; }
+        }
+        if constexpr (R == 2) {
+          if (lane == 0) asm volatile("cp.async.bulk.wait_group 0;" ::: "memory");
           __syncwarp();
-          if (lane == 0) mb_arrive(acc_empty + acc);
-        }
-        if (lane == 0) asm volatile("cp.async.bulk.wait_group.read 1;" ::: "memory");
-        __syncwarp();
-        uint8_t* bb = stg + buf * kEpiBuf;
-        const bool wide = c0 + 32 <= P.NT;
-        if (P.row_bias != nullptr) {
-          const float bv = m0 + lane < P.M ? P.row_bias[m0 + lane] : 0.f;
-#pragma unroll
-          for (int j = 0; j < 32; ++j) {
-            const float z = __uint_as_float(v[j]) + bv;
-            v[j] = __float_as_uint(P.act == 1 ? 1.f / (1.f + expf(-z)) : z);
+          double* red = reinterpret_cast<double*>(stg);
+#pragma unroll
+          for (int b = 0; b < kFwdTailBlk; ++b) {
+            red[(b * 2 + 0) * 32 + lane] = csum[b];
+            red[(b * 2 + 1) * 32 + lane] = csq[b];
+          }
+          asm volatile("bar.sync 1, 128;" ::: "memory");
+          if (warp == 10) {
+            for (int b = 0; 32 * b < P.NT; ++b) {
+              const int cc = 32 * b + lane, col = nt * P.NT + cc;
+              double s = 0.0, sq = 0.0;
+#pragma unroll
+              for (int w = 0; w < 4; ++w) {
+                const double* rw = reinterpret_cast<const double*>(stg + w * (2 * kEpiBuf));
+                s += rw[(b * 2 + 0) * 32 + lane];
+                sq += rw[(b * 2 + 1) * 32 + lane];
+              }
+              if (cc < P.NT && col < P.N) {
+                T.partials[((int64_t)first * 2 + 0) * P.N + col] = s;
+                T.partials[((int64_t)first * 2 + 1) * P.N + col] = sq;
+              }
+            }
           }
         }
-        if (P.trans_c) {
-#pragma unroll
-          for (int j = 0; j < 32; ++j)
-            *reinterpret_cast<uint32_t*>(bb + j * 128 + ((((lane >> 2) ^ (j & 7)) << 4) | ((lane & 3) << 2))) = v[j];
-        } else if (wide) {
-          uint8_t* bx = bb + lane * 128;
-          const int sw = lane & 7;
-#pragma unroll
-          for (int q = 0; q < 8; ++q)
-            *reinterpret_cast<uint4*>(bx + ((q ^ sw) << 4)) = make_uint4(v[4 * q], v[4 * q + 1], v[4 * q + 2], v[4 * q + 3]);
-        } else {
-          uint8_t* bx = bb + lane * 64;
-          const int sw = (lane >> 1) & 3;
-#pragma unroll
-          for (int q = 0; q < 4; ++q)
-            *reinterpret_cast<uint4*>(bx + ((q ^ sw) << 4)) = make_uint4(v[4 * q], v[4 * q + 1], v[4 * q + 2], v[4 * q + 3]);
+      };
+      if (prob == 0) epilogue(std::integral_constant<int, 0>());
+      else if (prob == 1) epilogue(std::integral_constant<int, 1>());
+      else epilogue(std::integral_constant<int, 2>());
+    } else {
+      const int quarter = warp % 4;
+      uint8_t* stg = s_stage + (warp - 10) * (2 * kEpiBuf);
+      const int64_t row_q = quarter * 32;
+      int acc = 0, buf = 0;
+      uint32_t acc_phase = 0;
+      for (int mt = first; mt < P.n_mtiles; mt += step) {
+        mb_wait(acc_full + acc, acc_phase);
+        if (warp == 10 && lane == 0) KGC_DBG(6);
+        asm volatile("tcgen05.fence::after_thread_sync;" ::: "memory");
+        const int64_t m0 = (int64_t)mt * kBM + row_q;
+        const uint32_t taddr = tmem_base + ((uint32_t)(quarter * 32) << 16) + acc * (kAccCols / 2);
+        for (int c0 = 0; c0 < P.NT; c0 += 32) {
+          uint32_t v[32];
+          tmem_ld32_g(taddr + c0, v);
+          asm volatile("tcgen05.wait::ld.sync.aligned;" ::: "memory");
+          if (c0 + 32 >= P.NT) {
+            asm volatile("tcgen05.fence::before_thread_sync;" ::: "memory");
+            __syncwarp();
+            if (lane == 0) mb_arrive(acc_empty + acc);
+          }
+          if (lane == 0) asm volatile("cp.async.bulk.wait_group.read 1;" ::: "memory");
+          __syncwarp();
+          uint8_t* bb = stg + buf * kEpiBuf;
+          const bool wide = c0 + 32 <= P.NT;
+          if (P.row_bias != nullptr) {
+            const float bv = m0 + lane < P.M ? P.row_bias[m0 + lane] : 0.f;
+#pragma unroll
+            for (int j = 0; j < 32; ++j) {
+              const float z = __uint_as_float(v[j]) + bv;
+              v[j] = __float_as_uint(P.act == 1 ? 1.f / (1.f + expf(-z)) : z);
+            }
+          }
+          if (P.trans_c) {
+#pragma unroll
+            for (int j = 0; j < 32; ++j)
+              *reinterpret_cast<uint32_t*>(bb + j * 128 + ((((lane >> 2) ^ (j & 7)) << 4) | ((lane & 3) << 2))) = v[j];
+          } else if (wide) {
+            uint8_t* bx = bb + lane * 128;
+            const int sw = lane & 7;
+#pragma unroll
+            for (int q = 0; q < 8; ++q)
+              *reinterpret_cast<uint4*>(bx + ((q ^ sw) << 4)) = make_uint4(v[4 * q], v[4 * q + 1], v[4 * q + 2], v[4 * q + 3]);
+          } else {
+            uint8_t* bx = bb + lane * 64;
+            const int sw = (lane >> 1) & 3;
+#pragma unroll
+            for (int q = 0; q < 4; ++q)
+              *reinterpret_cast<uint4*>(bx + ((q ^ sw) << 4)) = make_uint4(v[4 * q], v[4 * q + 1], v[4 * q + 2], v[4 * q + 3]);
+          }
+          asm volatile("fence.proxy.async.shared::cta;" ::: "memory");
+          __syncwarp();
+          if (lane == 0) {
+            const int col = nt * P.NT + c0;
+            if (m0 < P.M && col < P.N) {
+              if (P.trans_c) tma_store_2d(wide ? map_c : map_c16, bb, (int)m0, col);
+              else tma_store_2d(wide ? map_c : map_c16, bb, col, (int)m0);
+            }
+            asm volatile("cp.async.bulk.commit_group;" ::: "memory");
+          }
+          buf ^= 1;
         }
-        asm volatile("fence.proxy.async.shared::cta;" ::: "memory");
-        __syncwarp();
-        if (lane == 0) {
-          const int col = nt * P.NT + c0;
-          if (m0 < P.M && col < P.N) {
-            if (P.trans_c) tma_store_2d(wide ? map_c : map_c16, bb, (int)m0, col);
-            else tma_store_2d(wide ? map_c : map_c16, bb, col, (int)m0);
-          }
-          asm volatile("cp.async.bulk.commit_group;" ::: "memory");
-        }
-        buf ^= 1;
+        if (warp == 10 && lane == 0) KGC_DBG(7);
+        if (++acc == 2) { acc = 0; acc_phase ^= 1; }
       }
-      if (warp == 10 && lane == 0) KGC_DBG(7);
-      if (++acc == 2) { acc = 0; acc_phase ^= 1; }
-    }
-    if (lane == 0) asm volatile("cp.async.bulk.wait_group 0;" ::: "memory");
+      if (lane == 0) asm volatile("cp.async.bulk.wait_group 0;" ::: "memory");
+    }
   }
   asm volatile("tcgen05.fence::before_thread_sync;" ::: "memory");
   __syncthreads();
-  if (P.dbg != nullptr && threadIdx.x == 0) {
+  if constexpr (kFwdTail) {
+    cluster_sync_all();
+    long long* dbg = P.dbg;
+    asm volatile("" : "+l"(dbg));
+    if (dbg != nullptr && threadIdx.x == 0) {
+      long long g;
+      asm volatile("mov.u64 %0, %globaltimer;" : "=l"(g));
+      atomicMax(dbg + 8 * 64 + 1, g);
+      if (blockIdx.x == 0) { dbg[8 * 64 + 4] = g; dbg[8 * 64 + 5] = clock64(); }
+    }
+  } else if (P.dbg != nullptr && threadIdx.x == 0) {
     long long g;
     asm volatile("mov.u64 %0, %globaltimer;" : "=l"(g));
     atomicMax(reinterpret_cast<long long*>(P.dbg) + 8 * 64 + 1, g);
@@ -1118,13 +1346,53 @@
   P.stages = stages;
   const size_t smem = fixed + (size_t)stages * kTileA;
   static SmemAttrCache attr;
-  KGC_CUDA_TRY(attr.ensure(gemm_tf32x3_kernel, smem));
+  KGC_CUDA_TRY(attr.ensure(gemm_tf32x3_kernel<false>, smem));
   const int groups = n_prob * t.n_ntiles;
   int per = kNumSMs / groups;
   if (per > P.n_mtiles) per = P.n_mtiles;
   if (per < 1) per = 1;
-  gemm_tf32x3_kernel<<<per * groups, kThreadsG, smem, as_stream(stream)>>>(maps, P);
+  gemm_tf32x3_kernel<false><<<per * groups, kThreadsG, smem, as_stream(stream)>>>(maps, P, FwdTailArgs{});
   KGC_LAUNCH_CHECK();
+  return 0;
+}
+
+struct FwdTailPlan {
+  Tiling t;
+  int stages, owners;
+  size_t smem;
+};
+static int fwd_tail_plan(int64_t M, int32_t K, int32_t N, FwdTailPlan* pl) {
+  KGC_REQUIRE(M > 0 && make_tiling(N, K, &pl->t) == 0 && pl->t.NT <= 32 * kFwdTailBlk, "unsupported fused tail shape (K <= 256, N <= 1024)");
+  const int tile_b_al = (pl->t.NT * kBK * 4 + 1023) & ~1023;
+  const size_t fixed = (size_t)2 * pl->t.n_kb * tile_b_al + kEpiStage + kFwdTailRecv + 512 + 1024;
+  pl->stages = (int)((226 * 1024 - fixed) / kTileA);
+  if (pl->stages > kMaxStages) pl->stages = kMaxStages;
+  KGC_REQUIRE(pl->stages >= 2, "shared-memory plan does not fit");
+  pl->smem = fixed + (size_t)pl->stages * kTileA;
+  static SmemAttrCache attr;
+  KGC_CUDA_TRY(attr.ensure(gemm_tf32x3_kernel<true>, pl->smem));
+  static int clusters[64] = {0};
+  int dev = 0;
+  KGC_CUDA_TRY(cudaGetDevice(&dev));
+  int n_cl = dev >= 0 && dev < 64 ? clusters[dev] : 0;
+  if (n_cl == 0) {
+    cudaLaunchConfig_t cfg = {};
+    cudaLaunchAttribute at[1];
+    at[0].id = cudaLaunchAttributeClusterDimension;
+    at[0].val.clusterDim.x = 3; at[0].val.clusterDim.y = 1; at[0].val.clusterDim.z = 1;
+    cfg.gridDim = dim3(3 * (kNumSMs / 3), 1, 1);
+    cfg.blockDim = dim3(kThreadsG, 1, 1);
+    cfg.dynamicSmemBytes = pl->smem;
+    cfg.attrs = at;
+    cfg.numAttrs = 1;
+    KGC_CUDA_TRY(cudaOccupancyMaxActiveClusters(&n_cl, gemm_tf32x3_kernel<true>, &cfg));
+    KGC_REQUIRE(n_cl >= pl->t.n_ntiles, "too few resident 3-CTA clusters for the fused tail");
+    if (dev >= 0 && dev < 64) clusters[dev] = n_cl;
+  }
+  int per = n_cl / pl->t.n_ntiles;
+  const int64_t n_mtiles = ceil_div(M, kBM);
+  if (per > n_mtiles) per = (int)n_mtiles;
+  pl->owners = per;
   return 0;
 }
 
@@ -1144,6 +1412,56 @@
                                         const uint8_t* keep, int32_t keep_pitch, float keep_scale, void* stream) {
   KGC_REQUIRE(A && packed_b && C, "null pointer table");
   return launch_gemm_nt(n_prob, A, M, K, lda, packed_b, N, C, ldc, nullptr, 0, 0, 0, stream, keep, keep_pitch, keep_scale);
+}
+
+extern "C" int64_t kgc_gemm_nt_fwd_tail_blocks(int64_t M, int32_t K, int32_t N) {
+  FwdTailPlan pl;
+  if (fwd_tail_plan(M, K, N, &pl)) return 0;
+  return pl.owners;
+}
+
+extern "C" int kgc_gemm_nt_fwd_tail(const float* const* A, int64_t M, int32_t K, int64_t lda, const float* const* packed_b,
+                                    int32_t N, const uint8_t* keep, int32_t keep_pitch, float keep_scale, const float* bias,
+                                    float* pre, int64_t ldc, double* partials, int64_t n_blocks, void* stream) {
+  KGC_REQUIRE(A && packed_b && pre && partials, "null pointer");
+  FwdTailPlan pl;
+  if (fwd_tail_plan(M, K, N, &pl)) return 1;
+  KGC_REQUIRE(n_blocks == pl.owners, "partials must have kgc_gemm_nt_fwd_tail_blocks(M, K, N) rows");
+  KGC_REQUIRE(lda >= K && ldc >= N && ldc % 4 == 0 && (reinterpret_cast<uintptr_t>(pre) & 15) == 0,
+              "bad leading dimensions (pre: 16-byte aligned rows, TMA store)");
+  KGC_REQUIRE(keep == nullptr || (keep_pitch % 4 == 0 && (reinterpret_cast<uintptr_t>(keep) & 3) == 0 && 4 * keep_pitch >= N),
+              "keep flags: one byte per 4 columns, 4-byte aligned rows");
+  const Tiling& t = pl.t;
+  GemmMaps maps;
+  const int total = t.n_pad * t.k_pad;
+  for (int i = 0; i < kMaxBatch; ++i) {
+    if (make_map_f32(&maps.c[i], pre, M, N, ldc, 32, CU_TENSOR_MAP_SWIZZLE_128B, 32)) return 1;
+    if (make_map_f32(&maps.c16[i], pre, M, N, ldc, 32, CU_TENSOR_MAP_SWIZZLE_64B, 16)) return 1;
+    if (make_map_f32(&maps.a[i], A[i], M, K, lda, kBM)) return 1;
+    if (make_map_f32(&maps.bhi[i], packed_b[i], t.n_pad, t.k_pad, t.k_pad, t.NT)) return 1;
+    if (make_map_f32(&maps.blo[i], packed_b[i] + total, t.n_pad, t.k_pad, t.k_pad, t.NT)) return 1;
+  }
+  GemmParams P = {};
+  P.M = M; P.N = N; P.K = K; P.n_prob = kMaxBatch;
+  P.n_kb = t.n_kb; P.ksteps = t.ksteps; P.NT = t.NT; P.n_ntiles = t.n_ntiles;
+  P.n_mtiles = (int32_t)ceil_div(M, kBM);
+  P.stages = pl.stages;
+  P.C = pre; P.ldc = ldc; P.dbg = g_gemm_dbg;
+  FwdTailArgs T;
+  T.keep = keep; T.keep_pitch = keep_pitch; T.keep_scale = keep_scale; T.bias = bias; T.partials = partials;
+  cudaLaunchConfig_t cfg = {};
+  cudaLaunchAttribute at[1];
+  at[0].id = cudaLaunchAttributeClusterDimension;
+  at[0].val.clusterDim.x = 3; at[0].val.clusterDim.y = 1; at[0].val.clusterDim.z = 1;
+  cfg.gridDim = dim3((unsigned)(3 * t.n_ntiles * pl.owners), 1, 1);
+  cfg.blockDim = dim3(kThreadsG, 1, 1);
+  cfg.dynamicSmemBytes = pl.smem;
+  cfg.stream = as_stream(stream);
+  cfg.attrs = at;
+  cfg.numAttrs = 1;
+  KGC_CUDA_TRY(cudaLaunchKernelEx(&cfg, gemm_tf32x3_kernel<true>, maps, P, T));
+  KGC_LAUNCH_CHECK();
+  return 0;
 }
 
 extern "C" int kgc_gemm_nt_trans(const float* At, int64_t M, int32_t K, int64_t ldat, const float* packed_b, int32_t N,
diff --git a/kgc-gcn_b200/csrc/tail.cu b/kgc-gcn_b200/csrc/tail.cu
--- a/kgc-gcn_b200/csrc/tail.cu
+++ b/kgc-gcn_b200/csrc/tail.cu
@@ -346,7 +346,27 @@
   return 0;
 }
 
+__global__ void __launch_bounds__(kThreads)
+keep_flags_kernel(const DropCfg drop, int64_t n4, int Do4, uint8_t* __restrict__ keep) {
+  const int64_t i = blockIdx.x * (int64_t)kThreads + threadIdx.x;
+  if (i >= n4) return;
+  const uint32_t kb = nibble(drop_scale4(drop, 0, i)) | (nibble(drop_scale4(drop, 1, i)) << 4);
+  keep[(i / Do4) * kKeepPitch + i % Do4] = (uint8_t)kb;
+}
+
 extern "C" int32_t kgc_keep_pitch() { return kKeepPitch; }
+
+extern "C" int kgc_keep_flags(const uint8_t* mask_in, const uint8_t* mask_out, const int64_t* seed, float drop_p,
+                              float keep_scale, int64_t n_rows, int32_t Dout, uint8_t* keep, void* stream) {
+  KGC_REQUIRE(check_dout(Dout) == 0 && Dout <= 4 * kKeepPitch, "packed keep flags need Dout % 4 == 0 and Dout <= 256");
+  KGC_REQUIRE(keep != nullptr && n_rows > 0 && (mask_in == nullptr) == (mask_out == nullptr), "bad arguments");
+  const int Do4 = Dout / 4;
+  const int64_t n4 = n_rows * Do4;
+  keep_flags_kernel<<<(unsigned)ceil_div(n4, kThreads), kThreads, 0, as_stream(stream)>>>(
+      make_drop(mask_in, mask_out, seed, drop_p, keep_scale), n4, Do4, keep);
+  KGC_LAUNCH_CHECK();
+  return 0;
+}
 
 extern "C" int kgc_tail_fwd(const float* res3, const uint8_t* mask_in, const uint8_t* mask_out, const int64_t* seed,
                             float drop_p, float keep_scale, const float* bias, int64_t n_rows, int32_t Dout, float* pre,
```

After: 655.2 million (median of 6 runs). 25.5% lower.
